# SkyTNT/midi-model

Measured on AMD Instinct MI355X. Metric: MIDI events/sec, training step (fwd+bwd+clip+AdamW), tv2o-medium, seq=2048, higher is better.
Workload: dtype bf16; 1 GPU; tv2o-medium bf16 training step, per-GPU batch 16 x 2048 events x 8 tokens (BASELINE.json configs[1]); random-init weights, synthetic events; global_batch=16, seq_len=2048, parallelism=dp1, accumulate_grad_batches=1, optimizer=AdamW bf16-true + global-norm clip 1.0

## Files before the change

### include/midihip.h

```cpp
#ifndef MIDIHIP_H
#define MIDIHIP_H
#include <stdint.h>
#ifdef __cplusplus
extern "C" {
#endif

#define MH_F32 0
#define MH_BF16 1

#define MH_OK 0
#define MH_ERR_ARG (-1)
#define MH_ERR_LAUNCH (-2)
#define MH_ERR_UNSUPPORTED (-3)

const char* mh_last_error(void);
int mh_version(void);
int mh_ab_builds(void);
int mh_set_option(const char* name, int value);
int mh_get_option(const char* name);

int mh_gemm_nt(const void* A, int64_t lda, const void* B, int64_t ldb, void* C, int64_t ldc, const void* R,
               int64_t ldr, int64_t M, int64_t N, int64_t K, float alpha, float beta, int dtype, int splitk,
               void* workspace, void* stream);
int mh_gemm(const void* A, int64_t lda, int transA, const void* B, int64_t ldb, int transB, void* C, int64_t ldc,
            const void* R, int64_t ldr, int64_t M, int64_t N, int64_t K, float alpha, float beta, int dtype, int splitk,
            void* workspace, void* stream);
int mh_gemm_swiglu(const void* A, int64_t lda, const void* W, int64_t ldw, void* GU, int64_t ldgu, void* ACT,
                   int64_t ldact, int64_t M, int64_t I, int64_t K, int dtype, void* stream);
int mh_gemm_rope(const void* A, int64_t lda, const void* W, int64_t ldw, void* C, int64_t ldc, const void* table,
                 int64_t npos, int64_t S, int64_t pos0, int head_dim, int64_t M, int64_t N, int64_t K, int dtype, void* stream);
int mh_gemm_dswiglu(const void* A, int64_t lda, const void* B, int64_t ldb, const void* GU, int64_t ldgu, void* DGU,
                    int64_t lddgu, int64_t M, int64_t I, int64_t K, int dtype, void* stream);
int mh_gemm_rowss(const void* A, int64_t lda, const void* B, int64_t ldb, void* C, int64_t ldc, const void* R, int64_t ldr,
                  float* rowss, int64_t M, int64_t N, int64_t K, int dtype, void* stream);
int mh_row_rstd(const void* x, int64_t ldx, const float* parts, int nparts, int64_t M, int D, float eps, float* rstd, int dtype,
                void* stream);
int mh_gemm_rope_scaled(const void* A, int64_t lda, const void* W, int64_t ldw, void* C, int64_t ldc, const void* table,
                        int64_t npos, int64_t S, int64_t pos0, int head_dim, const float* rowscale, int64_t M, int64_t N, int64_t K,
                        int dtype, void* stream);
int mh_gemm_swiglu_scaled(const void* A, int64_t lda, const void* W, int64_t ldw, void* GU, int64_t ldgu, void* ACT, int64_t ldact,
                          const float* rowscale, int64_t M, int64_t I, int64_t K, int dtype, void* stream);
int mh_gemm_nt_scaled(const void* A, int64_t lda, const void* B, int64_t ldb, void* C, int64_t ldc, const float* rowscale, int64_t M,
                      int64_t N, int64_t K, int dtype, void* stream);
int mh_gemm_dswiglu_scaled(const void* A, int64_t lda, const void* B, int64_t ldb, const void* GU, int64_t ldgu, void* DGU,
                           int64_t lddgu, const float* rowscale, int64_t M, int64_t I, int64_t K, int dtype, void* stream);
int mh_splitk_fold_blocks(int64_t M);
int mh_gemm_splitk_reduce_fold(const void* workspace, void* C, int64_t ldc, const void* R, int64_t ldr, int64_t M, int64_t N,
                               int splitk, float alpha, float beta, const void* wnorm, const void* W, int64_t ldw, float* colpart,
                               int dtype, void* stream);
int mh_rmsnorm_bwd_folded(const void* x, const float* rstd, const void* t, const void* dres, void* dx, int64_t M, int D, int dtype,
                          void* stream);
int mh_scale_cols(const void* W, int64_t ldw, const void* w, void* out, int64_t ldo, int64_t Nr, int K, int dtype, void* stream);
int mh_scale_cols_batched(const int64_t* jobs, int njobs, int K, int dtype, void* stream);
int mh_gemm_splitk_reduce(const void* workspace, void* C, int64_t ldc, const void* R, int64_t ldr, int64_t M,
                          int64_t N, int splitk, float alpha, float beta, int dtype, void* stream);
#define MH_SKINNY_PLAIN 0
#define MH_SKINNY_GATEUP 1
int mh_gemm_skinny(const void* A, int64_t lda, const void* W, int64_t ldw, void* C, int64_t ldc, const void* R,
                   int64_t ldr, int mode, float norm_eps, const int64_t* row_ids, const int64_t* res_ids, int64_t M,
                   int64_t N, int64_t K, int dtype, void* stream);
int mh_transpose(const void* in, int64_t ldi, void* out, int64_t ldo, int64_t rows, int64_t cols, int dtype,
                 void* stream);

int mh_embed_sum_fwd(const int64_t* tok, const void* table, void* out, int64_t M, int T, int64_t V, int D,
                     int dtype, void* stream);
int mh_concat_tok_fwd(const void* hidden, const int64_t* tok, int64_t ldtok, const void* table, void* out,
                      int64_t M, int T, int64_t V, int D, int dtype, void* stream);
int mh_embed_scatter_bwd(const int64_t* tok, int64_t ldtok, int T, const void* dout, int rows_per_m, int jstride,
                         int j0, float* dtable_f32, int64_t M, int64_t V, int D, int64_t pad_id, int dtype,
                         void* stream);
int mh_embed_segment_bwd(const int64_t* src_rows, const int64_t* seg_start, const void* dout, int64_t ld,
                         float* dtable_f32, int64_t V, int D, int64_t n_occ, int64_t pad_id, int dtype, void* stream);
int mh_token_segments_chunk(void);
int mh_token_segments(const int64_t* tok, int64_t ldtok, int64_t n_rows, int n_cols, int64_t V, int64_t row_mul,
                      int64_t col_mul, int64_t add, int64_t* src_rows, int64_t* seg_start, int32_t* work, void* stream);
int mh_cast_from_f32(const float* src, void* dst, int64_t n, int accumulate, int dtype, void* stream);
int mh_copy_rows(const void* src, int64_t src_ld, void* dst, int64_t dst_ld, int64_t M, int D, int accumulate,
                 int dtype, void* stream);

int mh_collate_windows(const int16_t* tokens, int64_t n_events, const int64_t* win_start, const int64_t* win_len,
                       int64_t* out, int64_t B, int64_t L, int T, int64_t pad_id, void* stream);

int mh_augment_piece_stats(const int16_t* tokens, const int64_t* piece_off, int64_t n_pieces, const int32_t* tab,
                           int32_t* stats, void* stream);
int mh_augment_collate_windows(const int16_t* tokens, int64_t n_events, const int64_t* win_start, const int64_t* win_len,
                               const int64_t* win_piece, const int32_t* shifts, const int32_t* stats, const int32_t* tab,
                               int64_t* out, int64_t B, int64_t L, int T, int64_t pad_id, void* stream);

int mh_rmsnorm_fwd(const void* x, const void* w, void* y, float* rstd, int64_t M, int D, float eps, int dtype,
                   void* stream);
int mh_rmsnorm_bwd_blocks(int64_t M);
int mh_rmsnorm_bwd(const void* x, const void* w, const float* rstd, const void* dy, const void* dres, void* dx,
                   float* dw_partial, int64_t M, int D, int dtype, void* stream);
int mh_colsum(float* partial , int64_t nblk, void* out, int D, int accumulate, int dtype, void* stream);

int mh_rope(void* qkv, const float* cos_t, const float* sin_t, int64_t M, int64_t S, int64_t pos0, int H, int hd,
            int dir, int dtype, void* stream);

int mh_attn_prep_fwd(const void* qkv, void* vt, int64_t B, int64_t S, int H, int dtype, void* stream);
int mh_attn_fwd(const void* qkv, const void* vt, void* o, float* lse, int64_t B, int64_t S, int H, float scale,
                int dtype, void* stream);
int mh_attn_prep_bwd(const void* qkv, const void* o, const void* dout, float* delta, void* qt, void* kt, void* dot,
                     int64_t B, int64_t S, int H, int dtype, void* stream);
int mh_attn_bwd(const void* qkv, const void* dout, const float* lse, const float* delta, const void* qt,
                const void* kt, const void* dot, void* dqkv, int64_t B, int64_t S, int H, float scale,
                const float* cos_t, const float* sin_t, int dtype, void* stream);
int mh_attn_bwd_o(const void* qkv, const void* o, const void* dout, const float* lse, float* delta, void* dqkv, int64_t B,
                  int64_t S, int H, float scale, const float* cos_t, const float* sin_t, int dtype, void* stream);
int mh_attn_bwd_o_scaled(const void* qkv, const void* o, const void* dout, const float* lse, float* delta, void* dqkv,
                         const float* rowscale, int64_t B, int64_t S, int H, float scale, const float* cos_t, const float* sin_t,
                         int dtype, void* stream);
int mh_attn_fwd_timeline(const void* qkv, void* o, float* lse, int64_t B, int64_t S, int H, float scale, int lazy,
                         uint32_t* stamps, void* stream);
int mh_attn_fwd_plain(const void* qkv, void* o, float* lse, int64_t B, int64_t S, int H, float scale, int dtype,
                      void* stream);
int mh_attn_bwd_plain(const void* qkv, const void* dout, const float* lse, const float* delta, void* dqkv, int64_t B,
                      int64_t S, int H, float scale, int dtype, void* stream);

int mh_tokattn_fwd(const void* qkv, void* o, int64_t N, int T, int H, float scale, const float* cos_t, const float* sin_t,
                   int dtype, void* stream);
int mh_tokattn_bwd(const void* qkv, const void* dout, void* dqkv, int64_t N, int T, int H, float scale, const float* cos_t,
                   const float* sin_t, int dtype, void* stream);
int mh_tokattn_bwd_scaled(const void* qkv, const void* dout, void* dqkv, const float* rowscale, int64_t N, int T, int H, float scale,
                          const float* cos_t, const float* sin_t, int dtype, void* stream);

int mh_swiglu_fwd(const void* gu, void* a, int64_t M, int I, int dtype, void* stream);
int mh_swiglu_bwd(const void* gu, const void* da, void* dgu, int64_t M, int I, int dtype, void* stream);

int mh_cross_entropy(const void* logits, int64_t ldl, const int64_t* target, float* row_loss, void* dlogits,
                     const float* scale_dev, int64_t* argmax_out, int64_t R, int V, int64_t ignore, int dtype,
                     void* stream);
int mh_sum_f32(const float* x, int64_t n, float* out, void* stream);
int mh_count_valid(const int64_t* target, int64_t n, int64_t ignore, float* count, float* inv, void* stream);

int mh_sumsq(const void* g, int64_t n, float* partial1024, float* out, int accumulate, int dtype, void* stream);
int mh_clip_coef(const float* sumsq, float max_norm, float* coef, float* norm, void* stream);
int mh_adamw(void* p, const void* g, void* m, void* v, int64_t n, float lr, float beta1, float beta2, float eps,
             float weight_decay, float bias_corr1, float bias_corr2, const float* coef_dev, int dtype, void* stream);

int mh_kv_append(void* qkv, const float* cos_t, const float* sin_t, void* kcache, void* vcache, int64_t B, int H,
                 int hd, int64_t Lmax, int64_t pos, const int32_t* pos_dev, int dtype, void* stream);
int mh_attn_decode(const void* qkv, const void* kcache, const void* vcache, void* o, int64_t B, int H, int hd,
                   int64_t Lmax, int64_t len, float scale, const int32_t* pos_dev, int dtype, void* stream);
int mh_attn_decode_append(const void* qkv, const float* cos_t, const float* sin_t, void* kcache, void* vcache, void* o,
                          int64_t B, int H, int hd, int64_t Lmax, int64_t pos, float scale, const int32_t* pos_dev,
                          int dtype, void* stream);
int mh_kv_store_rows(const void* qkv, void* kcache, void* vcache, int64_t B, int64_t S, int H, int hd, int64_t Lmax,
                     int64_t pos0, int dtype, void* stream);
int mh_kv_gather_rows(const void* kcache, const void* vcache, void* qkv, int64_t B, int64_t n, int64_t Stot, int H, int hd,
                      int64_t Lmax, int dtype, void* stream);
int mh_attn_fwd_tail(const void* qkv, void* o, float* lse, int64_t B, int64_t S, int H, float scale, int64_t q_start,
                     int dtype, void* stream);
int mh_kv_store_prefill(const void* qkv, void* kcache, void* vcache, int64_t B, int64_t S, int H, int hd,
                        int64_t Lmax, int dtype, void* stream);

int mh_masked_softmax(const void* logits, int64_t ldl, const int32_t* lo, const int32_t* hi,
                      const uint8_t* first_mask, float* probs, int64_t B, int V, float temp, int dtype,
                      void* stream);
int mh_sample_top_p_k(const void* logits, int64_t ldl, const uint8_t* first_mask, const uint8_t* ban_mask, int first_lo,
                      int first_hi,
                      const int32_t* lo_tab, const int32_t* hi_tab, int tab_stride, int max_range, const int64_t* ev,
                      int pos, const float* q, int64_t* out,
                      int64_t out_stride, int64_t* out_b, int64_t* out_c, int64_t B, int V, float temp, float top_p,
                      int top_k, int fill_rest, int64_t fill_id, int dtype, void* stream);

int mh_comm_unique_id(void* id128);
int mh_comm_init(int rank, int world, const void* id128, int device, void** comm_out);
int mh_comm_info(void* comm, int* rank, int* world, int* rccl_version);
int mh_comm_allreduce(void* comm, void* buf, int64_t count, int dtype, int mean, void* stream);
int mh_comm_broadcast(void* comm, void* buf, int64_t count, int dtype, int root, void* stream);
int mh_comm_destroy(void* comm);

#ifdef __cplusplus
}
#endif
#endif
```

### midi-model_amd/csrc/attention_mfma.hip

```cpp
#include "attn_mfma_common.h"

#ifdef MH_AB_BUILDS
template <bool MASK>
__device__ inline void fwd_tile(const char* tK, const char* tV, const bf16x8 (&qf)[4], f32x16 (&oacc)[2], float& m,
                                float& l, int pli, int hi, int qrel, float sc) {
  f32x16 sacc[2] = {zero16(), zero16()};
#pragma unroll
  for (int kb = 0; kb < 2; ++kb)
#pragma unroll
    for (int s = 0; s < 4; ++s) sacc[kb] = mfma32(lds_frag(tK, kb * 32 + pli, 2 * s + hi), qf[s], sacc[kb]);
  float mx = -INFINITY;
#pragma unroll
  for (int kb = 0; kb < 2; ++kb)
#pragma unroll
    for (int r = 0; r < 16; ++r) {
      if (MASK) {
        if (kb * 32 + reg_index(r, hi) > qrel) sacc[kb][r] = -INFINITY;
      }
      mx = fmaxf(mx, sacc[kb][r]);
    }
  mx = fmaxf(mx, __shfl_xor(mx, 32, 64)) * sc;
  float mn = m, alpha = 1.f;
  if (__any(mx > m + RESCALE_THR)) {
    mn = fmaxf(m, mx);
// ... 291 lines not shown
  f32x16 dkacc[2] = {zero16(), zero16()}, dvacc[2] = {zero16(), zero16()};
  const int pli = pi32(li);
  const int qt_first = k0 / 64, qt_last = (S - 1) / 64;

  auto stage_all = [&](int qt, char* dst) {
    stage64(qbase, D3, (int64_t)qt * 64, S - 1, 0, dst, wave, lane);
    stage64(dobase, D, (int64_t)qt * 64, S - 1, 0, dst + TILE64, wave, lane);
    stage64(qtbase, Sp, 0, HD - 1, (int64_t)qt * 64, dst + 2 * TILE64, wave, lane);
    stage64(dotbase, Sp, 0, HD - 1, (int64_t)qt * 64, dst + 3 * TILE64, wave, lane);
    if (wave < 2) {
      const float* base = (wave == 0 ? lse_b : delta_b) + (int64_t)qt * 64;
      int l15 = lane & 15;
      asm volatile("" : "+v"(l15));
      glds16(base + 4 * l15, dst + 4 * TILE64 + wave * 1024);
    }
  };
  if (qt_first <= qt_last) stage_all(qt_first, smem);
#pragma unroll
  for (int s = 0; s < 4; ++s) {
    asm volatile("" : "+v"(kf[s]));
    asm volatile("" : "+v"(vf[s]));
  }
  __syncthreads();
  for (int qt = qt_first; qt <= qt_last; ++qt) {
    const int st = (qt - qt_first) & 1;
    const char* cur = smem + st * STG;
    char* nxt = smem + (st ^ 1) * STG;
    if (qt + 1 <= qt_last) stage_all(qt + 1, nxt);
    const int qs = qt * 64;
    if (qs + 63 >= kw0) {
      if (qs < kw0 + 31 || qs + 64 > S)
        dkv_tile<true>(cur, cur + TILE64, cur + 2 * TILE64, cur + 3 * TILE64, kf, vf, dkacc, dvacc, cur + 4 * TILE64, pli, hi,
                       krow - qs, S - qs, sc);
      else
        dkv_tile<false>(cur, cur + TILE64, cur + 2 * TILE64, cur + 3 * TILE64, kf, vf, dkacc, dvacc, cur + 4 * TILE64, pli, hi,
                        0, 64, sc);
    }
    __syncthreads();
  }
  if (krow < S) {
    bf16* krow_out = dqkv + (b * S + krow) * D3 + D + (int64_t)h * HD;
    store_grad_row(krow_out, dkacc, scale, hi, cos_t, sin_t, krow);
    store_grad_row(krow_out + D, dvacc, 1.f, hi, nullptr, nullptr, 0);
  }
}

#endif

extern thread_local int g_attn_v3;
int mh_attn_fwd_mfma3(const void* qkv, const void* vt, void* o, float* lse, int64_t B, int64_t S, int H, float scale,
                      hipStream_t st, int64_t q_start = 0);
int mh_attn_bwd_mfma3(const void* qkv, const void* dout, const float* lse, const float* delta, const void* qt, const void* kt,
                      const void* dot, void* dqkv, int64_t B, int64_t S, int H, float scale, const float* cos_t,
                      const float* sin_t, int which, hipStream_t st, const void* o = nullptr);

int mh_attn_fwd_mfma(const void* qkv, const void* vt, void* o, float* lse, int64_t B, int64_t S, int H, float scale,
                     hipStream_t st, int64_t q_start) {
  MH_REQUIRE(S < (1 << 24), "attn_fwd: sequence too long");
  if ((g_attn_v3 & 1) && (vt != nullptr || (g_attn_v3 & 16)))
    return mh_attn_fwd_mfma3(qkv, vt, o, lse, B, S, H, scale, st, q_start);
  MH_REQUIRE(q_start == 0, "attn_fwd_tail: served by the third form of the forward kernel only");
#ifndef MH_AB_BUILDS
  MH_REQUIRE(false, "attn_fwd(bf16): option attn_v3 = %d selects the first form of the kernel, which is only in the A/B test "
             "library (libmidihip_ab.so)", g_attn_v3);
#else
  MH_REQUIRE(vt != nullptr, "attn_fwd(bf16): the first form needs the transposed V copy (mh_attn_prep_fwd)");
  const int64_t Sp = (S + 63) / 64 * 64;
  const int nt = (int)((S + 127) / 128), BH = (int)(B * H);
  const unsigned grid = (unsigned)(nt * 8 * ((BH + 7) / 8));
  attn_fwd_kernel<<<grid, 256, 4 * TILE64, st>>>((const bf16*)qkv, (const bf16*)vt, (bf16*)o, lse, (int)S, (int)Sp, H,
                                        scale * LOG2E, BH, nt);
  MH_LAUNCH_CHECK();
  return MH_OK;
#endif
}

int mh_attn_bwd_o_mfma(const void* qkv, const void* o, const void* dout, const float* lse, float* delta, void* dqkv, int64_t B,
                       int64_t S, int H, float scale, const float* cos_t, const float* sin_t, hipStream_t st) {
  MH_REQUIRE(S < (1 << 24), "attn_bwd: sequence too long");
  MH_REQUIRE((g_attn_v3 & 14) == 14, "attn_bwd_o: served by the third form with transpose reads (mh_set_option(\"attn_v3\") bits 2|4|8); "
             "use mh_attn_prep_bwd + mh_attn_bwd otherwise");
  return mh_attn_bwd_mfma3(qkv, dout, lse, delta, nullptr, nullptr, nullptr, dqkv, B, S, H, scale, cos_t, sin_t, 14, st, o);
}

int mh_attn_bwd_mfma(const void* qkv, const void* dout, const float* lse, const float* delta, const void* qt,
                     const void* kt, const void* dot, void* dqkv, int64_t B, int64_t S, int H, float scale,
                     const float* cos_t, const float* sin_t, hipStream_t st) {
  MH_REQUIRE(S < (1 << 24), "attn_bwd: sequence too long");
  if ((g_attn_v3 & 14) == 14)
    return mh_attn_bwd_mfma3(qkv, dout, lse, delta, nullptr, nullptr, nullptr, dqkv, B, S, H, scale, cos_t, sin_t, 14, st);
  MH_REQUIRE(qt != nullptr && kt != nullptr && dot != nullptr, "attn_bwd(bf16): needs the transposed copies (mh_attn_prep_bwd)");
  const int64_t Sp = (S + 63) / 64 * 64;
  const int nt = (int)((S + 127) / 128), BH = (int)(B * H);
  const unsigned grid = (unsigned)(nt * 8 * ((BH + 7) / 8));
  if (g_attn_v3 & 6) {
    const int rc = mh_attn_bwd_mfma3(qkv, dout, lse, delta, qt, kt, dot, dqkv, B, S, H, scale, cos_t, sin_t, g_attn_v3 & 14, st);
    if (rc != MH_OK) return rc;
  }
#ifndef MH_AB_BUILDS
  MH_REQUIRE((g_attn_v3 & 6) == 6, "attn_bwd(bf16): option attn_v3 = %d selects first-form kernels, which are only in the A/B "
             "test library (libmidihip_ab.so)", g_attn_v3);
#else
  if (!(g_attn_v3 & 2)) {
    attn_bwd_dq_kernel<<<grid, 256, 6 * TILE64, st>>>((const bf16*)qkv, (const bf16*)dout, lse, delta, (const bf16*)kt,
                                             (bf16*)dqkv, (int)S, (int)Sp, H, scale, BH, nt, cos_t, sin_t);
    MH_LAUNCH_CHECK();
  }
  if (!(g_attn_v3 & 4)) {
    attn_bwd_dkv_kernel<<<grid, 256, 2 * DKV_STAGE, st>>>((const bf16*)qkv, (const bf16*)dout, lse, delta, (const bf16*)qt,
                                              (const bf16*)dot, (bf16*)dqkv, (int)S, (int)Sp, H, scale, BH, nt, cos_t, sin_t);
    MH_LAUNCH_CHECK();
  }
#endif
  (void)grid;
  return MH_OK;
}
```

### midi-model_amd/csrc/attention_mfma3.hip

```cpp
#include <stdlib.h>

#include "attn_mfma_common.h"

static int attn_env_int(const char* name, int dflt) {
  const char* v = getenv(name);
  return (v && *v) ? atoi(v) : dflt;
}
thread_local int g_attn_v3 = attn_env_int("MH_ATTN_V3", 255);
thread_local int g_attn_passes = attn_env_int("MH_ATTN_PASSES", 5);
thread_local int g_attn_v3_wps = attn_env_int("MH_ATTN_V3_WPS", 0);
thread_local const float* g_attn_bwd_rowscale = nullptr;

__device__ inline bf16x8 ldsv(const char* p) { return *reinterpret_cast<const bf16x8*>(p); }
typedef __attribute__((ext_vector_type(2))) float f32x2;
typedef __attribute__((ext_vector_type(2))) __bf16 bf16x2;
__device__ inline bf16x8 pack8_pk(const f32x16& v, int base) {
  union {
    bf16x8 v;
    bf16x2 h[4];
  } r;
#pragma unroll
  for (int i = 0; i < 4; ++i) r.h[i] = __builtin_convertvector(f32x2{v[base + 2 * i], v[base + 2 * i + 1]}, bf16x2);
  return r.v;
}
__device__ inline float xhalf_max(float v) {
  const int iv = __float_as_int(v);
  const auto pr = __builtin_amdgcn_permlane32_swap(iv, iv, false, false);
  return fmaxf(__int_as_float(pr[0]), __int_as_float(pr[1]));
}

constexpr float LZ_BOUND = 1099511627776.f;
__device__ inline uint64_t tl_now() {
  uint64_t t;
  asm volatile("s_memtime %0" : "=s"(t));
  return t;
}
template <bool MASK, bool TR, bool LZ = false, bool TL = false>
__device__ inline void fwd3_tile(const char* tK, const char* tV, const int (&trof)[2][2], const int (&foff)[4],
                                 const bf16x8 (&qf)[4], f32x16 (&oacc)[2], float& m, float& l, int hi, int qrel, float sc,
                                 uint64_t* ts = nullptr) {
  bf16x8 kf[2][4];
#pragma unroll
  for (int s = 0; s < 4; ++s)
#pragma unroll
    for (int kb = 0; kb < 2; ++kb) kf[kb][s] = ldsv(tK + foff[s] + kb * 4096);
  __builtin_amdgcn_sched_barrier(0);
  if constexpr (TL) ts[2] = tl_now();
  f32x16 sacc[2] = {zero16(), zero16()};
#pragma unroll
  for (int s = 0; s < 4; ++s)
#pragma unroll
    for (int kb = 0; kb < 2; ++kb) sacc[kb] = mfma32(kf[kb][s], qf[s], sacc[kb]);
  bf16x8 vf[4][2];
  u32x2 vr[4][2][2];
  if (TR) {
    unsigned tv[2][2];
#pragma unroll
    for (int db = 0; db < 2; ++db)
#pragma unroll
      for (int half = 0; half < 2; ++half) tv[db][half] = lds_addr32(tV) + (unsigned)trof[db][half];
#pragma unroll
    for (int db = 0; db < 2; ++db)
#pragma unroll
      for (int half = 0; half < 2; ++half) {
// ... 743 lines not shown
#define MH_FWD(WPS, TR_, LZ_)                                                                                                    \
  attn_fwd3_kernel<WPS, TR_, 2, LZ_><<<grid, 256, 4 * TILE64, st>>>((const bf16*)qkv, (const bf16*)vt, (bf16*)o, lse, (int)S, (int)Sp, H, \
                                                                 scale * LOG2E, BH, nt, nt_all)
#define MH_FWD3S(WPS, TR_, LZ_)                                                                                                  \
  attn_fwd3_kernel<WPS, TR_, 3, LZ_><<<grid, 256, 6 * TILE64, st>>>((const bf16*)qkv, (const bf16*)vt, (bf16*)o, lse, (int)S, (int)Sp, \
                                                                  H, scale * LOG2E, BH, nt, nt_all)
  const bool tr = (vt == nullptr);
  const bool lz = (g_attn_v3 & 128) != 0;
  if (tr && g_attn_v3_wps == 4) {
    if (lz) MH_FWD(4, true, true); else MH_FWD(4, true, false);
  } else if (tr && (g_attn_v3 & 64)) {
    if (lz) {
      if (g_attn_v3_wps == 3) MH_FWD3S(3, true, true); else MH_FWD3S(2, true, true);
    } else {
      if (g_attn_v3_wps == 3) MH_FWD3S(3, true, false); else MH_FWD3S(2, true, false);
    }
  } else if (tr) {
    if (g_attn_v3_wps == 3) MH_FWD(3, true, false); else MH_FWD(2, true, false);
  } else {
    if (g_attn_v3_wps == 2) MH_FWD(2, false, false); else MH_FWD(3, false, false);
  }
#undef MH_FWD
#undef MH_FWD3S
  MH_LAUNCH_CHECK();
  return MH_OK;
}

extern "C" int mh_attn_fwd_timeline(const void* qkv, void* o, float* lse, int64_t B, int64_t S, int H, float scale, int lazy,
                                    uint32_t* stamps, void* stream) {
#ifdef MH_AB_BUILDS
  MH_REQUIRE(stamps != nullptr && S >= 128 && S * 3 * H * HD < (int64_t(1) << 31), "attn_fwd_timeline: bad arguments");
  hipStream_t st = (hipStream_t)stream;
  const int64_t Sp = (S + 63) / 64 * 64;
  const int nt_all = (int)((S + 127) / 128), BH0 = (int)(B * H), nt = nt_all;
  const int BH = BH0 | ((g_attn_passes & 127) << 24);
  const unsigned grid = (unsigned)(nt * 8 * ((BH0 + 7) / 8));
  if (lazy)
    attn_fwd3_kernel<2, true, 3, true, true><<<grid, 256, 6 * TILE64 + TL_BYTES, st>>>((const bf16*)qkv, (const bf16*)stamps, (bf16*)o, lse, (int)S,
                                                                                   (int)Sp, H, scale * LOG2E, BH, nt, nt_all);
  else
    attn_fwd3_kernel<2, true, 3, false, true><<<grid, 256, 6 * TILE64 + TL_BYTES, st>>>((const bf16*)qkv, (const bf16*)stamps, (bf16*)o, lse, (int)S,
                                                                                    (int)Sp, H, scale * LOG2E, BH, nt, nt_all);
  MH_LAUNCH_CHECK();
  return MH_OK;
#else
  mh_set_error("attn_fwd_timeline: only in the A/B library (libmidihip_ab.so)");
  return MH_ERR_UNSUPPORTED;
#endif
}

int mh_attn_bwd_mfma3(const void* qkv, const void* dout, const float* lse, const float* delta, const void* qt, const void* kt,
                      const void* dot, void* dqkv, int64_t B, int64_t S, int H, float scale, const float* cos_t,
                      const float* sin_t, int which ,
                      hipStream_t st, const void* o ) {
  MH_REQUIRE(o == nullptr || (which & 14) == 14, "attn_bwd: delta inside the dQ kernel needs the third form of both kernels");
  MH_REQUIRE(S * 3 * H * HD < (int64_t(1) << 31), "attn_bwd: sequence too long (32-bit panel offsets)");
  const bool tr = (which & 8) != 0;
  MH_REQUIRE(tr || (qt != nullptr && kt != nullptr && dot != nullptr), "attn_bwd(bf16): needs the transposed copies (mh_attn_prep_bwd)");
  const int64_t Sp = (S + 63) / 64 * 64;
  const int nt = (int)((S + 127) / 128), BH0 = (int)(B * H);
  MH_REQUIRE(BH0 < (1 << 24), "attn_bwd: too many (batch, head) pairs");
  const int BH = BH0 | ((g_attn_passes & 127) << 24);
  const unsigned grid = (unsigned)(nt * 8 * ((BH0 + 7) / 8));
#define MH_DQ(WPS, TR_)                                                                                                     \
  attn_bwd_dq3_kernel<WPS, TR_><<<grid, 256, (TR_ ? 4 : 6) * TILE64, st>>>((const bf16*)qkv, (const bf16*)dout, lse, delta,     \
                                                                        (const bf16*)kt, (bf16*)dqkv, (int)S, (int)Sp, H, scale, \
                                                                        BH, nt, cos_t, sin_t, (const bf16*)o,         \
                                                                        const_cast<float*>(delta), g_attn_bwd_rowscale)
  if (which & 2) {
    if (g_attn_v3_wps == 2) {
      if (tr) MH_DQ(2, true); else MH_DQ(2, false);
    } else {
      if (tr) MH_DQ(3, true); else MH_DQ(3, false);
    }
    MH_LAUNCH_CHECK();
  }
#undef MH_DQ
  if (which & 4) {
    if (tr && o != nullptr)
      attn_bwd_dkv3_kernel<true, true><<<grid, 256, 2 * (2 * TILE64 + 2048), st>>>((const bf16*)qkv, (const bf16*)dout,
                                                                                 delta + (int64_t)BH0 * Sp, delta, nullptr, nullptr,
                                                                                 (bf16*)dqkv, (int)S, (int)Sp, H, scale, BH, nt,
                                                                                 cos_t, sin_t, g_attn_bwd_rowscale);
    else if (tr)
      attn_bwd_dkv3_kernel<true><<<grid, 256, 2 * (2 * TILE64 + 2048), st>>>((const bf16*)qkv, (const bf16*)dout, lse, delta, nullptr,
                                                                           nullptr, (bf16*)dqkv, (int)S, (int)Sp, H, scale, BH, nt,
                                                                           cos_t, sin_t, g_attn_bwd_rowscale);
    else
      attn_bwd_dkv3_kernel<false><<<grid, 256, 2 * DKV_STAGE, st>>>((const bf16*)qkv, (const bf16*)dout, lse, delta, (const bf16*)qt,
                                                                  (const bf16*)dot, (bf16*)dqkv, (int)S, (int)Sp, H, scale, BH, nt,
                                                                  cos_t, sin_t, g_attn_bwd_rowscale);
    MH_LAUNCH_CHECK();
  }
  return MH_OK;
}
```

### midi-model_amd/csrc/attention_small.hip

```cpp
#include "common.h"

#define DISPATCH_T(dtype, CALL)                                    \
  do {                                                             \
    if ((dtype) == MH_BF16) { using T = bf16; CALL; }              \
    else if ((dtype) == MH_F32) { using T = float; CALL; }         \
    else { mh_set_error("bad dtype %d", (int)(dtype)); return MH_ERR_ARG; } \
  } while (0)

template <typename T> __device__ inline void ld4(const T* p, float (&o)[4]);
template <> __device__ inline void ld4<float>(const float* p, float (&o)[4]) {
  f32x4 v = *reinterpret_cast<const f32x4*>(p);
  o[0] = v[0]; o[1] = v[1]; o[2] = v[2]; o[3] = v[3];
}
template <> __device__ inline void ld4<bf16>(const bf16* p, float (&o)[4]) {
  bf16x4 v = *reinterpret_cast<const bf16x4*>(p);
  o[0] = (float)v[0]; o[1] = (float)v[1]; o[2] = (float)v[2]; o[3] = (float)v[3];
}
template <typename T> __device__ inline void st4(T* p, const float (&o)[4]);
template <> __device__ inline void st4<float>(float* p, const float (&o)[4]) {
  *reinterpret_cast<f32x4*>(p) = f32x4{o[0], o[1], o[2], o[3]};
}
template <> __device__ inline void st4<bf16>(bf16* p, const float (&o)[4]) {
  bf16x4 v;
  v[0] = (bf16)o[0]; v[1] = (bf16)o[1]; v[2] = (bf16)o[2]; v[3] = (bf16)o[3];
// ... 90 lines not shown
      for (int t = 0; t < TN; ++t) {
        unpack(kraw[t], k[t]);
        unpack(vraw[t], v[t]);
        if (rot) rope_row<T>(k[t], rope_c, rope_s, t, lane, 1.f, true);
      }
    } else {
#pragma unroll
      for (int t = 0; t < TK; ++t) {
        if (t < Tn) {
          ldp<T>(base + t * D3 + D, lane, k[t]);
          ldp<T>(base + t * D3 + 2 * D, lane, v[t]);
          if (rot) rope_row<T>(k[t], rope_c, rope_s, t, lane, 1.f, true);
        }
      }
    }
#pragma unroll
    for (int i = 0; i < TK; ++i) {
      if (TN ? i >= TN : i >= Tn) break;
      float q[4];
      if constexpr (TN != 0) unpack(qraw[i], q);
      else ldp<T>(base + i * D3, lane, q);
      if (rot) rope_row<T>(q, rope_c, rope_s, i, lane, 1.f, true);
      float s[TK];
      float mx = -INFINITY;
#pragma unroll
      for (int j = 0; j <= i; ++j) {
        float p = q[0] * k[j][0] + q[1] * k[j][1] + q[2] * k[j][2] + q[3] * k[j][3];
        s[j] = wave_sum_fast(p) * scale;
        mx = fmaxf(mx, s[j]);
      }
      float den = 0.f;
#pragma unroll
      for (int j = 0; j <= i; ++j) {
        s[j] = __expf(s[j] - mx);
        den += s[j];
      }
      const float inv = 1.f / den;
      float acc[4] = {0.f, 0.f, 0.f, 0.f};
#pragma unroll
      for (int j = 0; j <= i; ++j) {
        const float p = s[j] * inv;
#pragma unroll
        for (int e = 0; e < 4; ++e) acc[e] += p * v[j][e];
      }
      stp<T>(o + (n * Tn + i) * D + (int64_t)h * 256, lane, acc);
    }
  }
}

template <typename T, int TN, bool BR>
__global__ __launch_bounds__(256) void tokattn_bwd_kernel(const T* __restrict__ qkv, const T* __restrict__ dout,
                                                          T* __restrict__ dqkv, int64_t NH, int Tn, int H, float scale,
                                                          const float* __restrict__ cos_t, const float* __restrict__ sin_t,
                                                          const float* __restrict__ rowscale ) {
  const int lane = threadIdx.x & 63;
  const int64_t D = (int64_t)H * 256, D3 = 3 * D;
  __shared__ float rope_c[TK * 128], rope_s[TK * 128];
  const bool rot = cos_t != nullptr;
  if (rot) {
    for (int i = threadIdx.x; i < Tn * 128; i += 256) {
      rope_c[i] = rnd<T>(cos_t[i]);
      rope_s[i] = rnd<T>(sin_t[i]);
    }
    __syncthreads();
  }
  for (int64_t w = (int64_t)blockIdx.x * 4 + (threadIdx.x >> 6); w < NH; w += (int64_t)gridDim.x * 4) {
    const int64_t n = w / H;
    const int h = (int)(w - n * H);
    const int64_t off = (int64_t)h * 256;
    const T* base = qkv + n * Tn * D3 + off;
    T* ob = dqkv + n * Tn * D3 + off;
    float k[TK][4], v[TK][4], dk[TK][4], dv[TK][4];
    RawRow<T> qraw[TN ? TN : 1], doraw[TN ? TN : 1];
    const float rs_lane = (rowscale != nullptr && lane < Tn) ? rowscale[n * Tn + lane] : 1.f;
#pragma unroll
    for (int t = 0; t < TK; ++t)
#pragma unroll
      for (int e = 0; e < 4; ++e) dk[t][e] = dv[t][e] = 0.f;
    if constexpr (TN != 0) {
      RawRow<T> kraw[TN ? TN : 1], vraw[TN ? TN : 1];
#pragma unroll
      for (int t = 0; t < TN; ++t) {
        kraw[t] = ldraw<T>(base + t * D3 + D, lane);
        vraw[t] = ldraw<T>(base + t * D3 + 2 * D, lane);
      }
#pragma unroll
      for (int t = 0; t < TN; ++t) {
        qraw[t] = ldraw<T>(base + t * D3, lane);
        doraw[t] = ldraw<T>(dout + (n * Tn + t) * D + off, lane);
      }
#pragma unroll
      for (int t = 0; t < TN; ++t) {
        unpack(kraw[t], k[t]);
        unpack(vraw[t], v[t]);
        if (rot) rope_row<T>(k[t], rope_c, rope_s, t, lane, 1.f, true);
      }
    } else {
#pragma unroll
      for (int t = 0; t < TK; ++t) {
        if (t < Tn) {
          ldp<T>(base + t * D3 + D, lane, k[t]);
          ldp<T>(base + t * D3 + 2 * D, lane, v[t]);
          if (rot) rope_row<T>(k[t], rope_c, rope_s, t, lane, 1.f, true);
        }
      }
    }
#pragma unroll
    for (int i = 0; i < TK; ++i) {
      if (TN ? i >= TN : i >= Tn) break;
      float q[4], dO[4], dq[4] = {0.f, 0.f, 0.f, 0.f};
      if constexpr (TN != 0) {
        unpack(qraw[i], q);
        unpack(doraw[i], dO);
      } else {
        ldp<T>(base + i * D3, lane, q);
        ldp<T>(dout + (n * Tn + i) * D + off, lane, dO);
      }
      if (rot) rope_row<T>(q, rope_c, rope_s, i, lane, 1.f, true);
      float p[TK], dp[TK];
      float mx = -INFINITY;
      if constexpr (BR) {
#pragma unroll
        for (int j = 0; j <= i; j += 2) {
          const bool two = j + 1 <= i;
          const int j1 = two ? j + 1 : j;
          const float a0 = q[0] * k[j][0] + q[1] * k[j][1] + q[2] * k[j][2] + q[3] * k[j][3];
          const float b0 = dO[0] * v[j][0] + dO[1] * v[j][1] + dO[2] * v[j][2] + dO[3] * v[j][3];
          const float a1 = two ? q[0] * k[j1][0] + q[1] * k[j1][1] + q[2] * k[j1][2] + q[3] * k[j1][3] : 0.f;
          const float b1 = two ? dO[0] * v[j1][0] + dO[1] * v[j1][1] + dO[2] * v[j1][2] + dO[3] * v[j1][3] : 0.f;
          const float r4 = wave_sum4(a0, b0, a1, b1);
          p[j] = wave_sum4_get<0>(r4) * scale;
          dp[j] = wave_sum4_get<1>(r4);
          mx = fmaxf(mx, p[j]);
          if (two) {
            p[j1] = wave_sum4_get<2>(r4) * scale;
            dp[j1] = wave_sum4_get<3>(r4);
            mx = fmaxf(mx, p[j1]);
          }
        }
      } else {
#pragma unroll
      for (int j = 0; j <= i; ++j) {
        float a = q[0] * k[j][0] + q[1] * k[j][1] + q[2] * k[j][2] + q[3] * k[j][3];
        float b = dO[0] * v[j][0] + dO[1] * v[j][1] + dO[2] * v[j][2] + dO[3] * v[j][3];
        p[j] = wave_sum_fast(a) * scale;
        dp[j] = wave_sum_fast(b);
        mx = fmaxf(mx, p[j]);
      }
      }
      float den = 0.f;
#pragma unroll
      for (int j = 0; j <= i; ++j) {
        p[j] = __expf(p[j] - mx);
        den += p[j];
      }
      const float inv = 1.f / den;
      float dsum = 0.f;
#pragma unroll
      for (int j = 0; j <= i; ++j) {
        p[j] *= inv;
        dsum += p[j] * dp[j];
      }
#pragma unroll
      for (int j = 0; j <= i; ++j) {
        const float ds = p[j] * (dp[j] - dsum) * scale;
#pragma unroll
        for (int e = 0; e < 4; ++e) {
          dq[e] += ds * k[j][e];
          dk[j][e] += ds * q[e];
          dv[j][e] += p[j] * dO[e];
        }
      }
      if (rot) rope_row<T>(dq, rope_c, rope_s, i, lane, -1.f, false);
      if (rowscale != nullptr) {
        const float rsc = __shfl(rs_lane, i, 64);
#pragma unroll
        for (int e = 0; e < 4; ++e) dq[e] *= rsc;
      }
      stp<T>(ob + i * D3, lane, dq);
    }
#pragma unroll
    for (int t = 0; t < TK; ++t) {
      if (TN ? t < TN : t < Tn) {
        if (rot) rope_row<T>(dk[t], rope_c, rope_s, t, lane, -1.f, false);
        if (rowscale != nullptr) {
          const float rsc = __shfl(rs_lane, t, 64);
#pragma unroll
          for (int e = 0; e < 4; ++e) {
            dk[t][e] *= rsc;
            dv[t][e] *= rsc;
          }
        }
        stp<T>(ob + t * D3 + D, lane, dk[t]);
        stp<T>(ob + t * D3 + 2 * D, lane, dv[t]);
      }
    }
  }
}

extern "C" int mh_tokattn_fwd(const void* qkv, void* o, int64_t N, int Tn, int H, float scale, const float* cos_t,
                              const float* sin_t, int dtype, void* stream) {
  MH_REQUIRE(N > 0 && Tn >= 1 && Tn <= TK && H >= 1, "tokattn_fwd: bad shape N=%ld T=%d H=%d", (long)N, Tn, H);
  const int64_t NH = N * H;
  int64_t g = (NH + 3) / 4;
  if (g > 32768) g = 32768;
  if (Tn == TK)
    DISPATCH_T(dtype, (tokattn_fwd_kernel<T, TK><<<(int)g, 256, 0, (hipStream_t)stream>>>((const T*)qkv, (T*)o, NH, Tn, H, scale,
                                                                                          cos_t, sin_t)));
  else
    DISPATCH_T(dtype, (tokattn_fwd_kernel<T, 0><<<(int)g, 256, 0, (hipStream_t)stream>>>((const T*)qkv, (T*)o, NH, Tn, H, scale,
                                                                                         cos_t, sin_t)));
  MH_LAUNCH_CHECK();
  return MH_OK;
}

thread_local int g_tokattn_bwd_batched = 1;
static int tokattn_bwd_any(const void* qkv, const void* dout, void* dqkv, const float* rowscale, int64_t N, int Tn, int H, float scale,
                           const float* cos_t, const float* sin_t, int dtype, void* stream) {
  MH_REQUIRE(N > 0 && Tn >= 1 && Tn <= TK && H >= 1, "tokattn_bwd: bad shape");
  const int64_t NH = N * H;
  int64_t g = (NH + 3) / 4;
  if (g > 32768) g = 32768;
  if (Tn == TK && g_tokattn_bwd_batched)
    DISPATCH_T(dtype, (tokattn_bwd_kernel<T, TK, true><<<(int)g, 256, 0, (hipStream_t)stream>>>(
                          (const T*)qkv, (const T*)dout, (T*)dqkv, NH, Tn, H, scale, cos_t, sin_t, rowscale)));
  else if (Tn == TK)
    DISPATCH_T(dtype, (tokattn_bwd_kernel<T, TK, false><<<(int)g, 256, 0, (hipStream_t)stream>>>(
                          (const T*)qkv, (const T*)dout, (T*)dqkv, NH, Tn, H, scale, cos_t, sin_t, rowscale)));
  else
    DISPATCH_T(dtype, (tokattn_bwd_kernel<T, 0, false><<<(int)g, 256, 0, (hipStream_t)stream>>>(
                          (const T*)qkv, (const T*)dout, (T*)dqkv, NH, Tn, H, scale, cos_t, sin_t, rowscale)));
  MH_LAUNCH_CHECK();
  return MH_OK;
}
extern "C" int mh_tokattn_bwd(const void* qkv, const void* dout, void* dqkv, int64_t N, int Tn, int H, float scale,
                              const float* cos_t, const float* sin_t, int dtype, void* stream) {
  return tokattn_bwd_any(qkv, dout, dqkv, nullptr, N, Tn, H, scale, cos_t, sin_t, dtype, stream);
}
extern "C" int mh_tokattn_bwd_scaled(const void* qkv, const void* dout, void* dqkv, const float* rowscale, int64_t N, int Tn, int H,
                                     float scale, const float* cos_t, const float* sin_t, int dtype, void* stream) {
  MH_REQUIRE(rowscale != nullptr, "tokattn_bwd_scaled: rowscale is NULL");
  return tokattn_bwd_any(qkv, dout, dqkv, rowscale, N, Tn, H, scale, cos_t, sin_t, dtype, stream);
}

template <typename T>
__global__ __launch_bounds__(256) void kv_append_kernel(T* __restrict__ qkv, const float* __restrict__ cos_t,
                                                        const float* __restrict__ sin_t, T* __restrict__ kc,
                                                        T* __restrict__ vc, int64_t B, int H, int hd, int64_t Lmax,
                                                        int64_t pos, const int32_t* __restrict__ pos_dev) {
  if (pos_dev != nullptr) pos = *pos_dev;
  if (pos >= Lmax) return;
  const int half = hd / 2;
  const int64_t total = B * H * half;
  const int64_t D = (int64_t)H * hd;
  for (int64_t it = (int64_t)blockIdx.x * 256 + threadIdx.x; it < total; it += (int64_t)gridDim.x * 256) {
    const int i = (int)(it % half);
    const int64_t bh = it / half;
    const int h = (int)(bh % H);
    const int64_t b = bh / H;
    const float c = rnd<T>(cos_t[pos * half + i]), s = rnd<T>(sin_t[pos * half + i]);
    T* row = qkv + b * 3 * D + (int64_t)h * hd;
    const float q1 = to_f(row[i]), q2 = to_f(row[i + half]);
    row[i] = from_f<T>(q1 * c - q2 * s);
    row[i + half] = from_f<T>(q2 * c + q1 * s);
    const float k1 = to_f(row[D + i]), k2 = to_f(row[D + i + half]);
    const T kr1 = from_f<T>(k1 * c - k2 * s), kr2 = from_f<T>(k2 * c + k1 * s);
    row[D + i] = kr1;
    row[D + i + half] = kr2;
    T* kd = kc + ((b * H + h) * Lmax + pos) * hd;
    T* vd = vc + ((b * H + h) * Lmax + pos) * hd;
    kd[i] = kr1;
    kd[i + half] = kr2;
    vd[i] = row[2 * D + i];
    vd[i + half] = row[2 * D + i + half];
  }
}

extern "C" int mh_kv_append(void* qkv, const float* cos_t, const float* sin_t, void* kcache, void* vcache, int64_t B,
                            int H, int hd, int64_t Lmax, int64_t pos, const int32_t* pos_dev, int dtype, void* stream) {
  MH_REQUIRE(B > 0 && H > 0 && hd % 2 == 0 && ((pos >= 0 && pos < Lmax) || pos_dev != nullptr),
             "kv_append: bad args (pos=%ld Lmax=%ld)", (long)pos, (long)Lmax);
  const int64_t total = B * H * (hd / 2);
  DISPATCH_T(dtype, (kv_append_kernel<T><<<(int)((total + 255) / 256), 256, 0, (hipStream_t)stream>>>(
                        (T*)qkv, cos_t, sin_t, (T*)kcache, (T*)vcache, B, H, hd, Lmax, pos, pos_dev)));
  MH_LAUNCH_CHECK();
  return MH_OK;
}

template <typename T>
__global__ __launch_bounds__(256) void kv_store_prefill_kernel(const T* __restrict__ qkv, T* __restrict__ kc,
                                                               T* __restrict__ vc, int64_t B, int64_t S, int H, int hd,
                                                               int64_t Lmax, int64_t pos0) {
  constexpr int N = Pack<T>::N;
  const int cph = hd / N;
  const int64_t total = B * S * H * cph;
// ... 517 lines not shown
#pragma unroll
    for (int e = 0; e < N; ++e) tile[i][ch * N + e] = v.v[e];
  }
  __syncthreads();
  for (int p = 0; p < 64 / RPP; ++p) {
    const int d = rr + p * RPP;
    Pack<T> v;
#pragma unroll
    for (int e = 0; e < N; ++e) v.v[e] = tile[ch * N + e][d];
    st16(out + (bh * 64 + d) * Sp + s0 + ch * N, v);
  }
}

template <typename T>
static int transpose_heads(const T* in, int64_t ld, int64_t col0, T* out, int64_t B, int64_t S, int H, hipStream_t st) {
  const int64_t Sp = (S + 63) / 64 * 64;
  dim3 grid((unsigned)(Sp / 64), (unsigned)(B * H));
  attn_transpose_kernel<T><<<grid, 256, 0, st>>>(in, ld, col0, out, S, Sp, H);
  MH_LAUNCH_CHECK();
  return MH_OK;
}

extern "C" int mh_attn_prep_fwd(const void* qkv, void* vt, int64_t B, int64_t S, int H, int dtype, void* stream) {
  MH_REQUIRE(B > 0 && S > 0 && H > 0 && B * H < 65536, "attn_prep_fwd: bad shape");
  if (dtype != MH_BF16) return MH_OK;
  const int64_t D = (int64_t)H * 64;
  return transpose_heads<bf16>((const bf16*)qkv, 3 * D, 2 * D, (bf16*)vt, B, S, H, (hipStream_t)stream);
}

extern "C" int mh_attn_prep_bwd(const void* qkv, const void* o, const void* dout, float* delta, void* qt, void* kt,
                                void* dot, int64_t B, int64_t S, int H, int dtype, void* stream) {
  MH_REQUIRE(B > 0 && S > 0 && H > 0 && B * H < 65536, "attn_prep_bwd: bad shape");
  hipStream_t st = (hipStream_t)stream;
  const int64_t total = B * S * H;
  int64_t g = (total * 8 + 255) / 256;
  if (g > 16384) g = 16384;
  DISPATCH_T(dtype, (attn_delta_kernel<T><<<(int)g, 256, 0, st>>>((const T*)o, (const T*)dout, delta, B, S, H)));
  MH_LAUNCH_CHECK();
  if (dtype != MH_BF16 || qt == nullptr) return MH_OK;
  const int64_t D = (int64_t)H * 64;
  int rc;
  if ((rc = transpose_heads<bf16>((const bf16*)qkv, 3 * D, 0, (bf16*)qt, B, S, H, st)) != MH_OK) return rc;
  if ((rc = transpose_heads<bf16>((const bf16*)qkv, 3 * D, D, (bf16*)kt, B, S, H, st)) != MH_OK) return rc;
  return transpose_heads<bf16>((const bf16*)dout, D, 0, (bf16*)dot, B, S, H, st);
}

int mh_attn_fwd_mfma(const void* qkv, const void* vt, void* o, float* lse, int64_t B, int64_t S, int H, float scale,
                     hipStream_t st, int64_t q_start);
int mh_attn_bwd_mfma(const void* qkv, const void* dout, const float* lse, const float* delta, const void* qt,
                     const void* kt, const void* dot, void* dqkv, int64_t B, int64_t S, int H, float scale,
                     const float* cos_t, const float* sin_t, hipStream_t st);

int mh_attn_bwd_o_mfma(const void* qkv, const void* o, const void* dout, const float* lse, float* delta, void* dqkv, int64_t B,
                       int64_t S, int H, float scale, const float* cos_t, const float* sin_t, hipStream_t st);

template <typename T>
static int attn_plain_fwd(const void* qkv, void* o, float* lse, int64_t B, int64_t S, int H, float scale, hipStream_t st,
                          int64_t q_start = 0) {
  const int first = (int)(q_start / 64);
  dim3 grid((unsigned)((S + 63) / 64 - first), (unsigned)(B * H));
  attn_plain_fwd_kernel<T><<<grid, 64, 0, st>>>((const T*)qkv, (T*)o, lse, S, H, scale, first);
  MH_LAUNCH_CHECK();
  return MH_OK;
}

template <typename T>
static int attn_plain_bwd(const void* qkv, const void* dout, const float* lse, const float* delta, void* dqkv, int64_t B,
                          int64_t S, int H, float scale, hipStream_t st) {
  dim3 grid((unsigned)((S + 63) / 64), (unsigned)(B * H));
  attn_plain_bwd_dq_kernel<T><<<grid, 64, 0, st>>>((const T*)qkv, (const T*)dout, lse, delta, (T*)dqkv, S, H, scale);
  MH_LAUNCH_CHECK();
  attn_plain_bwd_dkv_kernel<T><<<grid, 64, 0, st>>>((const T*)qkv, (const T*)dout, lse, delta, (T*)dqkv, S, H, scale);
  MH_LAUNCH_CHECK();
  return MH_OK;
}

extern "C" int mh_attn_fwd_plain(const void* qkv, void* o, float* lse, int64_t B, int64_t S, int H, float scale,
                                 int dtype, void* stream) {
  MH_REQUIRE(B > 0 && S > 0 && H > 0 && B * H < 65536, "attn_fwd: bad shape");
  DISPATCH_T(dtype, return attn_plain_fwd<T>(qkv, o, lse, B, S, H, scale, (hipStream_t)stream));
}

extern "C" int mh_attn_bwd_plain(const void* qkv, const void* dout, const float* lse, const float* delta, void* dqkv,
                                 int64_t B, int64_t S, int H, float scale, int dtype, void* stream) {
  MH_REQUIRE(B > 0 && S > 0 && H > 0 && B * H < 65536, "attn_bwd: bad shape");
  DISPATCH_T(dtype, return attn_plain_bwd<T>(qkv, dout, lse, delta, dqkv, B, S, H, scale, (hipStream_t)stream));
}

extern "C" int mh_attn_fwd(const void* qkv, const void* vt, void* o, float* lse, int64_t B, int64_t S, int H, float scale,
                           int dtype, void* stream) {
  MH_REQUIRE(B > 0 && S > 0 && H > 0 && B * H < 65536, "attn_fwd: bad shape");
  if (dtype == MH_BF16) return mh_attn_fwd_mfma(qkv, vt, o, lse, B, S, H, scale, (hipStream_t)stream, 0);
  if (dtype == MH_F32) return attn_plain_fwd<float>(qkv, o, lse, B, S, H, scale, (hipStream_t)stream);
  mh_set_error("attn_fwd: bad dtype");
  return MH_ERR_ARG;
}

extern "C" int mh_attn_fwd_tail(const void* qkv, void* o, float* lse, int64_t B, int64_t S, int H, float scale, int64_t q_start,
                                int dtype, void* stream) {
  MH_REQUIRE(B > 0 && S > 0 && H > 0 && B * H < 65536 && q_start >= 0 && q_start < S, "attn_fwd_tail: bad shape");
  if (dtype == MH_BF16) return mh_attn_fwd_mfma(qkv, nullptr, o, lse, B, S, H, scale, (hipStream_t)stream, q_start);
  if (dtype == MH_F32) return attn_plain_fwd<float>(qkv, o, lse, B, S, H, scale, (hipStream_t)stream, q_start);
  mh_set_error("attn_fwd_tail: bad dtype");
  return MH_ERR_ARG;
}

extern "C" int mh_rope(void* qkv, const float* cos_t, const float* sin_t, int64_t M, int64_t S, int64_t pos0, int H, int hd,
                       int dir, int dtype, void* stream);

extern "C" int mh_attn_bwd(const void* qkv, const void* dout, const float* lse, const float* delta, const void* qt,
                           const void* kt, const void* dot, void* dqkv, int64_t B, int64_t S, int H, float scale,
                           const float* cos_t, const float* sin_t, int dtype, void* stream) {
  MH_REQUIRE(B > 0 && S > 0 && H > 0 && B * H < 65536, "attn_bwd: bad shape");
  MH_REQUIRE((cos_t == nullptr) == (sin_t == nullptr), "attn_bwd: cos and sin tables come together");
  if (dtype == MH_BF16)
    return mh_attn_bwd_mfma(qkv, dout, lse, delta, qt, kt, dot, dqkv, B, S, H, scale, cos_t, sin_t, (hipStream_t)stream);
  if (dtype == MH_F32) {
    int rc = attn_plain_bwd<float>(qkv, dout, lse, delta, dqkv, B, S, H, scale, (hipStream_t)stream);
    if (rc == MH_OK && cos_t != nullptr) rc = mh_rope(dqkv, cos_t, sin_t, B * S, S, 0, H, 64, -1, dtype, stream);
    return rc;
  }
  mh_set_error("attn_bwd: bad dtype");
  return MH_ERR_ARG;
}

extern thread_local const float* g_attn_bwd_rowscale;
extern thread_local int g_attn_v3;
extern "C" int mh_attn_bwd_o_scaled(const void* qkv, const void* o, const void* dout, const float* lse, float* delta, void* dqkv,
                                    const float* rowscale, int64_t B, int64_t S, int H, float scale, const float* cos_t,
                                    const float* sin_t, int dtype, void* stream) {
  MH_REQUIRE(rowscale != nullptr, "attn_bwd_o_scaled: rowscale is NULL");
  MH_REQUIRE((g_attn_v3 & 46) == 46, "attn_bwd_o_scaled: needs the third form of the backward kernels (attn_v3 bits 1, 2, 3, 5)");
  g_attn_bwd_rowscale = rowscale;
  const int rc = mh_attn_bwd_o(qkv, o, dout, lse, delta, dqkv, B, S, H, scale, cos_t, sin_t, dtype, stream);
  g_attn_bwd_rowscale = nullptr;
  return rc;
}

extern "C" int mh_attn_bwd_o(const void* qkv, const void* o, const void* dout, const float* lse, float* delta, void* dqkv,
                             int64_t B, int64_t S, int H, float scale, const float* cos_t, const float* sin_t, int dtype,
                             void* stream) {
  MH_REQUIRE(B > 0 && S > 0 && H > 0 && B * H < 65536, "attn_bwd_o: bad shape");
  MH_REQUIRE((cos_t == nullptr) == (sin_t == nullptr), "attn_bwd_o: cos and sin tables come together");
  MH_REQUIRE(dtype == MH_BF16, "attn_bwd_o: bf16 only (fp32: mh_attn_prep_bwd + mh_attn_bwd)");
  return mh_attn_bwd_o_mfma(qkv, o, dout, lse, delta, dqkv, B, S, H, scale, cos_t, sin_t, (hipStream_t)stream);
}
```

### midi-model_amd/csrc/elementwise.hip

```cpp
#include "common.h"

#define DISPATCH_T(dtype, CALL)                                    \
  do {                                                             \
    if ((dtype) == MH_BF16) { using T = bf16; CALL; }              \
    else if ((dtype) == MH_F32) { using T = float; CALL; }         \
    else { mh_set_error("bad dtype %d", (int)(dtype)); return MH_ERR_ARG; } \
  } while (0)

static inline int grid_for(int64_t items, int per_block, int cap = 1 << 20) {
  int64_t g = (items + per_block - 1) / per_block;
  if (g < 1) g = 1;
  if (g > cap) g = cap;
  return (int)g;
}

template <typename T>
__global__ __launch_bounds__(256) void embed_sum_fwd_kernel(const int64_t* __restrict__ tok, const T* __restrict__ table,
                                                            T* __restrict__ out, int64_t M, int TT, int D, int64_t V) {
  constexpr int N = Pack<T>::N;
  const int lane = threadIdx.x & 63;
  const int64_t wave0 = (int64_t)blockIdx.x * 4 + (threadIdx.x >> 6);
  for (int64_t m = wave0; m < M; m += (int64_t)gridDim.x * 4) {
    constexpr int TMAXI = 8;
    int64_t ids[TMAXI];
// ... 489 lines not shown
  else
    DISPATCH_T(dtype, (rmsnorm_fwd_kernel<T><<<grid_for(M, 4, 65536), 256, 0, (hipStream_t)stream>>>(
                          (const T*)x, (const T*)w, (T*)y, rstd, M, D, eps)));
#undef MH_RMSF
  MH_LAUNCH_CHECK();
  return MH_OK;
}

__global__ __launch_bounds__(256) void rstd_from_parts_kernel(const float* __restrict__ parts, int nparts, int64_t M, float inv_d,
                                                              float eps, float* __restrict__ rstd) {
  __shared__ float acc[4][64];
  const int r = threadIdx.x & 63, q = threadIdx.x >> 6;
  const int64_t m = (int64_t)blockIdx.x * 64 + r;
  float ss = 0.f;
  if (m < M) {
#pragma unroll 4
    for (int p = q; p < nparts; p += 4) ss += parts[(int64_t)p * M + m];
  }
  acc[q][r] = ss;
  __syncthreads();
  if (q == 0 && m < M) rstd[m] = rsqrtf((acc[0][r] + acc[1][r] + acc[2][r] + acc[3][r]) * inv_d + eps);
}
template <typename T>
__global__ __launch_bounds__(256) void row_rstd_kernel(const T* __restrict__ x, int64_t ldx, int64_t M, int D, float eps,
                                                       float* __restrict__ rstd) {
  constexpr int N = Pack<T>::N;
  const int lane = threadIdx.x & 63;
  for (int64_t m = (int64_t)blockIdx.x * 4 + (threadIdx.x >> 6); m < M; m += (int64_t)gridDim.x * 4) {
    const T* xr = x + m * ldx;
    float ss = 0.f;
    for (int c = lane * N; c < D; c += 64 * N) {
      Pack<T> v = ld16(xr + c);
#pragma unroll
      for (int e = 0; e < N; ++e) ss += v.get(e) * v.get(e);
    }
    ss = wave_sum(ss);
    if (lane == 0) rstd[m] = rsqrtf(ss / (float)D + eps);
  }
}
extern "C" int mh_row_rstd(const void* x, int64_t ldx, const float* parts, int nparts, int64_t M, int D, float eps, float* rstd,
                           int dtype, void* stream) {
  MH_REQUIRE(M > 0 && D > 0 && rstd != nullptr && ((x != nullptr) != (parts != nullptr)), "row_rstd: give x OR parts (M=%ld D=%d)", (long)M, D);
  if (parts != nullptr) {
    MH_REQUIRE(nparts > 0 && (int64_t)nparts * 64 == D, "row_rstd: nparts = %d must be D / 64 (D = %d): one sum of squares per 64 columns", nparts, D);
    rstd_from_parts_kernel<<<(unsigned)((M + 63) / 64), 256, 0, (hipStream_t)stream>>>(parts, nparts, M, 1.0f / (float)D, eps, rstd);
  } else {
    MH_REQUIRE(D % 8 == 0 && ldx % 8 == 0 && ldx >= D && ((uintptr_t)x & 15) == 0, "row_rstd: rows must be 16-byte aligned");
    DISPATCH_T(dtype, (row_rstd_kernel<T><<<grid_for(M, 4, 65536), 256, 0, (hipStream_t)stream>>>((const T*)x, ldx, M, D, eps, rstd)));
  }
  MH_LAUNCH_CHECK();
  return MH_OK;
}

constexpr int RMS_BWD_MAX_BLOCKS = 1024;
extern "C" int mh_rmsnorm_bwd_blocks(int64_t M) {
  int64_t g = (M + 3) / 4;
  return (int)(g < RMS_BWD_MAX_BLOCKS ? (g < 1 ? 1 : g) : RMS_BWD_MAX_BLOCKS);
}

template <typename T>
__global__ __launch_bounds__(256) void rmsnorm_bwd_kernel(const T* __restrict__ x, const T* __restrict__ w,
                                                          const float* __restrict__ rstd, const T* __restrict__ dy,
                                                          const T* dres, T* dx, float* __restrict__ dw_partial,
                                                          int64_t M, int D) {
  constexpr int N = Pack<T>::N;
  extern __shared__ __attribute__((aligned(16))) float dw_acc[];
  const int lane = threadIdx.x & 63, wv = threadIdx.x >> 6;
  float* mine = dw_acc + wv * D;
  for (int c = lane; c < D; c += 64) mine[c] = 0.f;
  __syncthreads();
  for (int64_t m = (int64_t)blockIdx.x * 4 + wv; m < M; m += (int64_t)gridDim.x * 4) {
    const T* xr = x + m * D;
    const T* gr = dy + m * D;
    const float r = rstd[m];
    float dot = 0.f;
    for (int c = lane * N; c < D; c += 64 * N) {
      Pack<T> xv = ld16(xr + c), gv = ld16(gr + c), wv_ = ld16(w + c);
#pragma unroll
      for (int e = 0; e < N; ++e) dot += gv.get(e) * wv_.get(e) * (xv.get(e) * r);
    }
    dot = wave_sum(dot) / (float)D;
    for (int c = lane * N; c < D; c += 64 * N) {
      Pack<T> xv = ld16(xr + c), gv = ld16(gr + c), wv_ = ld16(w + c), o;
      Pack<T> rv;
      if (dres != nullptr) rv = ld16(dres + m * D + c);
#pragma unroll
      for (int e = 0; e < N; ++e) {
        const float xh = xv.get(e) * r;
        float d = r * (gv.get(e) * wv_.get(e) - xh * dot);
        if (dres != nullptr) d += rv.get(e);
        o.set(e, d);
        mine[c + e] += gv.get(e) * rnd<T>(xh);
      }
      st16(dx + m * D + c, o);
    }
  }
  __syncthreads();
  for (int c = threadIdx.x; c < D; c += 256)
    dw_partial[(int64_t)blockIdx.x * D + c] = dw_acc[c] + dw_acc[D + c] + dw_acc[2 * D + c] + dw_acc[3 * D + c];
}

template <typename T, int NCH, bool NT>
__global__ __launch_bounds__(256) void rmsnorm_bwd_reg_kernel(const T* __restrict__ x, const T* __restrict__ w,
                                                              const float* __restrict__ rstd, const T* __restrict__ dy,
                                                              const T* dres, T* dx, float* __restrict__ dw_partial,
                                                              int64_t M, int D) {
// ... 388 lines not shown
```

### midi-model_amd/csrc/gemm.hip

```cpp
#include <type_traits>

#include "common.h"

__device__ __attribute__((aligned(16))) char g_zero16[16];

template <typename T> struct Mma;
template <> struct Mma<bf16> {
  __device__ static inline f32x4 run(const Pack<bf16>& a, const Pack<bf16>& b, f32x4 c) {
    return __builtin_amdgcn_mfma_f32_16x16x32_bf16(a.v, b.v, c, 0, 0, 0);
  }
};
template <> struct Mma<float> {
  __device__ static inline f32x4 run(const Pack<float>& a, const Pack<float>& b, f32x4 c) {
#pragma unroll
    for (int e = 0; e < 4; ++e) c = __builtin_amdgcn_mfma_f32_16x16x4f32(a.v[e], b.v[e], c, 0, 0, 0);
    return c;
  }
};

constexpr int BM = 128, BN = 128;
constexpr int TILE_BYTES = 128 * 128;

template <typename T>
__device__ inline void stage_tile(const T* __restrict__ base, int64_t ld, int64_t row0, int64_t nrows, int64_t k0,
// ... 250 lines not shown
}

template <bool FOLD>
__global__ __launch_bounds__(256) void splitk_reduce4_kernel(const float* __restrict__ ws, bf16* __restrict__ C, int64_t ldc,
                                                             const bf16* R, int64_t ldr, int64_t M, int64_t N, int splitk,
                                                             float alpha, float beta, const bf16* __restrict__ wnorm,
                                                             const bf16* __restrict__ W, int64_t ldw, float* __restrict__ colpart);

template <typename T>
static int splitk_reduce_launch(const void* workspace, void* C, int64_t ldc, const void* R, int64_t ldr, int64_t M,
                                int64_t N, int splitk, float alpha, float beta, hipStream_t st) {
  MH_REQUIRE(M > 0 && N > 0 && splitk >= 1 && workspace != nullptr, "splitk_reduce: bad args");
  if constexpr (std::is_same<T, bf16>::value) {
    if (N % 4 == 0 && ldc % 4 == 0 && (R == nullptr || ldr % 4 == 0) && (((uintptr_t)C | (uintptr_t)R) & 7) == 0 &&
        ((uintptr_t)workspace & 15) == 0) {
      const int64_t rows_y = M < 2048 ? M : 2048;
      dim3 grid((unsigned)((N / 4 + 255) / 256), (unsigned)rows_y);
      splitk_reduce4_kernel<false><<<grid, 256, 0, st>>>((const float*)workspace, (bf16*)C, ldc, (const bf16*)R, ldr, M, N, splitk, alpha,
                                                         beta, nullptr, nullptr, 0, nullptr);
      MH_LAUNCH_CHECK();
      return MH_OK;
    }
  }
  const int64_t total = M * N;
  const int blocks = (int)((total + 255) / 256 < 4096 ? (total + 255) / 256 : 4096);
  splitk_reduce_kernel<T><<<blocks, 256, 0, st>>>((const float*)workspace, (T*)C, ldc, (const T*)R, ldr, M, N, splitk,
                                                  alpha, beta);
  MH_LAUNCH_CHECK();
  return MH_OK;
}

extern "C" int mh_gemm_splitk_reduce(const void* workspace, void* C, int64_t ldc, const void* R, int64_t ldr, int64_t M,
                                     int64_t N, int splitk, float alpha, float beta, int dtype, void* stream) {
  hipStream_t st = (hipStream_t)stream;
  if (dtype == MH_BF16) return splitk_reduce_launch<bf16>(workspace, C, ldc, R, ldr, M, N, splitk, alpha, beta, st);
  if (dtype == MH_F32) return splitk_reduce_launch<float>(workspace, C, ldc, R, ldr, M, N, splitk, alpha, beta, st);
  mh_set_error("splitk_reduce: bad dtype %d", dtype);
  return MH_ERR_ARG;
}

extern "C" int mh_gemm(const void* A, int64_t lda, int transA, const void* B, int64_t ldb, int transB, void* C,
                       int64_t ldc, const void* R, int64_t ldr, int64_t M, int64_t N, int64_t K, float alpha, float beta,
                       int dtype, int splitk, void* workspace, void* stream) {
  hipStream_t st = (hipStream_t)stream;
  if (dtype == MH_BF16)
    return gemm_launch<bf16>(A, lda, transA, B, ldb, transB, C, ldc, R, ldr, M, N, K, alpha, beta, splitk, workspace, st);
  if (dtype == MH_F32)
    return gemm_launch<float>(A, lda, transA, B, ldb, transB, C, ldc, R, ldr, M, N, K, alpha, beta, splitk, workspace, st);
  mh_set_error("gemm: bad dtype %d", dtype);
  return MH_ERR_ARG;
}

int mh_gemm_pp256_dswiglu_bf16(const void* A, int64_t lda, const void* B, int64_t ldb, const void* GU, int64_t ldgu,
                               void* DGU, int64_t lddgu, int64_t M, int64_t I, int64_t K, hipStream_t st, const float* rowscale);
int mh_gemm_pp256_scaled_bf16(const void* A, int64_t lda, const void* B, int64_t ldb, void* C, int64_t ldc, int64_t M, int64_t N,
                              int64_t K, const float* rowscale, hipStream_t st);

int mh_gemm_pp256_swiglu_bf16(const void* A, int64_t lda, const void* W, int64_t ldw, void* GU, int64_t ldgu, void* ACT,
                              int64_t ldact, int64_t M, int64_t I, int64_t K, hipStream_t st, const float* rowscale);

static int gemm_swiglu_any(const void* A, int64_t lda, const void* W, int64_t ldw, void* GU, int64_t ldgu, void* ACT,
                           int64_t ldact, const float* rowscale, int64_t M, int64_t I, int64_t K, int dtype, void* stream);

extern "C" int mh_gemm_swiglu(const void* A, int64_t lda, const void* W, int64_t ldw, void* GU, int64_t ldgu, void* ACT,
                              int64_t ldact, int64_t M, int64_t I, int64_t K, int dtype, void* stream) {
  return gemm_swiglu_any(A, lda, W, ldw, GU, ldgu, ACT, ldact, nullptr, M, I, K, dtype, stream);
}
extern "C" int mh_gemm_swiglu_scaled(const void* A, int64_t lda, const void* W, int64_t ldw, void* GU, int64_t ldgu, void* ACT,
                                     int64_t ldact, const float* rowscale, int64_t M, int64_t I, int64_t K, int dtype, void* stream) {
  MH_REQUIRE(rowscale != nullptr && ((uintptr_t)rowscale & 15) == 0, "gemm_swiglu_scaled: rowscale must be a 16-byte aligned fp32 [M]");
  return gemm_swiglu_any(A, lda, W, ldw, GU, ldgu, ACT, ldact, rowscale, M, I, K, dtype, stream);
}

static int gemm_swiglu_any(const void* A, int64_t lda, const void* W, int64_t ldw, void* GU, int64_t ldgu, void* ACT,
                           int64_t ldact, const float* rowscale, int64_t M, int64_t I, int64_t K, int dtype, void* stream) {
  MH_REQUIRE(dtype == MH_BF16 && g_mh_gemm_variant != 0,
             "gemm_swiglu: served by the production bf16 kernel only (use mh_gemm + mh_swiglu_fwd otherwise)");
  MH_REQUIRE(M > 0 && I > 0 && K > 0 && I % 128 == 0, "gemm_swiglu: bad shape M=%ld I=%ld K=%ld (I must be a multiple of 128)",
             (long)M, (long)I, (long)K);
  MH_REQUIRE(lda % 8 == 0 && ldw % 8 == 0 && ldact % 8 == 0 && lda >= K && ldw >= K && ldact >= I &&
                 (GU == nullptr || (ldgu % 8 == 0 && ldgu >= 2 * I)),
             "gemm_swiglu: leading dimensions must be multiples of 8 elements and cover the rows");
  MH_REQUIRE((((uintptr_t)A | (uintptr_t)W | (uintptr_t)GU | (uintptr_t)ACT) & 15) == 0, "gemm_swiglu: 16-byte alignment");
  return mh_gemm_pp256_swiglu_bf16(A, lda, W, ldw, GU, ldgu, ACT, ldact, M, I, K, (hipStream_t)stream, rowscale);
}

int mh_gemm_pp256_rope_bf16(const void* A, int64_t lda, const void* W, int64_t ldw, void* C, int64_t ldc, const void* table,
                            int64_t S, int64_t pos0, int64_t M, int64_t N, int64_t K, hipStream_t st, const float* rowscale);

static int gemm_rope_any(const void* A, int64_t lda, const void* W, int64_t ldw, void* C, int64_t ldc, const void* table,
                         int64_t npos, int64_t S, int64_t pos0, int head_dim, const float* rowscale, int64_t M, int64_t N, int64_t K,
                         int dtype, void* stream);

extern "C" int mh_gemm_rope(const void* A, int64_t lda, const void* W, int64_t ldw, void* C, int64_t ldc, const void* table,
                            int64_t npos, int64_t S, int64_t pos0, int head_dim, int64_t M, int64_t N, int64_t K, int dtype,
                            void* stream) {
  return gemm_rope_any(A, lda, W, ldw, C, ldc, table, npos, S, pos0, head_dim, nullptr, M, N, K, dtype, stream);
}
extern "C" int mh_gemm_rope_scaled(const void* A, int64_t lda, const void* W, int64_t ldw, void* C, int64_t ldc, const void* table,
                                   int64_t npos, int64_t S, int64_t pos0, int head_dim, const float* rowscale, int64_t M, int64_t N,
                                   int64_t K, int dtype, void* stream) {
  MH_REQUIRE(rowscale != nullptr && ((uintptr_t)rowscale & 15) == 0, "gemm_rope_scaled: rowscale must be a 16-byte aligned fp32 [M]");
  return gemm_rope_any(A, lda, W, ldw, C, ldc, table, npos, S, pos0, head_dim, rowscale, M, N, K, dtype, stream);
}

static int gemm_rope_any(const void* A, int64_t lda, const void* W, int64_t ldw, void* C, int64_t ldc, const void* table,
                         int64_t npos, int64_t S, int64_t pos0, int head_dim, const float* rowscale, int64_t M, int64_t N, int64_t K,
                         int dtype, void* stream) {
  MH_REQUIRE(dtype == MH_BF16 && g_mh_gemm_variant != 0,
             "gemm_rope: served by the production bf16 kernel only (use mh_gemm + mh_rope otherwise)");
  MH_REQUIRE(M > 0 && K > 0 && N > 0 && N % 192 == 0 && head_dim == 64,
             "gemm_rope: bad shape M=%ld N=%ld K=%ld head_dim=%d (N = 3 * heads * 64)", (long)M, (long)N, (long)K, head_dim);
  MH_REQUIRE(S > 0 && pos0 >= 0 && pos0 + (S < M ? S : M) <= npos && npos < (int64_t(1) << 31), "gemm_rope: table too short");
  MH_REQUIRE(S < (int64_t(1) << 31), "gemm_rope: S = %ld does not fit the 32 bits it travels in", (long)S);
  MH_REQUIRE(lda % 8 == 0 && ldw % 8 == 0 && ldc % 8 == 0 && lda >= K && ldw >= K && ldc >= N,
             "gemm_rope: leading dimensions must be multiples of 8 elements and cover the rows");
  MH_REQUIRE((((uintptr_t)A | (uintptr_t)W | (uintptr_t)C | (uintptr_t)table) & 15) == 0, "gemm_rope: 16-byte alignment");
  return mh_gemm_pp256_rope_bf16(A, lda, W, ldw, C, ldc, table, S, pos0, M, N, K, (hipStream_t)stream, rowscale);
}

int mh_gemm_pp256_rowss_bf16(const void* A, int64_t lda, const void* B, int64_t ldb, void* C, int64_t ldc, const void* R,
                             int64_t ldr, int64_t M, int64_t N, int64_t K, float* rowss, hipStream_t st);

extern "C" int mh_gemm_rowss(const void* A, int64_t lda, const void* B, int64_t ldb, void* C, int64_t ldc, const void* R,
                             int64_t ldr, float* rowss, int64_t M, int64_t N, int64_t K, int dtype, void* stream) {
  MH_REQUIRE(dtype == MH_BF16 && g_mh_gemm_variant != 0, "gemm_rowss: served by the production bf16 kernel only");
  MH_REQUIRE(M > 0 && N > 0 && K > 0 && N % 64 == 0 && rowss != nullptr, "gemm_rowss: bad shape M=%ld N=%ld K=%ld (N must be a multiple of 64)",
             (long)M, (long)N, (long)K);
  MH_REQUIRE(lda % 8 == 0 && ldb % 8 == 0 && ldc % 8 == 0 && lda >= K && ldb >= K && ldc >= N && (R == nullptr || (ldr % 8 == 0 && ldr >= N)),
             "gemm_rowss: leading dimensions must be multiples of 8 elements and cover the rows");
  MH_REQUIRE((((uintptr_t)A | (uintptr_t)B | (uintptr_t)C | (uintptr_t)R) & 15) == 0, "gemm_rowss: 16-byte alignment");
  MH_REQUIRE(((M + 255) / 256) * ((N + 255) / 256) < (1ll << 30), "gemm_rowss: too many tiles");
  return mh_gemm_pp256_rowss_bf16(A, lda, B, ldb, C, ldc, R, ldr, M, N, K, rowss, (hipStream_t)stream);
}

extern "C" int mh_gemm_dswiglu(const void* A, int64_t lda, const void* B, int64_t ldb, const void* GU, int64_t ldgu,
                               void* DGU, int64_t lddgu, int64_t M, int64_t I, int64_t K, int dtype, void* stream) {
  MH_REQUIRE(dtype == MH_BF16 && g_mh_gemm_variant != 0,
             "gemm_dswiglu: served by the production bf16 kernel only (use mh_gemm + mh_swiglu_bwd otherwise)");
  MH_REQUIRE(M > 0 && I > 0 && K > 0 && I % 8 == 0, "gemm_dswiglu: bad shape M=%ld I=%ld K=%ld", (long)M, (long)I, (long)K);
  MH_REQUIRE(lda % 8 == 0 && ldb % 8 == 0 && ldgu % 8 == 0 && lddgu % 8 == 0 && lda >= K && ldb >= I && ldgu >= 2 * I &&
                 lddgu >= 2 * I,
             "gemm_dswiglu: leading dimensions must be multiples of 8 elements and cover the rows");
  MH_REQUIRE((((uintptr_t)A | (uintptr_t)B | (uintptr_t)GU | (uintptr_t)DGU) & 15) == 0, "gemm_dswiglu: 16-byte alignment");
  return mh_gemm_pp256_dswiglu_bf16(A, lda, B, ldb, GU, ldgu, DGU, lddgu, M, I, K, (hipStream_t)stream, nullptr);
}

extern "C" int mh_gemm_dswiglu_scaled(const void* A, int64_t lda, const void* B, int64_t ldb, const void* GU, int64_t ldgu,
                                      void* DGU, int64_t lddgu, const float* rowscale, int64_t M, int64_t I, int64_t K, int dtype,
                                      void* stream) {
  MH_REQUIRE(dtype == MH_BF16 && g_mh_gemm_variant != 0, "gemm_dswiglu_scaled: served by the production bf16 kernel only");
  MH_REQUIRE(rowscale != nullptr && ((uintptr_t)rowscale & 15) == 0, "gemm_dswiglu_scaled: rowscale must be a 16-byte aligned fp32 [M]");
  MH_REQUIRE(M > 0 && I > 0 && K > 0 && I % 8 == 0, "gemm_dswiglu_scaled: bad shape M=%ld I=%ld K=%ld", (long)M, (long)I, (long)K);
  MH_REQUIRE(lda % 8 == 0 && ldb % 8 == 0 && ldgu % 8 == 0 && lddgu % 8 == 0 && lda >= K && ldb >= I && ldgu >= 2 * I &&
                 lddgu >= 2 * I,
             "gemm_dswiglu_scaled: leading dimensions must be multiples of 8 elements and cover the rows");
  MH_REQUIRE((((uintptr_t)A | (uintptr_t)B | (uintptr_t)GU | (uintptr_t)DGU) & 15) == 0, "gemm_dswiglu_scaled: 16-byte alignment");
  return mh_gemm_pp256_dswiglu_bf16(A, lda, B, ldb, GU, ldgu, DGU, lddgu, M, I, K, (hipStream_t)stream, rowscale);
}

extern "C" int mh_gemm_nt_scaled(const void* A, int64_t lda, const void* B, int64_t ldb, void* C, int64_t ldc,
                                 const float* rowscale, int64_t M, int64_t N, int64_t K, int dtype, void* stream) {
  MH_REQUIRE(dtype == MH_BF16 && g_mh_gemm_variant != 0, "gemm_nt_scaled: served by the production bf16 kernel only");
  MH_REQUIRE(rowscale != nullptr && ((uintptr_t)rowscale & 15) == 0, "gemm_nt_scaled: rowscale must be a 16-byte aligned fp32 [M]");
  MH_REQUIRE(M > 0 && N > 0 && K > 0, "gemm_nt_scaled: empty problem");
  MH_REQUIRE(lda % 8 == 0 && ldb % 8 == 0 && lda >= K && ldb >= K && ldc >= N, "gemm_nt_scaled: leading dimensions");
  MH_REQUIRE((((uintptr_t)A | (uintptr_t)B) & 15) == 0, "gemm_nt_scaled: 16-byte alignment");
  MH_REQUIRE(((M + 255) / 256) * ((N + 255) / 256) < (1ll << 30), "gemm_nt_scaled: too many tiles");
  return mh_gemm_pp256_scaled_bf16(A, lda, B, ldb, C, ldc, M, N, K, rowscale, (hipStream_t)stream);
}

constexpr int SKF_MAX_BLOCKS = 1024;
extern "C" int mh_splitk_fold_blocks(int64_t M) { return (int)(M < SKF_MAX_BLOCKS ? (M < 1 ? 1 : M) : SKF_MAX_BLOCKS); }

template <bool FOLD>
__global__ __launch_bounds__(256) void splitk_reduce4_kernel(const float* __restrict__ ws, bf16* __restrict__ C, int64_t ldc,
                                                             const bf16* R, int64_t ldr, int64_t M, int64_t N, int splitk,
                                                             float alpha, float beta, const bf16* __restrict__ wnorm,
                                                             const bf16* __restrict__ W, int64_t ldw, float* __restrict__ colpart) {
  const int64_t c = ((int64_t)blockIdx.x * 256 + threadIdx.x) * 4;
  if (c >= N) return;
  const int64_t total = M * N;
  float wn[4] = {1.f, 1.f, 1.f, 1.f}, cs[4] = {0.f, 0.f, 0.f, 0.f};
  if constexpr (FOLD) {
    const bf16x4 w4 = *reinterpret_cast<const bf16x4*>(wnorm + c);
#pragma unroll
    for (int e = 0; e < 4; ++e) wn[e] = (float)w4[e];
  }
  const bool use_r = (R != nullptr && beta != 0.f);
  for (int64_t m = blockIdx.y; m < M; m += gridDim.y) {
    f32x4 s = *reinterpret_cast<const f32x4*>(ws + m * N + c);
    if (splitk <= 8) {
      f32x4 p[7];
#pragma unroll
      for (int z = 1; z < 8; ++z)
        if (z < splitk) p[z - 1] = *reinterpret_cast<const f32x4*>(ws + (int64_t)z * total + m * N + c);
#pragma unroll
      for (int z = 1; z < 8; ++z)
        if (z < splitk) {
#pragma unroll
          for (int e = 0; e < 4; ++e) s[e] += p[z - 1][e];
        }
    } else {
      for (int z = 1; z < splitk; ++z) {
        const f32x4 p = *reinterpret_cast<const f32x4*>(ws + (int64_t)z * total + m * N + c);
#pragma unroll
        for (int e = 0; e < 4; ++e) s[e] += p[e];
      }
    }
    float x[4];
#pragma unroll
// ... 100 lines not shown
```

### midi-model_amd/csrc/gemm_pp256.hip

```cpp
#include <limits.h>

#include <type_traits>

#include "common.h"

namespace {

__device__ __attribute__((aligned(16))) char g_zero16[16];

constexpr int QBM = 256, QBN = 256, QBK = 32;
constexpr int OP_BYTES = 256 * 64;
constexpr int STAGE_BYTES = 2 * OP_BYTES;
constexpr int NSTAGE = 4;
constexpr int LDS_BYTES = NSTAGE * STAGE_BYTES;
constexpr int NWAVE = 8;
constexpr int NI = 2;

typedef __attribute__((ext_vector_type(4))) short s16x4_t;

__device__ inline int tswz(int krow) { return (krow & 3) | ((krow >> 1) & 4); }
__device__ inline int xswz(int row) { return (0x1230 >> (((row >> 2) & 3) * 4)) & 3; }

struct StageCtx {
  const bf16* p[NI];
// ... 24 lines not shown
    c.klim[it] = (r < nrows) ? (int)kend - krow : INT_MIN;
  }
}
template <bool TR>
__device__ inline bf16x8 frag(const char* tile, int row0, int fi, int fg) {
  if constexpr (!TR) {
    const int row = row0 + fi;
    return *reinterpret_cast<const bf16x8*>(tile + row * 64 + ((fg ^ xswz(row)) << 4));
  } else {
    typedef __attribute__((ext_vector_type(2))) unsigned int u32x2_t;
    union {
      bf16x8 v;
      u32x2_t h[2];
    } u;
#pragma unroll
    for (int t = 0; t < 2; ++t) {
      const int krow = fg * 8 + t * 4 + (fi >> 2);
      const int off = krow * 512 + (((row0 >> 4) ^ tswz(krow)) << 5) + ((fi & 3) << 3);
      const unsigned addr = (unsigned)(uintptr_t)(__attribute__((address_space(3))) const char*)(tile + off);
      asm volatile("ds_read_b64_tr_b16 %0, %1" : "=v"(u.h[t]) : "v"(addr));
    }
    return u.v;
  }
}

typedef __attribute__((ext_vector_type(4))) unsigned int u32x4;
__device__ inline __amdgpu_buffer_rsrc_t tile_rsrc(const void* base, int64_t bytes) {
  const unsigned n = bytes <= 0 ? 0u : (bytes > 0xfffffff0ll ? 0xfffffff0u : (unsigned)bytes);
  const uint64_t b = (uint64_t)(uintptr_t)base;
  const uint64_t bu = (uint64_t)(unsigned)__builtin_amdgcn_readfirstlane((int)(unsigned)b) |
                      ((uint64_t)(unsigned)__builtin_amdgcn_readfirstlane((int)(unsigned)(b >> 32)) << 32);
  return __builtin_amdgcn_make_buffer_rsrc(reinterpret_cast<void*>((uintptr_t)bu), 0, (unsigned)__builtin_amdgcn_readfirstlane((int)n), 0x00020000);
}
template <int AUX>
__device__ inline void tile_store_(const u32x4& v, __amdgpu_buffer_rsrc_t r, unsigned voff) {
  __builtin_amdgcn_raw_buffer_store_b128(v, r, voff, 0, AUX);
}
#define tile_store(v, r, voff, aux) tile_store_<aux>(v, r, voff)
__device__ inline u32x4 as_u32x4(const bf16x8& v) {
  union {
    bf16x8 b;
    u32x4 u;
  } x;
  x.b = v;
  return x.u;
}
__device__ inline bf16x8 as_bf16x8(const u32x4& v) {
  union {
    bf16x8 b;
    u32x4 u;
  } x;
  x.u = v;
  return x.b;
}

constexpr int P8_REGION = 128 * 128;
constexpr int P8_BUF = 4 * P8_REGION;
constexpr int P8_DBG_BYTES = 8 * 2048;

template <int EPI, int ABL, bool TB>
__device__ __forceinline__ void p8_main_loop(char* smem, const bf16* __restrict__ A, int64_t lda, const bf16* __restrict__ B,
                                             int64_t ldb, int64_t M, int64_t N, int64_t m0, int64_t n0, int64_t kbeg, int64_t kend,
                                             int wave, int lane, const void* __restrict__ zero16, f32x4 (&acc)[4][8]) {
  constexpr bool TL = (ABL & 128) != 0;
  constexpr int LA = 7;
  const int grp = wave >> 2, wn = wave & 3;
  const int fi = lane & 15, fg = lane >> 4;
  const int nt = (kend > kbeg) ? (int)((kend - kbeg + 63) / 64) : 0;
  const int nreg = 4 * nt;

  int tl_n = 0;
  auto stamp = [&]() {
    if constexpr (TL) {
      const uint64_t c = __builtin_readcyclecounter();
      if (lane == 0 && tl_n < 252) *reinterpret_cast<uint64_t*>(smem + 2 * P8_BUF + wave * 2048 + tl_n * 8) = c;
      ++tl_n;
    }
  };
  auto mark = [&](int slot) {
    if constexpr (TL) {
      const uint64_t c = __builtin_readcyclecounter();
      if (lane == 0) *reinterpret_cast<uint64_t*>(smem + 2 * P8_BUF + wave * 2048 + slot * 8) = c;
    }
  };
  mark(252);

  const bf16* pa[2];
  const bf16* pb[2];
  int kla[2][2], klb[2][2];
  const int64_t hoff_a = 64 * lda, hoff_b = TB ? 32 * ldb : (EPI == 2) ? (N / 2) * ldb : 32 * ldb;
#pragma unroll
  for (int it = 0; it < 2; ++it) {
    const int lr = (wave * 2 + it) * 8 + (lane >> 3);
    const int ch = (lane & 7) ^ ((lr >> 1) & 7);
    const int64_t ra = m0 + (lr >> 6) * 128 + (lr & 63);
    pa[it] = A + (ra < M ? ra : 0) * lda + ch * 8;
    kla[0][it] = (ra < M) ? (int)kend - ch * 8 : INT_MIN;
    kla[1][it] = (ra + 64 < M) ? (int)kend - ch * 8 : INT_MIN;
    if constexpr (TB) {
      const int krow = (wave + NWAVE * it) * 2 + (lane >> 5), pc = lane & 31;
      const int lg = (pc >> 1) ^ tswz(krow);
      const int64_t r = n0 + lg * 16 + (pc & 1) * 8;
      pb[it] = B + (int64_t)krow * ldb + (r < N ? r : 0);
      klb[0][it] = (r < N) ? (int)kend - krow : INT_MIN;
      klb[1][it] = (r < N) ? (int)kend - krow - 32 : INT_MIN;
    } else {
// ... 121 lines not shown
  auto tile_g0 = [&](int t, auto steady) {
#pragma unroll
    for (int p = 0; p < 2; ++p) {
      stamp();
      load_slot(t, p, steady);
      bar();
      stamp();
      mfma_phase(p);
      wait_next(2 * t + p, steady);
      bar();
    }
  };
  auto tile_g1 = [&](int t, auto steady) {
#pragma unroll
    for (int p = 0; p < 2; ++p) {
      stamp();
      if (2 * t + p > 0) mfma_phase(p ^ 1);
      else stamp();
      bar();
      stamp();
      load_slot(t, p, steady);
      wait_next(2 * t + p, steady);
      bar();
    }
  };

#pragma unroll
  for (int s = 0; s < LA; ++s)
    if (s < nreg) issue(s);
  if (nt > 0) wait_out((nreg < LA ? nreg : LA) - need(0));
  bar();
  mark(253);
  const int nsteady = nt > 2 ? nt - 2 : 0;
  if (grp == 0) {
    for (int t = 0; t < nsteady; ++t) tile_g0(t, std::true_type{});
    for (int t = nsteady; t < nt; ++t) tile_g0(t, std::false_type{});
  } else {
    for (int t = 0; t < nsteady; ++t) tile_g1(t, std::true_type{});
    for (int t = nsteady; t < nt; ++t) tile_g1(t, std::false_type{});
    if (nt > 0) mfma_phase(1);
  }
  mark(254);
  if constexpr (TL) {
    asm volatile("s_waitcnt lgkmcnt(0)" ::: "memory");
  }
}

template <bool TA, bool TB, int ABL, int EPI, int ML, int NRM>
__global__ __launch_bounds__(512, 2) void gemm_pp256_kernel(const bf16* __restrict__ A, int64_t lda,
                                                            const bf16* __restrict__ B, int64_t ldb, bf16* C, int64_t ldc,
                                                            const bf16* R, int64_t ldr, int64_t M, int64_t N, int64_t K,
                                                            float alpha, float beta, int tiles_n, int nwg,
                                                            int64_t k_per_split, float* __restrict__ ws,
                                                            const void* __restrict__ zero16, float* aux, int lean_epi) {
  static_assert(NRM == 0 || (ML == 1 && ABL == 0 && !TA && (!TB || (EPI == 1 && NRM == 2))), "the norm forms ride on the K-step-64 loops only");
  static_assert(NRM != 1 || EPI == 0, "sum-of-squares partials come out of the plain epilogue");
  extern __shared__ __attribute__((aligned(16))) char smem[];
  const int tid = threadIdx.x, lane = tid & 63;
  const int wave = __builtin_amdgcn_readfirstlane(tid >> 6);
  const int grp = wave >> 2;
  const int wn = wave & 3;

  const int nitems = nwg * (int)gridDim.z;
  const int lin = blockIdx.x + nwg * (int)blockIdx.z;
  const int q = nitems >> 3, r8 = nitems & 7, xcd = lin & 7;
  const int item = (xcd < r8 ? xcd * (q + 1) : r8 * (q + 1) + (xcd - r8) * q) + (lin >> 3);
  const int zslice = item / nwg;
  int tm, tn;
  gemm_tile_of(item - zslice * nwg, nwg / tiles_n, tiles_n, 4, tm, tn);
  const int64_t m0 = (int64_t)tm * QBM, n0 = (int64_t)tn * (EPI == 2 ? 128 : QBN);

  const int64_t kbeg = (int64_t)zslice * k_per_split;
  const int64_t kend = (kbeg + k_per_split < K) ? kbeg + k_per_split : K;

  f32x4 acc[4][8];
#pragma unroll
  for (int a = 0; a < 4; ++a)
#pragma unroll
    for (int b = 0; b < 8; ++b) acc[a][b] = f32x4{0.f, 0.f, 0.f, 0.f};
  const int fi = lane & 15, fg = lane >> 4;
  auto bar = [&]() {
    __builtin_amdgcn_sched_barrier(0);
    __builtin_amdgcn_s_barrier();
    __builtin_amdgcn_sched_barrier(0);
  };

  if constexpr (ML >= 1) {
    if constexpr (NRM == 2) {
      if (wave == 0) {
        const int64_t r = m0 + lane * 4;
        glds16((r + 4 <= M) ? (const void*)(aux + r) : zero16, smem + LDS_BYTES);
      }
    }
    p8_main_loop<EPI, ABL, TB>(smem, A, lda, B, ldb, M, N, m0, n0, kbeg, kend, wave, lane, zero16, acc);
    if constexpr ((ABL & 128) != 0) {
      __syncthreads();
      if (blockIdx.x == 0 && blockIdx.z == 0)
        for (int i = tid; i < P8_DBG_BYTES / 8; i += 512)
          reinterpret_cast<uint64_t*>(ws)[i] = reinterpret_cast<const uint64_t*>(smem + 2 * P8_BUF)[i];
      __syncthreads();
    }
  } else {
  const int nt = (kend > kbeg) ? (int)((kend - kbeg + QBK - 1) / QBK) : 0;
  StageCtx ca, cb;
  if constexpr (TA) stage_init_t(ca, A, lda, m0, M, kend, wave, lane);
  else stage_init_n(ca, A, lda, m0, M, kend, wave, lane, (ABL & 8) != 0);
  if constexpr (TB) stage_init_t(cb, B, ldb, n0, N, kend, wave, lane);
  else stage_init_n(cb, B, ldb, n0, N, kend, wave, lane, (ABL & 8) != 0, EPI == 2 ? N / 2 - 128 : 0);
  auto issue_one = [&](int t, int j) {
    char* buf = smem + (t & (NSTAGE - 1)) * STAGE_BYTES + (j >> 1) * OP_BYTES + (wave + NWAVE * (j & 1)) * 1024;
    const int k0 = (int)kbeg + t * QBK;
    const StageCtx& c = (j >> 1) ? cb : ca;
    const bool tr = (j >> 1) ? TB : TA;
    const int64_t ld = (j >> 1) ? ldb : lda;
    const bf16* p = c.p[j & 1] + (tr ? (int64_t)k0 * ld : (int64_t)k0);
    const void* src = (k0 < c.klim[j & 1]) ? (const void*)p : zero16;
    glds16(src, buf);
  };
#pragma unroll
  for (int s0 = 0; s0 < 3; ++s0)
    if (s0 < nt) {
#pragma unroll
      for (int j = 0; j < 4; ++j) issue_one(s0, j);
    }

  bf16x8 fx[8], fw[4];
  auto load_frags = [&](int t) {
    const char* tA = smem + (t & (NSTAGE - 1)) * STAGE_BYTES;
    const char* tB = tA + OP_BYTES;
    if ((ABL & 2) && t > 0) return;
#pragma unroll
    for (int f = 0; f < 4; ++f)
      fw[f] = frag<TB>(tB, EPI == 2 ? (f >> 1) * 128 + wn * 32 + (f & 1) * 16 : wn * 64 + f * 16, fi, fg);
#pragma unroll
    for (int f = 0; f < 8; ++f) fx[f] = frag<TA>(tA, grp * 128 + f * 16, fi, fg);
  };
  auto mfma_all = [&](int t) {
    __builtin_amdgcn_s_setprio(1);
#pragma unroll
    for (int fn = 0; fn < 4; ++fn) {
#pragma unroll
      for (int fm = 0; fm < 8; ++fm)
        if (!(ABL & 4)) acc[fn][fm] = __builtin_amdgcn_mfma_f32_16x16x32_bf16(fw[fn], fx[fm], acc[fn][fm], 0, 0, 0);
    }
    __builtin_amdgcn_s_setprio(0);
  };
  auto wait_step = [&](int t) {
    if (t + 2 < nt) asm volatile("s_waitcnt vmcnt(8)" ::: "memory");
    else if (t + 1 < nt) asm volatile("s_waitcnt vmcnt(4)" ::: "memory");
    else asm volatile("s_waitcnt vmcnt(0)" ::: "memory");
  };
  auto load_segment = [&](int t) {
    load_frags(t);
    if (t + 3 < nt && !(ABL & 1)) {
#pragma unroll
      for (int j = 0; j < 4; ++j) issue_one(t + 3, j);
    }
    asm volatile("s_waitcnt lgkmcnt(0)" ::: "memory");
    __builtin_amdgcn_sched_barrier(0);
  };
  constexpr bool MIDBAR = ((ABL & 64) != 0) == (TA || TB);
  if (grp == 0) {
    for (int t = 0; t < nt; ++t) {
      wait_step(t);
      bar();
      load_segment(t);
      if (MIDBAR) bar();
      mfma_all(t);
    }
    bar();
  } else {
    for (int t = 0; t < nt; ++t) {
      wait_step(t);
      bar();
      if (t > 0) mfma_all(t - 1);
      if (MIDBAR) bar();
      load_segment(t);
    }
    bar();
    if (nt > 0) mfma_all(nt - 1);
  }
  }

  float rs[8];
  if constexpr (NRM == 2) {
    const float* rl = reinterpret_cast<const float*>(smem + LDS_BYTES);
#pragma unroll
    for (int fm = 0; fm < 8; ++fm) rs[fm] = rl[grp * 128 + fm * 16 + fi];
  }
  const bool partial = (gridDim.z > 1);
  float* wsz = partial ? ws + (int64_t)zslice * M * N : nullptr;
  if constexpr ((ABL & 32) != 0) {
    if (acc[0][0][0] != 1.2345e38f) return;
  }
  if constexpr (EPI == 1) {
    if (lean_epi && m0 + QBM <= M && n0 + QBN <= N && ldc < (1 << 22) && ldr < (1 << 22)) {
      char* wreg = smem + wave * 16384;
      const int lrow = lane >> 3, c = lane & 7;
      const __amdgpu_buffer_rsrc_t rg = tile_rsrc(R + m0 * ldr + n0 + wn * 64, (255 * ldr + N + 64) * 2);
      const __amdgpu_buffer_rsrc_t rc = tile_rsrc(C + m0 * ldc + n0 + wn * 64, (255 * ldc + N + 64) * 2);
      const unsigned vo_r = (unsigned)(((grp * 128 + lrow) * (int)ldr + c * 8) * 2), so_r = (unsigned)ldr * 16u;
      const unsigned vo_c = (unsigned)(((grp * 128 + lrow) * (int)ldc + c * 8) * 2), so_c = (unsigned)ldc * 16u;
      const unsigned up_off = (unsigned)N * 2u;
      bf16x8 gq[2][8], uq[2][8];
      auto request = [&](int half, int i0) {
#pragma unroll
        for (int i = i0; i < i0 + 4; ++i) {
          gq[half][i] = as_bf16x8(__builtin_amdgcn_raw_buffer_load_b128(rg, vo_r, (unsigned)(half * 8 + i) * so_r, 0));
          uq[half][i] = as_bf16x8(__builtin_amdgcn_raw_buffer_load_b128(rg, vo_r, (unsigned)(half * 8 + i) * so_r + up_off, 0));
        }
      };
      request(0, 0);
      request(0, 4);
#pragma unroll
      for (int half = 0; half < 2; ++half) {
#pragma unroll
        for (int fmh = 0; fmh < 4; ++fmh)
#pragma unroll
          for (int fn = 0; fn < 4; ++fn) {
            const int row = fmh * 16 + fi, ch = fn * 4 + fg;
            f32x4 t4 = acc[fn][half * 4 + fmh];
            if constexpr (NRM == 2) t4 *= rs[half * 4 + fmh];
            *reinterpret_cast<f32x4*>(wreg + row * 256 + ((ch ^ (row & 15)) << 4)) = t4;
          }
#pragma unroll
        for (int i = 0; i < 8; ++i) {
          if (half == 0 && (i == 2 || i == 6)) request(1, i == 2 ? 0 : 4);
          const int row = i * 8 + lrow;
          const f32x4 lo = *reinterpret_cast<const f32x4*>(wreg + row * 256 + (((2 * c) ^ (row & 15)) << 4));
          const f32x4 hi = *reinterpret_cast<const f32x4*>(wreg + row * 256 + (((2 * c + 1) ^ (row & 15)) << 4));
          const float v[8] = {lo[0], lo[1], lo[2], lo[3], hi[0], hi[1], hi[2], hi[3]};
          float dv[8], g[8], u[8], dg[8], du[8];
          expand8_bf16(cvt8_bf16(v), dv);
          expand8_bf16(gq[half][i], g);
          expand8_bf16(uq[half][i], u);
          mh_dswiglu8(dv, g, u, dg, du);
          const unsigned so = (unsigned)(half * 8 + i) * so_c;
          tile_store(as_u32x4(cvt8_bf16(dg)), rc, vo_c + so, 2 );
          tile_store(as_u32x4(cvt8_bf16(du)), rc, vo_c + so + up_off, 2);
        }
      }
      return;
    }
    char* wreg = smem + wave * 16384;
    const int lrow = lane >> 3, c = lane & 7;
    const int64_t n = n0 + wn * 64 + c * 8;
    const bool n_ok = (n + 8 <= N);
    bf16x8 gq[2][8], uq[2][8];
    auto request = [&](int half) {
#pragma unroll
      for (int i = 0; i < 8; ++i) {
        const int64_t m = m0 + grp * 128 + half * 64 + i * 8 + lrow;
        if (m < M && n_ok) {
          gq[half][i] = *reinterpret_cast<const bf16x8*>(R + m * ldr + n);
          uq[half][i] = *reinterpret_cast<const bf16x8*>(R + m * ldr + N + n);
        }
      }
    };
    request(0);
#pragma unroll
    for (int half = 0; half < 2; ++half) {
      const bf16x8 (&gv)[8] = gq[half];
      const bf16x8 (&uv)[8] = uq[half];
#pragma unroll
      for (int fmh = 0; fmh < 4; ++fmh)
#pragma unroll
        for (int fn = 0; fn < 4; ++fn) {
          const int row = fmh * 16 + fi, ch = fn * 4 + fg;
          f32x4 t4 = acc[fn][half * 4 + fmh];
          if constexpr (NRM == 2) t4 *= rs[half * 4 + fmh];
          *reinterpret_cast<f32x4*>(wreg + row * 256 + ((ch ^ (row & 15)) << 4)) = t4;
        }
      if (half == 0) request(1);
#pragma unroll
      for (int i = 0; i < 8; ++i) {
        const int row = i * 8 + lrow;
        const f32x4 lo = *reinterpret_cast<const f32x4*>(wreg + row * 256 + (((2 * c) ^ (row & 15)) << 4));
        const f32x4 hi = *reinterpret_cast<const f32x4*>(wreg + row * 256 + (((2 * c + 1) ^ (row & 15)) << 4));
        const int64_t m = m0 + grp * 128 + half * 64 + row;
        if (m >= M || !n_ok) continue;
        const float v[8] = {lo[0], lo[1], lo[2], lo[3], hi[0], hi[1], hi[2], hi[3]};
        float dv[8], g[8], u[8], dg[8], du[8];
        expand8_bf16(cvt8_bf16(v), dv);
        expand8_bf16(gv[i], g);
        expand8_bf16(uv[i], u);
#pragma unroll
        for (int e = 0; e < 8; ++e) {
          const float sig = mh_sigmoid(g[e]);
          const float silu = g[e] * sig;
          dg[e] = dv[e] * u[e] * (sig * (1.f + g[e] * (1.f - sig)));
          du[e] = dv[e] * silu;
        }
        const bf16x8 og = cvt8_bf16(dg), ou = cvt8_bf16(du);
        __builtin_nontemporal_store(og, reinterpret_cast<bf16x8*>(C + m * ldc + n));
        __builtin_nontemporal_store(ou, reinterpret_cast<bf16x8*>(C + m * ldc + N + n));
      }
    }
    return;
  }
  if constexpr (EPI == 2 && ML == 1) {
    char* wreg = smem + wave * 16384;
    const int64_t I = N >> 1, colw = n0 + wn * 32;
    bf16* act = const_cast<bf16*>(R);
    const int64_t rows_left = (M - m0 < QBM) ? M - m0 : QBM;
    const __amdgpu_buffer_rsrc_t ra = tile_rsrc(act + m0 * ldr + colw, ((rows_left - 1) * ldr + 32) * 2);
    const __amdgpu_buffer_rsrc_t rc = tile_rsrc(C != nullptr ? C + m0 * ldc + colw : nullptr, C != nullptr ? ((rows_left - 1) * ldc + I + 32) * 2 : 0);
    const int r4 = lane >> 2, c4 = lane & 3;
    const unsigned vo_a = (unsigned)(((grp * 128 + r4) * (int)ldr + c4 * 8) * 2), so_a = (unsigned)ldr * 32u;
    const unsigned vo_c = (unsigned)(((grp * 128 + r4) * (int)ldc + c4 * 8) * 2), so_c = (unsigned)ldc * 32u;
    const bool keep = (C != nullptr);
#pragma unroll
    for (int half = 0; half < 2; ++half) {
#pragma unroll
      for (int fmh = 0; fmh < 4; ++fmh) {
        const int fm = half * 4 + fmh;
        float gf[8], uf[8];
#pragma unroll
        for (int e = 0; e < 4; ++e) {
          gf[e] = acc[0][fm][e];
          gf[4 + e] = acc[1][fm][e];
          uf[e] = acc[2][fm][e];
          uf[4 + e] = acc[3][fm][e];
        }
        if constexpr (NRM == 2) {
#pragma unroll
          for (int e = 0; e < 8; ++e) {
            gf[e] *= rs[fm];
            uf[e] *= rs[fm];
          }
        }
        const bf16x8 og = cvt8_bf16(gf), ou = cvt8_bf16(uf);
        float gr[8], ur[8], sv[8], sr[8], av[8];
        expand8_bf16(og, gr);
        expand8_bf16(ou, ur);
        mh_silu8(gr, sv);
        expand8_bf16(cvt8_bf16(sv), sr);
#pragma unroll
        for (int e = 0; e < 8; ++e) av[e] = sr[e] * ur[e];
        const bf16x8 oa = cvt8_bf16(av);
        const int row = fmh * 16 + fi, off = row * 64 + ((fg ^ ((row >> 1) & 3)) << 4);
        *reinterpret_cast<u32x4*>(wreg + off) = as_u32x4(oa);
        if (keep) {
          *reinterpret_cast<u32x4*>(wreg + 4096 + off) = as_u32x4(og);
          *reinterpret_cast<u32x4*>(wreg + 8192 + off) = as_u32x4(ou);
        }
      }
#pragma unroll
      for (int i = 0; i < 4; ++i) {
// ... 140 lines not shown
    bf16x8 cq[2][8], sq[2][8];
    auto request = [&](int half) {
      if (rot) {
#pragma unroll
        for (int i = 0; i < 8; ++i) {
          const int64_t m = m0 + grp * 128 + half * 64 + i * 8 + lrow;
          const int64_t pos = pos0 + (m < M ? m : M - 1) % S_;
          cq[half][i] = *reinterpret_cast<const bf16x8*>(tab + pos * 96 + fo);
          sq[half][i] = *reinterpret_cast<const bf16x8*>(tab + pos * 96 + so);
        }
      }
    };
    request(0);
#pragma unroll
    for (int half = 0; half < 2; ++half) {
      const bf16x8 (&cv)[8] = cq[half];
      const bf16x8 (&sv)[8] = sq[half];
#pragma unroll
      for (int fmh = 0; fmh < 4; ++fmh)
#pragma unroll
        for (int fn = 0; fn < 4; ++fn) {
          const int row = fmh * 16 + fi, ch = fn * 4 + fg;
          f32x4 a4 = acc[fn][half * 4 + fmh];
          if constexpr (NRM == 2) a4 *= rs[half * 4 + fmh];
          const bf16x2 lo = __builtin_convertvector(f32x2{a4[0], a4[1]}, bf16x2), hi2 = __builtin_convertvector(f32x2{a4[2], a4[3]}, bf16x2);
          f32x4 r4;
          r4[0] = (float)lo[0];
          r4[1] = (float)lo[1];
          r4[2] = (float)hi2[0];
          r4[3] = (float)hi2[1];
          *reinterpret_cast<f32x4*>(wreg + row * 256 + ((ch ^ (row & 15)) << 4)) = r4;
        }
      if (half == 0) request(1);
#pragma unroll
      for (int i = 0; i < 8; ++i) {
        const int row = i * 8 + lrow;
        const f32x4 lo = *reinterpret_cast<const f32x4*>(wreg + row * 256 + (((2 * c) ^ (row & 15)) << 4));
        const f32x4 hi = *reinterpret_cast<const f32x4*>(wreg + row * 256 + (((2 * c + 1) ^ (row & 15)) << 4));
        const int64_t m = m0 + grp * 128 + half * 64 + row;
        float v[8] = {lo[0], lo[1], lo[2], lo[3], hi[0], hi[1], hi[2], hi[3]};
        if (rot) {
          const int pc = c ^ 4;
          const f32x4 plo = *reinterpret_cast<const f32x4*>(wreg + row * 256 + (((2 * pc) ^ (row & 15)) << 4));
          const f32x4 phi = *reinterpret_cast<const f32x4*>(wreg + row * 256 + (((2 * pc + 1) ^ (row & 15)) << 4));
          const float pv[8] = {plo[0], plo[1], plo[2], plo[3], phi[0], phi[1], phi[2], phi[3]};
          float cf[8], sf[8];
          expand8_bf16(cv[i], cf);
          expand8_bf16(sv[i], sf);
#pragma unroll
          for (int e = 0; e < 8; ++e) v[e] = __builtin_fmaf(v[e], cf[e], pv[e] * sf[e]);
        }
        if (m >= M || n + 8 > N) continue;
        __builtin_nontemporal_store(cvt8_bf16(v), reinterpret_cast<bf16x8*>(C + m * ldc + n));
      }
    }
    return;
  }
  const bool use_r = (R != nullptr && beta != 0.f);
  const bool line_ok = !partial && (ldc & 7) == 0 && ((uintptr_t)C & 15) == 0 &&
                       (!use_r || ((ldr & 7) == 0 && ((uintptr_t)R & 15) == 0));
  if (lean_epi && line_ok && m0 + QBM <= M && n0 + QBN <= N && ldc < (1 << 22) && ldr < (1 << 22)) {
    char* wreg = smem + wave * 16384;
    const int lrow = lane >> 3, c = lane & 7;
    const __amdgpu_buffer_rsrc_t rc = tile_rsrc(C + m0 * ldc + n0 + wn * 64, (255 * ldc + 64) * 2);
    const __amdgpu_buffer_rsrc_t rr = tile_rsrc(use_r ? R + m0 * ldr + n0 + wn * 64 : nullptr, use_r ? (255 * ldr + 64) * 2 : 0);
    const unsigned vo_c = (unsigned)(((grp * 128 + lrow) * (int)ldc + c * 8) * 2), so_c = (unsigned)ldc * 16u;
    const unsigned vo_r = (unsigned)(((grp * 128 + lrow) * (int)ldr + c * 8) * 2), so_r = (unsigned)ldr * 16u;
    float* auxp = nullptr;
    if constexpr (NRM == 1) auxp = aux + ((n0 + wn * 64) >> 6) * M + m0 + grp * 128 + lrow;
    auto turn = [&](auto with_r) {
    constexpr bool use_r = decltype(with_r)::value;
    bf16x8 rv[2][8];
    if (use_r) {
#pragma unroll
      for (int half = 0; half < 2; ++half)
#pragma unroll
        for (int i = 0; i < 8; ++i)
          rv[half][i] = as_bf16x8(__builtin_amdgcn_raw_buffer_load_b128(rr, vo_r, (unsigned)(half * 8 + i) * so_r, 0));
    }
#pragma unroll
    for (int half = 0; half < 2; ++half) {
#pragma unroll
      for (int fmh = 0; fmh < 4; ++fmh)
#pragma unroll
        for (int fn = 0; fn < 4; ++fn) {
          const int row = fmh * 16 + fi, ch = fn * 4 + fg;
          f32x4 t4 = acc[fn][half * 4 + fmh];
          if constexpr (NRM == 2) t4 *= rs[half * 4 + fmh];
          *reinterpret_cast<f32x4*>(wreg + row * 256 + ((ch ^ (row & 15)) << 4)) = t4;
        }
#pragma unroll
      for (int i = 0; i < 8; ++i) {
        const int row = i * 8 + lrow;
        const f32x4 lo = *reinterpret_cast<const f32x4*>(wreg + row * 256 + (((2 * c) ^ (row & 15)) << 4));
        const f32x4 hi = *reinterpret_cast<const f32x4*>(wreg + row * 256 + (((2 * c + 1) ^ (row & 15)) << 4));
        float v[8] = {lo[0], lo[1], lo[2], lo[3], hi[0], hi[1], hi[2], hi[3]};
        if (use_r) {
#pragma unroll
          for (int e = 0; e < 8; ++e) v[e] = alpha * v[e] + beta * (float)rv[half][i][e];
        } else {
#pragma unroll
          for (int e = 0; e < 8; ++e) v[e] = alpha * v[e];
        }
        bf16x8 o;
#pragma unroll
        for (int e = 0; e < 8; ++e) o[e] = (bf16)v[e];
// ... 92 lines not shown
  }
  const bool vec_ok = partial ? ((N & 3) == 0)
                              : ((ldc & 3) == 0 && ((uintptr_t)C & 15) == 0 &&
                                 (R == nullptr || ((ldr & 3) == 0 && ((uintptr_t)R & 15) == 0)));
#pragma unroll
  for (int fm = 0; fm < 8; ++fm) {
    const int64_t m = m0 + grp * 128 + fm * 16 + fi;
    if (m >= M) continue;
#pragma unroll
    for (int fn = 0; fn < 4; ++fn) {
      const int64_t n = n0 + wn * 64 + fn * 16 + fg * 4;
      if (n >= N) continue;
      f32x4 v = acc[fn][fm];
      if constexpr (NRM == 2) v *= rs[fm];
      if (partial) {
        float* dst = wsz + m * N + n;
        if (vec_ok && n + 3 < N) {
          *reinterpret_cast<f32x4*>(dst) = v;
        } else {
          for (int e = 0; e < 4 && n + e < N; ++e) dst[e] = v[e];
        }
        continue;
      }
      if (vec_ok && n + 3 < N) {
        if (R != nullptr && beta != 0.f) {
          bf16x4 rv = *reinterpret_cast<const bf16x4*>(R + m * ldr + n);
#pragma unroll
          for (int e = 0; e < 4; ++e) v[e] = alpha * v[e] + beta * (float)rv[e];
        } else {
#pragma unroll
          for (int e = 0; e < 4; ++e) v[e] = alpha * v[e];
        }
        bf16x4 o;
#pragma unroll
        for (int e = 0; e < 4; ++e) o[e] = (bf16)v[e];
        *reinterpret_cast<bf16x4*>(C + m * ldc + n) = o;
      } else {
        for (int e = 0; e < 4 && n + e < N; ++e) {
          float x = alpha * v[e];
          if (R != nullptr && beta != 0.f) x += beta * (float)R[m * ldr + n + e];
          C[m * ldc + n + e] = (bf16)x;
        }
      }
    }
  }
}

}
extern thread_local int g_mh_gemm_lean_epi;
namespace {
template <bool TA, bool TB, int ABL, int EPI = 0, int ML = 0, int NRM = 0>
int launch_one(const void* A, int64_t lda, const void* B, int64_t ldb, void* C, int64_t ldc, const void* R, int64_t ldr,
               int64_t M, int64_t N, int64_t K, float alpha, float beta, int splitk, void* workspace, hipStream_t st,
               float* aux = nullptr) {
  constexpr int LDSB = LDS_BYTES + ((ABL & 128) ? P8_DBG_BYTES : 0) + (NRM == 2 ? 1024 : 0);
  constexpr int MAX_DEV = 64;
  static void* zero16_of[MAX_DEV] = {};
  static bool attr_set_of[MAX_DEV] = {};
  int dev = 0;
  if (hipGetDevice(&dev) != hipSuccess || dev < 0 || dev >= MAX_DEV) {
    mh_set_error("gemm_pp256: no current device (or ordinal %d beyond %d)", dev, MAX_DEV - 1);
    return MH_ERR_LAUNCH;
  }
  void* zero16 = __atomic_load_n(&zero16_of[dev], __ATOMIC_ACQUIRE);
  if (zero16 == nullptr) {
    if (hipGetSymbolAddress(&zero16, HIP_SYMBOL(g_zero16)) != hipSuccess) {
      mh_set_error("gemm_pp256: hipGetSymbolAddress(g_zero16) failed");
      return MH_ERR_LAUNCH;
    }
    __atomic_store_n(&zero16_of[dev], zero16, __ATOMIC_RELEASE);
  }
  if (!__atomic_load_n(&attr_set_of[dev], __ATOMIC_ACQUIRE)) {
    hipError_t e = hipFuncSetAttribute(reinterpret_cast<const void*>(&gemm_pp256_kernel<TA, TB, ABL, EPI, ML, NRM>),
                                       hipFuncAttributeMaxDynamicSharedMemorySize, LDSB);
    if (e != hipSuccess) {
      mh_set_error("gemm_pp256: cannot raise dynamic LDS to %d bytes: %s", LDSB, hipGetErrorString(e));
      return MH_ERR_LAUNCH;
    }
    __atomic_store_n(&attr_set_of[dev], true, __ATOMIC_RELEASE);
  }
  const int64_t tiles_m = (M + QBM - 1) / QBM, tiles_n = (EPI == 2) ? N / 256 : (N + QBN - 1) / QBN;
  const int nwg = (int)(tiles_m * tiles_n);
  constexpr int KSTEP = (ML == 1) ? 64 : QBK;
  const int64_t kps = ((K + splitk - 1) / splitk + KSTEP - 1) / KSTEP * KSTEP;
  dim3 grid(nwg, 1, splitk);
  gemm_pp256_kernel<TA, TB, ABL, EPI, ML, NRM><<<grid, 512, LDSB, st>>>((const bf16*)A, lda, (const bf16*)B, ldb, (bf16*)C, ldc,
                                                          (const bf16*)R, ldr, M, N, K, alpha, beta, (int)tiles_n, nwg, kps,
                                                          (float*)workspace, zero16, aux, g_mh_gemm_lean_epi);
  MH_LAUNCH_CHECK();
  return MH_OK;
}

}

extern thread_local int g_mh_gemm_ablate;
extern thread_local int g_mh_gemm_k64;

int mh_gemm_pp256_bf16(const void* A, int64_t lda, int ta, const void* B, int64_t ldb, int tb, void* C, int64_t ldc,
                       const void* R, int64_t ldr, int64_t M, int64_t N, int64_t K, float alpha, float beta, int splitk,
                       void* workspace, hipStream_t st) {
#define MH_PP(TA_, TB_, ABL_) \
  return launch_one<TA_, TB_, ABL_>(A, lda, B, ldb, C, ldc, R, ldr, M, N, K, alpha, beta, splitk, workspace, st)
#ifndef MH_AB_BUILDS
  MH_REQUIRE(g_mh_gemm_ablate == 0, "gemm: option gemm_ablate = %d selects a micro-benchmark build, which is only in the A/B test "
             "library (libmidihip_ab.so)", g_mh_gemm_ablate);
#else
  MH_REQUIRE(g_mh_gemm_ablate != 128 || (workspace != nullptr && splitk == 1), "gemm_ablate 128 (timeline) needs a workspace and splitk 1");
  MH_REQUIRE(!(g_mh_gemm_k64 && !ta && !tb) || g_mh_gemm_ablate == 0 || g_mh_gemm_ablate == 1 || g_mh_gemm_ablate == 4 ||
                 g_mh_gemm_ablate == 128 || g_mh_gemm_ablate == 64,
             "gemm_ablate %d is not built for the K-step-64 main loop (set gemm_k64 = 0 for the K-step-32 ablations)", g_mh_gemm_ablate);
  if (ta == tb && g_mh_gemm_ablate && !(g_mh_gemm_k64 && !ta)) {
#define MH_AB(X_) \
  case X_:        \
    if (ta) MH_PP(true, true, X_); \
    MH_PP(false, false, X_);
    switch (g_mh_gemm_ablate) { MH_AB(1) MH_AB(3) MH_AB(4) MH_AB(5) MH_AB(8) MH_AB(12) MH_AB(32) default: break; }
#undef MH_AB
  }
  if (g_mh_gemm_ablate == 64) {
    if (ta && tb) MH_PP(true, true, 64);
    if (ta) MH_PP(true, false, 64);
    if (tb) MH_PP(false, true, 64);
    MH_PP(false, false, 64);
  }
#endif
  if (ta && tb) MH_PP(true, true, 0);
  if (ta) MH_PP(true, false, 0);
  if (tb && g_mh_gemm_k64 == 1)
    return launch_one<false, true, 0, 0, 1>(A, lda, B, ldb, C, ldc, R, ldr, M, N, K, alpha, beta, splitk, workspace, st);
  if (tb) MH_PP(false, true, 0);
  if (g_mh_gemm_k64) {
#define MH_P8(ABL_) \
  return launch_one<false, false, ABL_, 0, 1>(A, lda, B, ldb, C, ldc, R, ldr, M, N, K, alpha, beta, splitk, workspace, st)
#ifdef MH_AB_BUILDS
    switch (g_mh_gemm_ablate) {
      case 1: MH_P8(1);
      case 4: MH_P8(4);
      case 128: MH_P8(128);
      default: break;
    }
#endif
    MH_P8(0);
#undef MH_P8
  }
  MH_PP(false, false, 0);
#undef MH_PP
}

int mh_gemm_pp256_swiglu_bf16(const void* A, int64_t lda, const void* W, int64_t ldw, void* GU, int64_t ldgu, void* ACT,
                              int64_t ldact, int64_t M, int64_t I, int64_t K, hipStream_t st, const float* rowscale) {
  MH_REQUIRE(ldgu < (1 << 22) && ldact < (1 << 22), "gemm_swiglu: row strides beyond 2^22 elements are not supported (32-bit tile offsets)");
  if (rowscale != nullptr) {
    MH_REQUIRE(g_mh_gemm_k64 != 0 && M % 4 == 0, "gemm_swiglu: the row-scaled form needs the K-step-64 main loop and M %% 4 == 0");
    return launch_one<false, false, 0, 2, 1, 2>(A, lda, W, ldw, GU, ldgu, ACT, ldact, M, 2 * I, K, 1.f, 0.f, 1, nullptr, st,
                                                const_cast<float*>(rowscale));
  }
  if (g_mh_gemm_k64) return launch_one<false, false, 0, 2, 1>(A, lda, W, ldw, GU, ldgu, ACT, ldact, M, 2 * I, K, 1.f, 0.f, 1, nullptr, st);
  return launch_one<false, false, 0, 2>(A, lda, W, ldw, GU, ldgu, ACT, ldact, M, 2 * I, K, 1.f, 0.f, 1, nullptr, st);
}

int mh_gemm_pp256_rope_bf16(const void* A, int64_t lda, const void* W, int64_t ldw, void* C, int64_t ldc, const void* table,
                            int64_t S, int64_t pos0, int64_t M, int64_t N, int64_t K, hipStream_t st, const float* rowscale) {
  MH_REQUIRE(ldc < (1 << 22) && M < (int64_t(1) << 31) - 256, "gemm_rope: row stride beyond 2^22 elements / more than 2^31 rows are not supported (32-bit tile offsets and positions)");
  if (rowscale != nullptr) {
    MH_REQUIRE(g_mh_gemm_k64 != 0 && M % 4 == 0, "gemm_rope: the row-scaled form needs the K-step-64 main loop and M %% 4 == 0");
    return launch_one<false, false, 0, 3, 1, 2>(A, lda, W, ldw, C, ldc, table, S | (pos0 << 32), M, N, K, 1.f, 0.f, 1, nullptr, st,
                                                const_cast<float*>(rowscale));
  }
  if (g_mh_gemm_k64) return launch_one<false, false, 0, 3, 1>(A, lda, W, ldw, C, ldc, table, S | (pos0 << 32), M, N, K, 1.f, 0.f, 1, nullptr, st);
  return launch_one<false, false, 0, 3>(A, lda, W, ldw, C, ldc, table, S | (pos0 << 32), M, N, K, 1.f, 0.f, 1, nullptr, st);
}

int mh_gemm_pp256_scaled_bf16(const void* A, int64_t lda, const void* B, int64_t ldb, void* C, int64_t ldc, int64_t M, int64_t N,
                              int64_t K, const float* rowscale, hipStream_t st) {
  MH_REQUIRE(g_mh_gemm_k64 != 0 && M % 4 == 0, "gemm_nt_scaled: needs the K-step-64 main loop and M %% 4 == 0");
  return launch_one<false, false, 0, 0, 1, 2>(A, lda, B, ldb, C, ldc, nullptr, 0, M, N, K, 1.f, 0.f, 1, nullptr, st,
                                              const_cast<float*>(rowscale));
}

int mh_gemm_pp256_dswiglu_bf16(const void* A, int64_t lda, const void* B, int64_t ldb, const void* GU, int64_t ldgu,
                               void* DGU, int64_t lddgu, int64_t M, int64_t I, int64_t K, hipStream_t st, const float* rowscale) {
  if (rowscale != nullptr) {
    MH_REQUIRE(g_mh_gemm_k64 == 1 && M % 4 == 0, "gemm_dswiglu_scaled: needs the K-step-64 dgrad loop and M %% 4 == 0");
    return launch_one<false, true, 0, 1, 1, 2>(A, lda, B, ldb, DGU, lddgu, GU, ldgu, M, I, K, 1.f, 0.f, 1, nullptr, st,
                                               const_cast<float*>(rowscale));
  }
  if (g_mh_gemm_k64 == 1) return launch_one<false, true, 0, 1, 1>(A, lda, B, ldb, DGU, lddgu, GU, ldgu, M, I, K, 1.f, 0.f, 1, nullptr, st);
  return launch_one<false, true, 0, 1>(A, lda, B, ldb, DGU, lddgu, GU, ldgu, M, I, K, 1.f, 0.f, 1, nullptr, st);
}

int mh_gemm_pp256_rowss_bf16(const void* A, int64_t lda, const void* B, int64_t ldb, void* C, int64_t ldc, const void* R,
                             int64_t ldr, int64_t M, int64_t N, int64_t K, float* rowss, hipStream_t st) {
  MH_REQUIRE(g_mh_gemm_k64 != 0, "gemm_rowss: needs the K-step-64 main loop (option gemm_k64)");
  return launch_one<false, false, 0, 0, 1, 1>(A, lda, B, ldb, C, ldc, R, ldr, M, N, K, 1.f, R ? 1.f : 0.f, 1, nullptr, st, rowss);
}
```

### midi-model_amd/engine.py

```python
from __future__ import annotations

import math
from dataclasses import dataclass, field
from typing import Callable, List, NamedTuple, Optional

import os

import torch

from . import ops


@dataclass
class StackSpec:
    name: str
    D: int
    H: int
    I: int
    L: int
    eps: float
    theta: float
    kind: str

    @property
    def hd(self) -> int:
        return self.D // self.H

    @property
    def scale(self) -> float:
        return self.hd ** -0.5


@dataclass
class LayerTensors:
    wqkv: torch.Tensor = None
    wo: torch.Tensor = None
    wgu: torch.Tensor = None
    wd: torch.Tensor = None
    n1: torch.Tensor = None
    n2: torch.Tensor = None


@dataclass
class StackTensors:
    embed: torch.Tensor = None
    layers: List[LayerTensors] = field(default_factory=list)
    norm: torch.Tensor = None


class RopeTable:

    def __init__(self, hd: int, theta: float, device, npos: int = 0):
        self.hd, self.theta, self.device = hd, theta, device
        self.cos = self.sin = None
        self._fused = None
        self.n = 0
        if npos:
            self.ensure(npos)

    def ensure(self, npos: int):
        if npos <= self.n:
            return
        npos = max(npos, 2 * self.n, 64)
# ... 112 lines not shown

FOLD_MIN_ROWS_PREFOLDED = 8192
FOLD_MIN_ROWS_ON_THE_FLY = 131072


def layer_forward_folded(spec: StackSpec, lw: LayerTensors, fold, x: torch.Tensor, nseq: int, slen: int, rope: RopeTable,
                         parts_in: Optional[torch.Tensor], kv_out: Optional[list] = None, saved_out: Optional[list] = None,
                         lean: bool = False):
    M, D = x.shape
    H, I = spec.H, spec.I
    save = saved_out is not None
    wq_n, wgu_n = fold
    rstd1 = _empty((M,), x, torch.float32)
    if parts_in is not None:
        ops.row_rstd(rstd1, D, spec.eps, parts=parts_in)
    else:
        ops.row_rstd(rstd1, D, spec.eps, x=x)
    qkv = _empty((M, 3 * D), x)
    o = _empty((M, D), x)
    lse = None
    if spec.kind == "event":
        ops.gemm_rope(x, wq_n, qkv, rope.fused(), slen, 0, spec.hd, rowscale=rstd1)
        lse = _empty((nseq * H * ops.round_up(slen, 64),), x, torch.float32)
        ops.attn_fwd(qkv, o, lse, nseq, slen, H, spec.scale)
    else:
        ops.gemm_nt_scaled(x, wq_n, qkv, rstd1)
        ops.tokattn_fwd(qkv, o, nseq, slen, H, spec.scale, rope.cos, rope.sin)
    if kv_out is not None:
        kv_out.append(qkv)
    parts = _empty((D // 64, M), x, torch.float32)
    x2 = _empty((M, D), x)
    ops.gemm_rowss(o, lw.wo, x2, parts, res=x)
    rstd2 = _empty((M,), x, torch.float32) if save else rstd1
    ops.row_rstd(rstd2, D, spec.eps, parts=parts)
    gu = _empty((M, 2 * I), x) if save else None
    a = _empty((M, I), x)
    ops.gemm_swiglu(x2, wgu_n, gu, a, rowscale=rstd2)
    parts3 = _empty((D // 64, M), x, torch.float32) if save else parts
    x3 = _empty((M, D), x)
    ops.gemm_rowss(a, lw.wd, x3, parts3, res=x2)
    if save:
        saved_out.append(LayerSaved(x, rstd1, None, qkv, o, lse, x2, rstd2, None, gu, None if lean else a))
    return x3, parts3


def train_fold_ok(spec: StackSpec, x: torch.Tensor) -> bool:
    ok = (x.dtype == torch.bfloat16 and ops.swiglu_fused_ok(x, spec.I) and ops.dswiglu_ok(x, spec.I) and spec.D % 64 == 0
          and x.shape[0] % 4 == 0 and ops.get_option("gemm_k64") == 1 and os.environ.get("MH_NORM_FOLD_TRAIN", "1") != "0")
    if ok and spec.kind == "event":
        ok = ops.rope_fused_ok(x, spec.hd) and ops.attn_bwd_scaled_ok(x)
    return ok


def runs_folded(spec: StackSpec, x: torch.Tensor, save: bool, kv_out: Optional[list], fold_kept: bool) -> bool:
    if save:
        return fold_kept and kv_out is None and train_fold_ok(spec, x)
    return (spec.kind == "event" and x.shape[0] >= (FOLD_MIN_ROWS_PREFOLDED if fold_kept else FOLD_MIN_ROWS_ON_THE_FLY)
            and ops.norm_fold_ok(x, spec.D, spec.hd, spec.I))


def layer_backward(spec: StackSpec, lw: LayerTensors, lg: LayerTensors, keep: LayerSaved, dx: torch.Tensor, nseq: int, slen: int,
                   rope: RopeTable, accumulate: bool) -> torch.Tensor:
    M, D = dx.shape
    H, I = spec.H, spec.I
    a = keep.a
    if a is None:
        a = _empty((M, I), dx)
        ops.swiglu_fwd(keep.gu, a)
    dgu = _empty((M, 2 * I), dx)
    if ops.dswiglu_ok(dx, I):
        ops.gemm_dswiglu(dx, lw.wd, keep.gu, dgu)
    else:
        da = _empty((M, I), dx)
        ops.gemm_nt(dx, lw.wd, da, tb=True)
        ops.swiglu_bwd(keep.gu, da, dgu)
        del da
    linear_wgrad(dx, a, lg.wd, accumulate)
    del a
    dh2 = _empty((M, D), dx)
    ops.gemm_nt(dgu, lw.wgu, dh2, tb=True)
    linear_wgrad(dgu, keep.h2, lg.wgu, accumulate)
    del dgu
    dx2 = _empty((M, D), dx)
    ops.rmsnorm_bwd(keep.x2, lw.n2, keep.rstd2, dh2, dx, dx2, lg.n2, accumulate)
    do = dh2
    ops.gemm_nt(dx2, lw.wo, do, tb=True)
    linear_wgrad(dx2, keep.o, lg.wo, accumulate)
    dqkv = _empty((M, 3 * D), dx)
    if spec.kind == "event":
        ops.attn_bwd(keep.qkv, keep.o, do, keep.lse, dqkv, nseq, slen, H, spec.scale, rope.cos, rope.sin)
    else:
        ops.tokattn_bwd(keep.qkv, do, dqkv, nseq, slen, H, spec.scale, rope.cos, rope.sin)
    dh1 = do
    ops.gemm_nt(dqkv, lw.wqkv, dh1, tb=True)
    linear_wgrad(dqkv, keep.h1, lg.wqkv, accumulate)
    del dqkv
    ops.rmsnorm_bwd(keep.x, lw.n1, keep.rstd1, dh1, dx2, dx, lg.n1, accumulate)
    return dx


def layer_backward_folded(spec: StackSpec, lw: LayerTensors, lg: LayerTensors, fold, keep: LayerSaved, dx: torch.Tensor, nseq: int,
                          slen: int, rope: RopeTable, accumulate: bool) -> torch.Tensor:
    M, D = dx.shape
    H, I = spec.H, spec.I
    wq_n, wgu_n = fold
    a = keep.a
    if a is None:
        a = _empty((M, I), dx)
        ops.swiglu_fwd(keep.gu, a)
    dz2 = _empty((M, 2 * I), dx)
    ops.gemm_dswiglu(dx, lw.wd, keep.gu, dz2, rowscale=keep.rstd2)
    linear_wgrad(dx, a, lg.wd, accumulate)
    del a
    t2 = _empty((M, D), dx)
    ops.gemm_nt(dz2, wgu_n, t2, tb=True)
    ops.wgrad_folded(dz2, keep.x2, lg.wgu, lw.n2, lw.wgu, lg.n2, accumulate)
    del dz2
    dx2 = _empty((M, D), dx)
    ops.rmsnorm_bwd_folded(keep.x2, keep.rstd2, t2, dx, dx2)
    do = t2
    ops.gemm_nt(dx2, lw.wo, do, tb=True)
    linear_wgrad(dx2, keep.o, lg.wo, accumulate)
    dz1 = _empty((M, 3 * D), dx)
    if spec.kind == "event":
        ops.attn_bwd(keep.qkv, keep.o, do, keep.lse, dz1, nseq, slen, H, spec.scale, rope.cos, rope.sin, rowscale=keep.rstd1)
    else:
        ops.tokattn_bwd(keep.qkv, do, dz1, nseq, slen, H, spec.scale, rope.cos, rope.sin, rowscale=keep.rstd1)
    t1 = do
    ops.gemm_nt(dz1, wq_n, t1, tb=True)
    ops.wgrad_folded(dz1, keep.x, lg.wqkv, lw.n1, lw.wqkv, lg.n1, accumulate)
    del dz1
    ops.rmsnorm_bwd_folded(keep.x, keep.rstd1, t1, dx2, dx)
    return dx


def stack_forward(spec: StackSpec, W: StackTensors, x: torch.Tensor, nseq: int, slen: int, rope: RopeTable,
                  save: bool, kv_out: Optional[list] = None, lean: bool = False, folded=None):
    _check_heads(spec)
    M, D = x.shape
    assert M == nseq * slen
    rope.ensure(slen)
    if runs_folded(spec, x, save, kv_out, folded is not None):
        if folded is None:
            folded = fold_norm_weights(W)
    else:
        folded = None
    saved = [] if save else None
    parts = None
    for li, lw in enumerate(W.layers):
        if folded is not None:
            x, parts = layer_forward_folded(spec, lw, folded[li], x, nseq, slen, rope, parts, kv_out, saved, lean)
        else:
            x, keep = layer_forward(spec, lw, x, nseq, slen, rope, kv_out, save, lean and save)
            if save:
                saved.append(keep)
    y = _empty((M, D), x)
    rstdf = _empty((M,), x, torch.float32) if save or folded is None else None
    ops.rmsnorm_fwd(x, W.norm, y, rstdf, spec.eps)
    return y, (StackSaved(saved, x, rstdf, nseq, slen, folded) if save else None)


def stack_backward(spec: StackSpec, W: StackTensors, G: StackTensors, ctx: StackSaved, dy: torch.Tensor,
                   rope: RopeTable, accumulate: bool, on_layer_done: Optional[Callable[[int], None]] = None):
    M, D = dy.shape
    dx = _empty((M, D), dy)
    ops.rmsnorm_bwd(ctx.x_last, W.norm, ctx.rstdf, dy, None, dx, G.norm, accumulate)
    for li in range(len(W.layers) - 1, -1, -1):
        lw, lg = W.layers[li], G.layers[li]
        if ctx.folded is not None:
            dx = layer_backward_folded(spec, lw, lg, ctx.folded[li], ctx.layers[li], dx, ctx.nseq, ctx.slen, rope, accumulate)
        else:
            dx = layer_backward(spec, lw, lg, ctx.layers[li], dx, ctx.nseq, ctx.slen, rope, accumulate)
        ctx.layers[li] = None
        if on_layer_done is not None:
            on_layer_done(li)
    return dx
# ... 155 lines not shown
```

### midi-model_amd/ops.py

```python
from __future__ import annotations

from typing import Optional

import os
import threading

import torch

from .lib import MH_BF16, MH_F32, lib

_DT = {torch.float32: MH_F32, torch.bfloat16: MH_BF16}


def dt(t: torch.Tensor) -> int:
    try:
        return _DT[t.dtype]
    except KeyError:
        raise TypeError(f"unsupported dtype {t.dtype}: the HIP path computes in float32 or bfloat16") from None


def _stream() -> int:
    return torch.cuda.current_stream().cuda_stream


# ... 162 lines not shown
              rowscale: Optional[torch.Tensor] = None):
    M, K = x.shape
    N = wqkv.shape[0]
    assert qkv.shape == (M, N) and wqkv.shape[1] == K and table.dtype == torch.bfloat16 and table.shape[1] == 96
    prof = gemm_profile
    if prof is not None:
        e0, e1 = torch.cuda.Event(enable_timing=True), torch.cuda.Event(enable_timing=True)
        e0.record()
    if rowscale is not None:
        assert rowscale.shape == (M,) and rowscale.dtype == torch.float32 and rowscale.is_contiguous()
        lib().call("mh_gemm_rope_scaled", _p(x), _rowmajor(x), _p(wqkv), _rowmajor(wqkv), _p(qkv), _rowmajor(qkv), _p(table),
                   table.shape[0], S, pos0, hd, _p(rowscale), M, N, K, dt(x), _stream())
    else:
        lib().call("mh_gemm_rope", _p(x), _rowmajor(x), _p(wqkv), _rowmajor(wqkv), _p(qkv), _rowmajor(qkv), _p(table),
                   table.shape[0], S, pos0, hd, M, N, K, dt(x), _stream())
    if prof is not None:
        e1.record()
        prof.append((e0, e1, 2.0 * M * N * K, (M, N, K, 1, 0, 0, "+rope")))
    return qkv


def swiglu_fused_ok(x: torch.Tensor, I: int) -> bool:
    return x.dtype == torch.bfloat16 and I % 128 == 0 and get_option("gemm") != 0 and (_FUSE & 1) != 0


def gemm_swiglu(x: torch.Tensor, wgu: torch.Tensor, gu: Optional[torch.Tensor], a: torch.Tensor,
                rowscale: Optional[torch.Tensor] = None) -> torch.Tensor:
    M, K = x.shape
    I = a.shape[1]
    assert wgu.shape == (2 * I, K) and a.shape[0] == M and x.dtype == wgu.dtype == a.dtype
    assert gu is None or (gu.shape == (M, 2 * I) and gu.dtype == x.dtype)
    prof = gemm_profile
    if prof is not None:
        e0, e1 = torch.cuda.Event(enable_timing=True), torch.cuda.Event(enable_timing=True)
        e0.record()
    if rowscale is not None:
        assert rowscale.shape == (M,) and rowscale.dtype == torch.float32 and rowscale.is_contiguous()
        lib().call("mh_gemm_swiglu_scaled", _p(x), _rowmajor(x), _p(wgu), _rowmajor(wgu), _p(gu), _rowmajor(gu) if gu is not None else 0,
                   _p(a), _rowmajor(a), _p(rowscale), M, I, K, dt(x), _stream())
    else:
        lib().call("mh_gemm_swiglu", _p(x), _rowmajor(x), _p(wgu), _rowmajor(wgu), _p(gu), _rowmajor(gu) if gu is not None else 0,
                   _p(a), _rowmajor(a), M, I, K, dt(x), _stream())
    if prof is not None:
        e1.record()
        prof.append((e0, e1, 2.0 * M * 2 * I * K, (M, 2 * I, K, 1, 0, 0, "+swiglu")))
    return a


def dswiglu_ok(dx: torch.Tensor, I: int) -> bool:
    return dx.dtype == torch.bfloat16 and I % 8 == 0 and get_option("gemm") != 0 and (_FUSE & 2) != 0


def gemm_dswiglu(dx: torch.Tensor, wd: torch.Tensor, gu: torch.Tensor, dgu: torch.Tensor,
                 rowscale: Optional[torch.Tensor] = None) -> torch.Tensor:
    M, K = dx.shape
    I = wd.shape[1]
    assert wd.shape[0] == K and gu.shape == (M, 2 * I) and dgu.shape == (M, 2 * I) and dx.dtype == wd.dtype == gu.dtype
    prof = gemm_profile
    if prof is not None:
        e0, e1 = torch.cuda.Event(enable_timing=True), torch.cuda.Event(enable_timing=True)
        e0.record()
    if rowscale is not None:
        assert rowscale.shape == (M,) and rowscale.dtype == torch.float32 and rowscale.is_contiguous()
        lib().call("mh_gemm_dswiglu_scaled", _p(dx), _rowmajor(dx), _p(wd), _rowmajor(wd), _p(gu), _rowmajor(gu), _p(dgu),
                   _rowmajor(dgu), _p(rowscale), M, I, K, dt(dx), _stream())
    else:
        lib().call("mh_gemm_dswiglu", _p(dx), _rowmajor(dx), _p(wd), _rowmajor(wd), _p(gu), _rowmajor(gu), _p(dgu), _rowmajor(dgu),
                   M, I, K, dt(dx), _stream())
    if prof is not None:
        e1.record()
        prof.append((e0, e1, 2.0 * M * I * K, (M, I, K, 1, 0, 1, "+dswiglu")))
    return dgu


SKINNY_PLAIN, SKINNY_GATEUP = 0, 1


def gemm_skinny(a: torch.Tensor, w: torch.Tensor, out: torch.Tensor, *, mode: int = SKINNY_PLAIN,
                res: Optional[torch.Tensor] = None, norm_eps: float = 0.0, row_ids: Optional[torch.Tensor] = None,
                res_ids: Optional[torch.Tensor] = None) -> torch.Tensor:
    M, N = out.shape
    K = w.shape[1]
    assert a.shape[1] == K and (row_ids is not None or a.shape[0] == M), (a.shape, out.shape)
    assert w.shape[0] == (2 * N if mode == SKINNY_GATEUP else N), (a.shape, w.shape, out.shape, mode)
    for t in (row_ids, res_ids):
        assert t is None or (t.dtype == torch.int64 and t.is_contiguous() and t.numel() == M)
    assert a.shape[0] * _rowmajor(a) < 2 ** 31 and (res is None or res.shape[0] * _rowmajor(res) < 2 ** 31), "gemm_skinny: table too large"
    lib().call("mh_gemm_skinny", _p(a), _rowmajor(a), _p(w), _rowmajor(w), _p(out), _rowmajor(out), _p(res),
               _rowmajor(res) if res is not None else 0, mode, norm_eps, _p(row_ids), _p(res_ids), M, N, K, dt(out),
               _stream())
    return out


def skinny_ok(x: torch.Tensor, K: int) -> bool:
    return x.dtype == torch.bfloat16 and x.shape[0] <= 64 and K % 256 == 0


gemm_profile = None


def transpose(x: torch.Tensor, out: Optional[torch.Tensor] = None, pad_to: int = 8) -> torch.Tensor:
    R, C = x.shape
    if out is None:
        Rp = round_up(R, pad_to)
        out = torch.empty((C, Rp), dtype=x.dtype, device=x.device)
        if Rp != R:
            out[:, R:].zero_()
    lib().call("mh_transpose", _p(x), _rowmajor(x), _p(out), _rowmajor(out), R, C, dt(x), _stream())
    return out


def collate_windows(tokens_i16: torch.Tensor, win_start: torch.Tensor, win_len: torch.Tensor, out: torch.Tensor, pad_id: int):
    B, L, T = out.shape
    assert tokens_i16.dtype == torch.int16 and tokens_i16.is_contiguous() and tokens_i16.shape[1] == T
    assert win_start.dtype == torch.int64 and win_len.dtype == torch.int64 and out.dtype == torch.int64 and out.is_contiguous()
# ... 162 lines not shown

def rope_(qkv: torch.Tensor, cos_t: torch.Tensor, sin_t: torch.Tensor, S: int, pos0: int, H: int, hd: int, direction: int = 1):
    M = qkv.shape[0]
    assert qkv.is_contiguous() and qkv.shape[1] == 3 * H * hd
    assert cos_t.shape[0] >= pos0 + min(S, M), "RoPE table too short"
    lib().call("mh_rope", _p(qkv), _p(cos_t), _p(sin_t), M, S, pos0, H, hd, direction, dt(qkv), _stream())
    return qkv


def attn_fwd(qkv, o, lse, B: int, S: int, H: int, scale: float):
    vt = None
    if qkv.dtype == torch.bfloat16 and (_attn_v3() & 17) != 17:
        Sp = round_up(S, 64)
        vt = torch.empty((B * H * 64 * Sp,), dtype=qkv.dtype, device=qkv.device)
        lib().call("mh_attn_prep_fwd", _p(qkv), _p(vt), B, S, H, dt(qkv), _stream())
    lib().call("mh_attn_fwd", _p(qkv), _p(vt), _p(o), _p(lse), B, S, H, scale, dt(qkv), _stream())
    return o


def attn_bwd_scaled_ok(qkv: torch.Tensor) -> bool:
    return qkv.dtype == torch.bfloat16 and (_attn_v3() & 46) == 46


def attn_bwd(qkv, o, dout, lse, dqkv, B: int, S: int, H: int, scale: float, cos_t=None, sin_t=None, rowscale=None):
    Sp = round_up(S, 64)
    v3 = _attn_v3()
    fused = qkv.dtype == torch.bfloat16 and (v3 & 14) == 14 and (v3 & 32) != 0
    delta = torch.empty(((2 if fused else 1) * B * H * Sp,), dtype=torch.float32, device=qkv.device)
    if rowscale is not None:
        assert fused and rowscale.shape == (B * S,) and rowscale.dtype == torch.float32 and rowscale.is_contiguous()
        lib().call("mh_attn_bwd_o_scaled", _p(qkv), _p(o), _p(dout), _p(lse), _p(delta), _p(dqkv), _p(rowscale), B, S, H, scale,
                   _p(cos_t), _p(sin_t), dt(qkv), _stream())
        return dqkv
    if fused:
        lib().call("mh_attn_bwd_o", _p(qkv), _p(o), _p(dout), _p(lse), _p(delta), _p(dqkv), B, S, H, scale, _p(cos_t), _p(sin_t),
                   dt(qkv), _stream())
        return dqkv
    qt = kt = dot = None
    if qkv.dtype == torch.bfloat16 and (v3 & 14) != 14:
        n = B * H * 64 * Sp
        buf = torch.empty((3, n), dtype=qkv.dtype, device=qkv.device)
        qt, kt, dot = buf[0], buf[1], buf[2]
    lib().call("mh_attn_prep_bwd", _p(qkv), _p(o), _p(dout), _p(delta), _p(qt), _p(kt), _p(dot), B, S, H, dt(qkv), _stream())
    lib().call("mh_attn_bwd", _p(qkv), _p(dout), _p(lse), _p(delta), _p(qt), _p(kt), _p(dot), _p(dqkv), B, S, H, scale,
               _p(cos_t), _p(sin_t), dt(qkv), _stream())
    return dqkv


def tokattn_fwd(qkv, o, N: int, T: int, H: int, scale: float, cos_t=None, sin_t=None):
    lib().call("mh_tokattn_fwd", _p(qkv), _p(o), N, T, H, scale, _p(cos_t), _p(sin_t), dt(qkv), _stream())
    return o


def tokattn_bwd(qkv, dout, dqkv, N: int, T: int, H: int, scale: float, cos_t=None, sin_t=None, rowscale=None):
    if rowscale is not None:
        assert rowscale.shape == (N * T,) and rowscale.dtype == torch.float32 and rowscale.is_contiguous()
        lib().call("mh_tokattn_bwd_scaled", _p(qkv), _p(dout), _p(dqkv), _p(rowscale), N, T, H, scale, _p(cos_t), _p(sin_t),
                   dt(qkv), _stream())
        return dqkv
    lib().call("mh_tokattn_bwd", _p(qkv), _p(dout), _p(dqkv), N, T, H, scale, _p(cos_t), _p(sin_t), dt(qkv), _stream())
    return dqkv


def swiglu_fwd(gu, a):
    M, I2 = gu.shape
    lib().call("mh_swiglu_fwd", _p(gu), _p(a), M, I2 // 2, dt(gu), _stream())
    return a


def swiglu_bwd(gu, da, dgu):
    M, I2 = gu.shape
    lib().call("mh_swiglu_bwd", _p(gu), _p(da), _p(dgu), M, I2 // 2, dt(gu), _stream())
    return dgu


def cross_entropy(logits, V: int, target, row_loss, dlogits=None, scale_dev=None, argmax_out=None, ignore: int = 0):
    R = logits.shape[0]
    lib().call("mh_cross_entropy", _p(logits), _rowmajor(logits), _p(target), _p(row_loss), _p(dlogits), _p(scale_dev),
               _p(argmax_out), R, V, ignore, dt(logits), _stream())


def sum_f32(x, out):
    lib().call("mh_sum_f32", _p(x), x.numel(), _p(out), _stream())


def count_valid(target, ignore: int, count, inv):
    lib().call("mh_count_valid", _p(target), target.numel(), ignore, _p(count), _p(inv), _stream())


def sumsq(g, partial1024, out, accumulate: bool):
    lib().call("mh_sumsq", _p(g), g.numel(), _p(partial1024), _p(out), int(accumulate), dt(g), _stream())


def clip_coef(sumsq_t, max_norm: float, coef, norm):
    lib().call("mh_clip_coef", _p(sumsq_t), max_norm, _p(coef), _p(norm), _stream())


def adamw(p, g, m, v, lr, b1, b2, eps, wd, bc1, bc2, coef_dev):
    lib().call("mh_adamw", _p(p), _p(g), _p(m), _p(v), p.numel(), lr, b1, b2, eps, wd, bc1, bc2, _p(coef_dev), dt(p), _stream())


def kv_append(qkv, cos_t, sin_t, kc, vc, B: int, H: int, hd: int, Lmax: int, pos: int, pos_dev=None):
    lib().call("mh_kv_append", _p(qkv), _p(cos_t), _p(sin_t), _p(kc), _p(vc), B, H, hd, Lmax, pos, _p(pos_dev), dt(qkv),
               _stream())


def attn_decode(qkv, kc, vc, o, B: int, H: int, hd: int, Lmax: int, length: int, scale: float, pos_dev=None):
# ... 67 lines not shown
```

Baseline: 362,400 events/s.

## Fuse RMSNorm backward into dgrad GEMM epilogue via row-dot partials

Computes the RMSNorm-backward row-dot partials inside the dswiglu GEMM and the token-attention backward kernel. A small kernel turns those partials into per-row coefficients, and a new dgrad GEMM epilogue applies the norm backward and the residual add directly. This removes the separate rmsnorm_bwd_folded pass and the intermediate t2/dx round trip for token stacks, and for event stacks on the MLP path only when the env var is set to 2. The costs are extra partial buffers, one extra coefficient launch, and heavier GEMM and attention epilogues. The attention rowscale is also passed explicitly instead of through a thread-local global.

```diff
diff --git a/include/midihip.h b/include/midihip.h
--- a/include/midihip.h
+++ b/include/midihip.h
@@ -44,6 +44,11 @@
                       int64_t N, int64_t K, int dtype, void* stream);
 int mh_gemm_dswiglu_scaled(const void* A, int64_t lda, const void* B, int64_t ldb, const void* GU, int64_t ldgu, void* DGU,
                            int64_t lddgu, const float* rowscale, int64_t M, int64_t I, int64_t K, int dtype, void* stream);
+int mh_gemm_dswiglu_parts(const void* A, int64_t lda, const void* B, int64_t ldb, const void* GU, int64_t ldgu, void* DGU,
+                          int64_t lddgu, const float* rowscale, float* parts, int64_t M, int64_t I, int64_t K, int dtype, void* stream);
+int mh_row_coef(const float* parts, int nparts, const float* rstd, int64_t M, int D, float* coef, void* stream);
+int mh_gemm_dgrad_normbwd(const void* A, int64_t lda, const void* B, int64_t ldb, void* C, int64_t ldc, const void* R, int64_t ldr,
+                          const void* X, int64_t ldx, const float* coef, int64_t M, int64_t N, int64_t K, int dtype, void* stream);
 int mh_splitk_fold_blocks(int64_t M);
 int mh_gemm_splitk_reduce_fold(const void* workspace, void* C, int64_t ldc, const void* R, int64_t ldr, int64_t M, int64_t N,
                                int splitk, float alpha, float beta, const void* wnorm, const void* W, int64_t ldw, float* colpart,
@@ -123,6 +128,8 @@
                    const float* sin_t, int dtype, void* stream);
 int mh_tokattn_bwd_scaled(const void* qkv, const void* dout, void* dqkv, const float* rowscale, int64_t N, int T, int H, float scale,
                           const float* cos_t, const float* sin_t, int dtype, void* stream);
+int mh_tokattn_bwd_parts(const void* qkv, const void* dout, void* dqkv, const float* rowscale, float* parts, int64_t N, int T, int H,
+                         float scale, const float* cos_t, const float* sin_t, int dtype, void* stream);
 
 int mh_swiglu_fwd(const void* gu, void* a, int64_t M, int I, int dtype, void* stream);
 int mh_swiglu_bwd(const void* gu, const void* da, void* dgu, int64_t M, int I, int dtype, void* stream);
diff --git a/midi-model_amd/csrc/attention_mfma.hip b/midi-model_amd/csrc/attention_mfma.hip
--- a/midi-model_amd/csrc/attention_mfma.hip
+++ b/midi-model_amd/csrc/attention_mfma.hip
@@ -367,7 +367,7 @@
                       hipStream_t st, int64_t q_start = 0);
 int mh_attn_bwd_mfma3(const void* qkv, const void* dout, const float* lse, const float* delta, const void* qt, const void* kt,
                       const void* dot, void* dqkv, int64_t B, int64_t S, int H, float scale, const float* cos_t,
-                      const float* sin_t, int which, hipStream_t st, const void* o = nullptr);
+                      const float* sin_t, int which, hipStream_t st, const void* o = nullptr, const float* rowscale = nullptr);
 
 int mh_attn_fwd_mfma(const void* qkv, const void* vt, void* o, float* lse, int64_t B, int64_t S, int H, float scale,
                      hipStream_t st, int64_t q_start) {
@@ -391,11 +391,12 @@
 }
 
 int mh_attn_bwd_o_mfma(const void* qkv, const void* o, const void* dout, const float* lse, float* delta, void* dqkv, int64_t B,
-                       int64_t S, int H, float scale, const float* cos_t, const float* sin_t, hipStream_t st) {
+                       int64_t S, int H, float scale, const float* cos_t, const float* sin_t, hipStream_t st,
+                       const float* rowscale ) {
   MH_REQUIRE(S < (1 << 24), "attn_bwd: sequence too long");
   MH_REQUIRE((g_attn_v3 & 14) == 14, "attn_bwd_o: served by the third form with transpose reads (mh_set_option(\"attn_v3\") bits 2|4|8); "
              "use mh_attn_prep_bwd + mh_attn_bwd otherwise");
-  return mh_attn_bwd_mfma3(qkv, dout, lse, delta, nullptr, nullptr, nullptr, dqkv, B, S, H, scale, cos_t, sin_t, 14, st, o);
+  return mh_attn_bwd_mfma3(qkv, dout, lse, delta, nullptr, nullptr, nullptr, dqkv, B, S, H, scale, cos_t, sin_t, 14, st, o, rowscale);
 }
 
 int mh_attn_bwd_mfma(const void* qkv, const void* dout, const float* lse, const float* delta, const void* qt,
diff --git a/midi-model_amd/csrc/attention_mfma3.hip b/midi-model_amd/csrc/attention_mfma3.hip
--- a/midi-model_amd/csrc/attention_mfma3.hip
+++ b/midi-model_amd/csrc/attention_mfma3.hip
@@ -9,7 +9,6 @@
 thread_local int g_attn_v3 = attn_env_int("MH_ATTN_V3", 255);
 thread_local int g_attn_passes = attn_env_int("MH_ATTN_PASSES", 5);
 thread_local int g_attn_v3_wps = attn_env_int("MH_ATTN_V3_WPS", 0);
-thread_local const float* g_attn_bwd_rowscale = nullptr;
 
 __device__ inline bf16x8 ldsv(const char* p) { return *reinterpret_cast<const bf16x8*>(p); }
 typedef __attribute__((ext_vector_type(2))) float f32x2;
@@ -859,7 +858,8 @@
 int mh_attn_bwd_mfma3(const void* qkv, const void* dout, const float* lse, const float* delta, const void* qt, const void* kt,
                       const void* dot, void* dqkv, int64_t B, int64_t S, int H, float scale, const float* cos_t,
                       const float* sin_t, int which ,
-                      hipStream_t st, const void* o ) {
+                      hipStream_t st, const void* o ,
+                      const float* rowscale ) {
   MH_REQUIRE(o == nullptr || (which & 14) == 14, "attn_bwd: delta inside the dQ kernel needs the third form of both kernels");
   MH_REQUIRE(S * 3 * H * HD < (int64_t(1) << 31), "attn_bwd: sequence too long (32-bit panel offsets)");
   const bool tr = (which & 8) != 0;
@@ -873,7 +873,7 @@
   attn_bwd_dq3_kernel<WPS, TR_><<<grid, 256, (TR_ ? 4 : 6) * TILE64, st>>>((const bf16*)qkv, (const bf16*)dout, lse, delta,     \
                                                                         (const bf16*)kt, (bf16*)dqkv, (int)S, (int)Sp, H, scale, \
                                                                         BH, nt, cos_t, sin_t, (const bf16*)o,         \
-                                                                        const_cast<float*>(delta), g_attn_bwd_rowscale)
+                                                                        const_cast<float*>(delta), rowscale)
   if (which & 2) {
     if (g_attn_v3_wps == 2) {
       if (tr) MH_DQ(2, true); else MH_DQ(2, false);
@@ -888,15 +888,15 @@
       attn_bwd_dkv3_kernel<true, true><<<grid, 256, 2 * (2 * TILE64 + 2048), st>>>((const bf16*)qkv, (const bf16*)dout,
                                                                                  delta + (int64_t)BH0 * Sp, delta, nullptr, nullptr,
                                                                                  (bf16*)dqkv, (int)S, (int)Sp, H, scale, BH, nt,
-                                                                                 cos_t, sin_t, g_attn_bwd_rowscale);
+                                                                                 cos_t, sin_t, rowscale);
     else if (tr)
       attn_bwd_dkv3_kernel<true><<<grid, 256, 2 * (2 * TILE64 + 2048), st>>>((const bf16*)qkv, (const bf16*)dout, lse, delta, nullptr,
                                                                            nullptr, (bf16*)dqkv, (int)S, (int)Sp, H, scale, BH, nt,
-                                                                           cos_t, sin_t, g_attn_bwd_rowscale);
+                                                                           cos_t, sin_t, rowscale);
     else
       attn_bwd_dkv3_kernel<false><<<grid, 256, 2 * DKV_STAGE, st>>>((const bf16*)qkv, (const bf16*)dout, lse, delta, (const bf16*)qt,
                                                                   (const bf16*)dot, (bf16*)dqkv, (int)S, (int)Sp, H, scale, BH, nt,
-                                                                  cos_t, sin_t, g_attn_bwd_rowscale);
+                                                                  cos_t, sin_t, rowscale);
     MH_LAUNCH_CHECK();
   }
   return MH_OK;
diff --git a/midi-model_amd/csrc/attention_small.hip b/midi-model_amd/csrc/attention_small.hip
--- a/midi-model_amd/csrc/attention_small.hip
+++ b/midi-model_amd/csrc/attention_small.hip
@@ -166,7 +166,8 @@
 __global__ __launch_bounds__(256) void tokattn_bwd_kernel(const T* __restrict__ qkv, const T* __restrict__ dout,
                                                           T* __restrict__ dqkv, int64_t NH, int Tn, int H, float scale,
                                                           const float* __restrict__ cos_t, const float* __restrict__ sin_t,
-                                                          const float* __restrict__ rowscale ) {
+                                                          const float* __restrict__ rowscale ,
+                                                          float* __restrict__ parts ) {
   const int lane = threadIdx.x & 63;
   const int64_t D = (int64_t)H * 256, D3 = 3 * D;
   __shared__ float rope_c[TK * 128], rope_s[TK * 128];
@@ -185,6 +186,10 @@
     const T* base = qkv + n * Tn * D3 + off;
     T* ob = dqkv + n * Tn * D3 + off;
     float k[TK][4], v[TK][4], dk[TK][4], dv[TK][4];
+    auto uni = [](float x) { return __int_as_float(__builtin_amdgcn_readfirstlane(__float_as_int(x))); };
+    float rd[TK];
+#pragma unroll
+    for (int t = 0; t < TK; ++t) rd[t] = 0.f;
     RawRow<T> qraw[TN ? TN : 1], doraw[TN ? TN : 1];
     const float rs_lane = (rowscale != nullptr && lane < Tn) ? rowscale[n * Tn + lane] : 1.f;
 #pragma unroll
@@ -262,6 +267,11 @@
         mx = fmaxf(mx, p[j]);
       }
       }
+      float ssc[TK];
+      if (parts != nullptr) {
+#pragma unroll
+        for (int j = 0; j <= i; ++j) ssc[j] = uni(p[j]);
+      }
       float den = 0.f;
 #pragma unroll
       for (int j = 0; j <= i; ++j) {
@@ -274,6 +284,16 @@
       for (int j = 0; j <= i; ++j) {
         p[j] *= inv;
         dsum += p[j] * dp[j];
+      }
+      if (parts != nullptr) {
+        float dqq = 0.f;
+#pragma unroll
+        for (int j = 0; j <= i; ++j) {
+          const float u = p[j] * (dp[j] - dsum) * ssc[j];
+          dqq += u;
+          if (j < i) rd[j] = uni(rd[j] + (u + p[j] * dp[j]));
+          else rd[i] = uni(rd[i] + (dqq + (u + p[j] * dp[j])));
+        }
       }
 #pragma unroll
       for (int j = 0; j <= i; ++j) {
@@ -308,6 +328,12 @@
         stp<T>(ob + t * D3 + D, lane, dk[t]);
         stp<T>(ob + t * D3 + 2 * D, lane, dv[t]);
       }
+    }
+    if (parts != nullptr) {
+      static_assert(TK == 8, "the select below covers eight rows");
+      const float lo = (lane & 2) ? ((lane & 1) ? rd[3] : rd[2]) : ((lane & 1) ? rd[1] : rd[0]);
+      const float hi = (lane & 2) ? ((lane & 1) ? rd[7] : rd[6]) : ((lane & 1) ? rd[5] : rd[4]);
+      if (lane < Tn) parts[(int64_t)h * (NH / H) * Tn + n * Tn + lane] = rs_lane * ((lane & 4) ? hi : lo);
     }
   }
 }
@@ -329,32 +355,38 @@
 }
 
 thread_local int g_tokattn_bwd_batched = 1;
-static int tokattn_bwd_any(const void* qkv, const void* dout, void* dqkv, const float* rowscale, int64_t N, int Tn, int H, float scale,
-                           const float* cos_t, const float* sin_t, int dtype, void* stream) {
+static int tokattn_bwd_any(const void* qkv, const void* dout, void* dqkv, const float* rowscale, float* parts, int64_t N, int Tn, int H,
+                           float scale, const float* cos_t, const float* sin_t, int dtype, void* stream) {
   MH_REQUIRE(N > 0 && Tn >= 1 && Tn <= TK && H >= 1, "tokattn_bwd: bad shape");
+  MH_REQUIRE(parts == nullptr || rowscale != nullptr, "tokattn_bwd: the row-dot partials come with the row-scaled form");
   const int64_t NH = N * H;
   int64_t g = (NH + 3) / 4;
   if (g > 32768) g = 32768;
   if (Tn == TK && g_tokattn_bwd_batched)
     DISPATCH_T(dtype, (tokattn_bwd_kernel<T, TK, true><<<(int)g, 256, 0, (hipStream_t)stream>>>(
-                          (const T*)qkv, (const T*)dout, (T*)dqkv, NH, Tn, H, scale, cos_t, sin_t, rowscale)));
+                          (const T*)qkv, (const T*)dout, (T*)dqkv, NH, Tn, H, scale, cos_t, sin_t, rowscale, parts)));
   else if (Tn == TK)
     DISPATCH_T(dtype, (tokattn_bwd_kernel<T, TK, false><<<(int)g, 256, 0, (hipStream_t)stream>>>(
-                          (const T*)qkv, (const T*)dout, (T*)dqkv, NH, Tn, H, scale, cos_t, sin_t, rowscale)));
+                          (const T*)qkv, (const T*)dout, (T*)dqkv, NH, Tn, H, scale, cos_t, sin_t, rowscale, parts)));
   else
     DISPATCH_T(dtype, (tokattn_bwd_kernel<T, 0, false><<<(int)g, 256, 0, (hipStream_t)stream>>>(
-                          (const T*)qkv, (const T*)dout, (T*)dqkv, NH, Tn, H, scale, cos_t, sin_t, rowscale)));
+                          (const T*)qkv, (const T*)dout, (T*)dqkv, NH, Tn, H, scale, cos_t, sin_t, rowscale, parts)));
   MH_LAUNCH_CHECK();
   return MH_OK;
 }
 extern "C" int mh_tokattn_bwd(const void* qkv, const void* dout, void* dqkv, int64_t N, int Tn, int H, float scale,
                               const float* cos_t, const float* sin_t, int dtype, void* stream) {
-  return tokattn_bwd_any(qkv, dout, dqkv, nullptr, N, Tn, H, scale, cos_t, sin_t, dtype, stream);
+  return tokattn_bwd_any(qkv, dout, dqkv, nullptr, nullptr, N, Tn, H, scale, cos_t, sin_t, dtype, stream);
 }
 extern "C" int mh_tokattn_bwd_scaled(const void* qkv, const void* dout, void* dqkv, const float* rowscale, int64_t N, int Tn, int H,
                                      float scale, const float* cos_t, const float* sin_t, int dtype, void* stream) {
   MH_REQUIRE(rowscale != nullptr, "tokattn_bwd_scaled: rowscale is NULL");
-  return tokattn_bwd_any(qkv, dout, dqkv, rowscale, N, Tn, H, scale, cos_t, sin_t, dtype, stream);
+  return tokattn_bwd_any(qkv, dout, dqkv, rowscale, nullptr, N, Tn, H, scale, cos_t, sin_t, dtype, stream);
+}
+extern "C" int mh_tokattn_bwd_parts(const void* qkv, const void* dout, void* dqkv, const float* rowscale, float* parts, int64_t N, int Tn,
+                                    int H, float scale, const float* cos_t, const float* sin_t, int dtype, void* stream) {
+  MH_REQUIRE(rowscale != nullptr && parts != nullptr, "tokattn_bwd_parts: rowscale or parts is NULL");
+  return tokattn_bwd_any(qkv, dout, dqkv, rowscale, parts, N, Tn, H, scale, cos_t, sin_t, dtype, stream);
 }
 
 template <typename T>
@@ -978,7 +1010,7 @@
                      const float* cos_t, const float* sin_t, hipStream_t st);
 
 int mh_attn_bwd_o_mfma(const void* qkv, const void* o, const void* dout, const float* lse, float* delta, void* dqkv, int64_t B,
-                       int64_t S, int H, float scale, const float* cos_t, const float* sin_t, hipStream_t st);
+                       int64_t S, int H, float scale, const float* cos_t, const float* sin_t, hipStream_t st, const float* rowscale);
 
 template <typename T>
 static int attn_plain_fwd(const void* qkv, void* o, float* lse, int64_t B, int64_t S, int H, float scale, hipStream_t st,
@@ -1050,17 +1082,16 @@
   return MH_ERR_ARG;
 }
 
-extern thread_local const float* g_attn_bwd_rowscale;
 extern thread_local int g_attn_v3;
 extern "C" int mh_attn_bwd_o_scaled(const void* qkv, const void* o, const void* dout, const float* lse, float* delta, void* dqkv,
                                     const float* rowscale, int64_t B, int64_t S, int H, float scale, const float* cos_t,
                                     const float* sin_t, int dtype, void* stream) {
   MH_REQUIRE(rowscale != nullptr, "attn_bwd_o_scaled: rowscale is NULL");
   MH_REQUIRE((g_attn_v3 & 46) == 46, "attn_bwd_o_scaled: needs the third form of the backward kernels (attn_v3 bits 1, 2, 3, 5)");
-  g_attn_bwd_rowscale = rowscale;
-  const int rc = mh_attn_bwd_o(qkv, o, dout, lse, delta, dqkv, B, S, H, scale, cos_t, sin_t, dtype, stream);
-  g_attn_bwd_rowscale = nullptr;
-  return rc;
+  MH_REQUIRE(B > 0 && S > 0 && H > 0 && B * H < 65536, "attn_bwd_o_scaled: bad shape");
+  MH_REQUIRE((cos_t == nullptr) == (sin_t == nullptr), "attn_bwd_o_scaled: cos and sin tables come together");
+  MH_REQUIRE(dtype == MH_BF16, "attn_bwd_o_scaled: bf16 only");
+  return mh_attn_bwd_o_mfma(qkv, o, dout, lse, delta, dqkv, B, S, H, scale, cos_t, sin_t, (hipStream_t)stream, rowscale);
 }
 
 extern "C" int mh_attn_bwd_o(const void* qkv, const void* o, const void* dout, const float* lse, float* delta, void* dqkv,
@@ -1069,5 +1100,5 @@
   MH_REQUIRE(B > 0 && S > 0 && H > 0 && B * H < 65536, "attn_bwd_o: bad shape");
   MH_REQUIRE((cos_t == nullptr) == (sin_t == nullptr), "attn_bwd_o: cos and sin tables come together");
   MH_REQUIRE(dtype == MH_BF16, "attn_bwd_o: bf16 only (fp32: mh_attn_prep_bwd + mh_attn_bwd)");
-  return mh_attn_bwd_o_mfma(qkv, o, dout, lse, delta, dqkv, B, S, H, scale, cos_t, sin_t, (hipStream_t)stream);
-}
+  return mh_attn_bwd_o_mfma(qkv, o, dout, lse, delta, dqkv, B, S, H, scale, cos_t, sin_t, (hipStream_t)stream, nullptr);
+}
diff --git a/midi-model_amd/csrc/elementwise.hip b/midi-model_amd/csrc/elementwise.hip
--- a/midi-model_amd/csrc/elementwise.hip
+++ b/midi-model_amd/csrc/elementwise.hip
@@ -565,6 +565,27 @@
   return MH_OK;
 }
 
+__global__ __launch_bounds__(256) void coef_from_parts_kernel(const float* __restrict__ parts, int nparts, const float* __restrict__ rstd,
+                                                              int64_t M, float inv_d, float* __restrict__ coef) {
+  __shared__ float acc[4][64];
+  const int r = threadIdx.x & 63, q = threadIdx.x >> 6;
+  const int64_t m = (int64_t)blockIdx.x * 64 + r;
+  float s = 0.f;
+  if (m < M) {
+#pragma unroll 4
+    for (int p = q; p < nparts; p += 4) s += parts[(int64_t)p * M + m];
+  }
+  acc[q][r] = s;
+  __syncthreads();
+  if (q == 0 && m < M) coef[m] = rstd[m] * inv_d * (acc[0][r] + acc[1][r] + acc[2][r] + acc[3][r]);
+}
+extern "C" int mh_row_coef(const float* parts, int nparts, const float* rstd, int64_t M, int D, float* coef, void* stream) {
+  MH_REQUIRE(M > 0 && D > 0 && nparts > 0 && parts != nullptr && rstd != nullptr && coef != nullptr, "row_coef: bad arguments M=%ld D=%d nparts=%d", (long)M, D, nparts);
+  coef_from_parts_kernel<<<(unsigned)((M + 63) / 64), 256, 0, (hipStream_t)stream>>>(parts, nparts, rstd, M, 1.0f / (float)D, coef);
+  MH_LAUNCH_CHECK();
+  return MH_OK;
+}
+
 constexpr int RMS_BWD_MAX_BLOCKS = 1024;
 extern "C" int mh_rmsnorm_bwd_blocks(int64_t M) {
   int64_t g = (M + 3) / 4;
diff --git a/midi-model_amd/csrc/gemm.hip b/midi-model_amd/csrc/gemm.hip
--- a/midi-model_amd/csrc/gemm.hip
+++ b/midi-model_amd/csrc/gemm.hip
@@ -326,7 +326,11 @@
 }
 
 int mh_gemm_pp256_dswiglu_bf16(const void* A, int64_t lda, const void* B, int64_t ldb, const void* GU, int64_t ldgu,
-                               void* DGU, int64_t lddgu, int64_t M, int64_t I, int64_t K, hipStream_t st, const float* rowscale);
+                               void* DGU, int64_t lddgu, int64_t M, int64_t I, int64_t K, hipStream_t st, const float* rowscale,
+                               float* parts);
+int mh_gemm_pp256_normbwd_bf16(const void* A, int64_t lda, const void* B, int64_t ldb, void* C, int64_t ldc, const void* R,
+                               int64_t ldr, const void* X, int64_t ldx, const float* coef, int64_t M, int64_t N, int64_t K,
+                               hipStream_t st);
 int mh_gemm_pp256_scaled_bf16(const void* A, int64_t lda, const void* B, int64_t ldb, void* C, int64_t ldc, int64_t M, int64_t N,
                               int64_t K, const float* rowscale, hipStream_t st);
 
@@ -417,12 +421,12 @@
                  lddgu >= 2 * I,
              "gemm_dswiglu: leading dimensions must be multiples of 8 elements and cover the rows");
   MH_REQUIRE((((uintptr_t)A | (uintptr_t)B | (uintptr_t)GU | (uintptr_t)DGU) & 15) == 0, "gemm_dswiglu: 16-byte alignment");
-  return mh_gemm_pp256_dswiglu_bf16(A, lda, B, ldb, GU, ldgu, DGU, lddgu, M, I, K, (hipStream_t)stream, nullptr);
-}
-
-extern "C" int mh_gemm_dswiglu_scaled(const void* A, int64_t lda, const void* B, int64_t ldb, const void* GU, int64_t ldgu,
-                                      void* DGU, int64_t lddgu, const float* rowscale, int64_t M, int64_t I, int64_t K, int dtype,
-                                      void* stream) {
+  return mh_gemm_pp256_dswiglu_bf16(A, lda, B, ldb, GU, ldgu, DGU, lddgu, M, I, K, (hipStream_t)stream, nullptr, nullptr);
+}
+
+static int gemm_dswiglu_scaled_any(const void* A, int64_t lda, const void* B, int64_t ldb, const void* GU, int64_t ldgu,
+                                   void* DGU, int64_t lddgu, const float* rowscale, float* parts, int64_t M, int64_t I, int64_t K,
+                                   int dtype, void* stream) {
   MH_REQUIRE(dtype == MH_BF16 && g_mh_gemm_variant != 0, "gemm_dswiglu_scaled: served by the production bf16 kernel only");
   MH_REQUIRE(rowscale != nullptr && ((uintptr_t)rowscale & 15) == 0, "gemm_dswiglu_scaled: rowscale must be a 16-byte aligned fp32 [M]");
   MH_REQUIRE(M > 0 && I > 0 && K > 0 && I % 8 == 0, "gemm_dswiglu_scaled: bad shape M=%ld I=%ld K=%ld", (long)M, (long)I, (long)K);
@@ -430,7 +434,36 @@
                  lddgu >= 2 * I,
              "gemm_dswiglu_scaled: leading dimensions must be multiples of 8 elements and cover the rows");
   MH_REQUIRE((((uintptr_t)A | (uintptr_t)B | (uintptr_t)GU | (uintptr_t)DGU) & 15) == 0, "gemm_dswiglu_scaled: 16-byte alignment");
-  return mh_gemm_pp256_dswiglu_bf16(A, lda, B, ldb, GU, ldgu, DGU, lddgu, M, I, K, (hipStream_t)stream, rowscale);
+  return mh_gemm_pp256_dswiglu_bf16(A, lda, B, ldb, GU, ldgu, DGU, lddgu, M, I, K, (hipStream_t)stream, rowscale, parts);
+}
+
+extern "C" int mh_gemm_dswiglu_scaled(const void* A, int64_t lda, const void* B, int64_t ldb, const void* GU, int64_t ldgu,
+                                      void* DGU, int64_t lddgu, const float* rowscale, int64_t M, int64_t I, int64_t K, int dtype,
+                                      void* stream) {
+  return gemm_dswiglu_scaled_any(A, lda, B, ldb, GU, ldgu, DGU, lddgu, rowscale, nullptr, M, I, K, dtype, stream);
+}
+
+extern "C" int mh_gemm_dswiglu_parts(const void* A, int64_t lda, const void* B, int64_t ldb, const void* GU, int64_t ldgu,
+                                     void* DGU, int64_t lddgu, const float* rowscale, float* parts, int64_t M, int64_t I, int64_t K,
+                                     int dtype, void* stream) {
+  MH_REQUIRE(parts != nullptr && I % 64 == 0, "gemm_dswiglu_parts: parts is NULL or I = %ld is not a multiple of 64", (long)I);
+  return gemm_dswiglu_scaled_any(A, lda, B, ldb, GU, ldgu, DGU, lddgu, rowscale, parts, M, I, K, dtype, stream);
+}
+
+extern "C" int mh_gemm_dgrad_normbwd(const void* A, int64_t lda, const void* B, int64_t ldb, void* C, int64_t ldc, const void* R,
+                                     int64_t ldr, const void* X, int64_t ldx, const float* coef, int64_t M, int64_t N, int64_t K,
+                                     int dtype, void* stream) {
+  MH_REQUIRE(dtype == MH_BF16 && g_mh_gemm_variant != 0, "gemm_dgrad_normbwd: served by the production bf16 kernel only");
+  MH_REQUIRE(A != nullptr && B != nullptr && C != nullptr && R != nullptr && X != nullptr && coef != nullptr, "gemm_dgrad_normbwd: NULL argument");
+  MH_REQUIRE(((uintptr_t)coef & 15) == 0, "gemm_dgrad_normbwd: coef must be a 16-byte aligned fp32 [M]");
+  MH_REQUIRE(M > 0 && N > 0 && K > 0, "gemm_dgrad_normbwd: empty problem");
+  MH_REQUIRE(lda % 8 == 0 && ldb % 8 == 0 && ldc % 8 == 0 && ldr % 8 == 0 && ldx % 8 == 0 && lda >= K && ldb >= N && ldc >= N &&
+                 ldr >= N && ldx >= N,
+             "gemm_dgrad_normbwd: leading dimensions must be multiples of 8 elements and cover the rows");
+  MH_REQUIRE((((uintptr_t)A | (uintptr_t)B | (uintptr_t)C | (uintptr_t)R | (uintptr_t)X) & 15) == 0, "gemm_dgrad_normbwd: 16-byte alignment");
+  MH_REQUIRE(C != R && C != X, "gemm_dgrad_normbwd: C must alias neither R nor X");
+  MH_REQUIRE(((M + 255) / 256) * (N / 256) < (1ll << 30), "gemm_dgrad_normbwd: too many tiles");
+  return mh_gemm_pp256_normbwd_bf16(A, lda, B, ldb, C, ldc, R, ldr, X, ldx, coef, M, N, K, (hipStream_t)stream);
 }
 
 extern "C" int mh_gemm_nt_scaled(const void* A, int64_t lda, const void* B, int64_t ldb, void* C, int64_t ldc,
diff --git a/midi-model_amd/csrc/gemm_pp256.hip b/midi-model_amd/csrc/gemm_pp256.hip
--- a/midi-model_amd/csrc/gemm_pp256.hip
+++ b/midi-model_amd/csrc/gemm_pp256.hip
@@ -100,6 +100,26 @@
   } x;
   x.u = v;
   return x.b;
+}
+
+__device__ inline float line_dot2(const bf16x8& a0, const bf16x8& b0, const bf16x8& a1, const bf16x8& b1) {
+  union {
+    bf16x8 v8;
+    bf16x2 h[4];
+  } ua0, ub0, ua1, ub1;
+  ua0.v8 = a0;
+  ub0.v8 = b0;
+  ua1.v8 = a1;
+  ub1.v8 = b1;
+  float d = 0.f;
+#pragma unroll
+  for (int e = 0; e < 4; ++e) d = __builtin_amdgcn_fdot2_f32_bf16(ua0.h[e], ub0.h[e], d, false);
+#pragma unroll
+  for (int e = 0; e < 4; ++e) d = __builtin_amdgcn_fdot2_f32_bf16(ua1.h[e], ub1.h[e], d, false);
+  d += dpp_move<0xB1>(d);
+  d += dpp_move<0x4E>(d);
+  d += dpp_move<0x141>(d);
+  return d;
 }
 
 constexpr int P8_REGION = 128 * 128;
@@ -327,8 +347,12 @@
                                                             const bf16* R, int64_t ldr, int64_t M, int64_t N, int64_t K,
                                                             float alpha, float beta, int tiles_n, int nwg,
                                                             int64_t k_per_split, float* __restrict__ ws,
-                                                            const void* __restrict__ zero16, float* aux, int lean_epi) {
-  static_assert(NRM == 0 || (ML == 1 && ABL == 0 && !TA && (!TB || (EPI == 1 && NRM == 2))), "the norm forms ride on the K-step-64 loops only");
+                                                            const void* __restrict__ zero16, float* aux, int lean_epi,
+                                                            const bf16* X, int64_t ldx, float* parts) {
+  static_assert(NRM == 0 || (ML == 1 && ABL == 0 && !TA && (!TB || (EPI == 1 && (NRM == 2 || NRM == 4)) || (EPI == 0 && NRM == 3))), "the norm forms ride on the K-step-64 loops only");
+  static_assert(NRM != 4 || (TB && EPI == 1), "the row-dot partials come out of the SwiGLU-backward epilogue");
+  constexpr bool RSC = (NRM == 2 || NRM == 4);
+  static_assert(NRM != 3 || (TB && EPI == 0), "the norm-backward epilogue belongs to the dgrad form");
   static_assert(NRM != 1 || EPI == 0, "sum-of-squares partials come out of the plain epilogue");
   extern __shared__ __attribute__((aligned(16))) char smem[];
   const int tid = threadIdx.x, lane = tid & 63;
@@ -361,7 +385,7 @@
   };
 
   if constexpr (ML >= 1) {
-    if constexpr (NRM == 2) {
+    if constexpr (NRM >= 2) {
       if (wave == 0) {
         const int64_t r = m0 + lane * 4;
         glds16((r + 4 <= M) ? (const void*)(aux + r) : zero16, smem + LDS_BYTES);
@@ -458,7 +482,7 @@
   }
 
   float rs[8];
-  if constexpr (NRM == 2) {
+  if constexpr (RSC) {
     const float* rl = reinterpret_cast<const float*>(smem + LDS_BYTES);
 #pragma unroll
     for (int fm = 0; fm < 8; ++fm) rs[fm] = rl[grp * 128 + fm * 16 + fi];
@@ -478,6 +502,8 @@
       const unsigned vo_c = (unsigned)(((grp * 128 + lrow) * (int)ldc + c * 8) * 2), so_c = (unsigned)ldc * 16u;
       const unsigned up_off = (unsigned)N * 2u;
       bf16x8 gq[2][8], uq[2][8];
+      __amdgpu_buffer_rsrc_t rp;
+      if constexpr (NRM == 4) rp = tile_rsrc(parts + ((n0 + wn * 64) >> 6) * M + m0, 256 * 4);
       auto request = [&](int half, int i0) {
 #pragma unroll
         for (int i = i0; i < i0 + 4; ++i) {
@@ -495,7 +521,7 @@
           for (int fn = 0; fn < 4; ++fn) {
             const int row = fmh * 16 + fi, ch = fn * 4 + fg;
             f32x4 t4 = acc[fn][half * 4 + fmh];
-            if constexpr (NRM == 2) t4 *= rs[half * 4 + fmh];
+            if constexpr (RSC) t4 *= rs[half * 4 + fmh];
             *reinterpret_cast<f32x4*>(wreg + row * 256 + ((ch ^ (row & 15)) << 4)) = t4;
           }
 #pragma unroll
@@ -511,8 +537,13 @@
           expand8_bf16(uq[half][i], u);
           mh_dswiglu8(dv, g, u, dg, du);
           const unsigned so = (unsigned)(half * 8 + i) * so_c;
-          tile_store(as_u32x4(cvt8_bf16(dg)), rc, vo_c + so, 2 );
-          tile_store(as_u32x4(cvt8_bf16(du)), rc, vo_c + so + up_off, 2);
+          const bf16x8 og = cvt8_bf16(dg), ou = cvt8_bf16(du);
+          tile_store(as_u32x4(og), rc, vo_c + so, 2 );
+          tile_store(as_u32x4(ou), rc, vo_c + so + up_off, 2);
+          if constexpr (NRM == 4) {
+            const float d = line_dot2(og, gq[half][i], ou, uq[half][i]);
+            if (c == 0) __builtin_amdgcn_raw_buffer_store_b32(__float_as_uint(d), rp, (unsigned)((grp * 128 + half * 64 + i * 8 + lrow) * 4), 0, 0);
+          }
         }
       }
       return;
@@ -543,7 +574,7 @@
         for (int fn = 0; fn < 4; ++fn) {
           const int row = fmh * 16 + fi, ch = fn * 4 + fg;
           f32x4 t4 = acc[fn][half * 4 + fmh];
-          if constexpr (NRM == 2) t4 *= rs[half * 4 + fmh];
+          if constexpr (RSC) t4 *= rs[half * 4 + fmh];
           *reinterpret_cast<f32x4*>(wreg + row * 256 + ((ch ^ (row & 15)) << 4)) = t4;
         }
       if (half == 0) request(1);
@@ -569,6 +600,10 @@
         const bf16x8 og = cvt8_bf16(dg), ou = cvt8_bf16(du);
         __builtin_nontemporal_store(og, reinterpret_cast<bf16x8*>(C + m * ldc + n));
         __builtin_nontemporal_store(ou, reinterpret_cast<bf16x8*>(C + m * ldc + N + n));
+        if constexpr (NRM == 4) {
+          const float d = line_dot2(og, gv[i], ou, uv[i]);
+          if (c == 0) parts[((n0 + wn * 64) >> 6) * M + m] = d;
+        }
       }
     }
     return;
@@ -815,6 +850,54 @@
         }
         if (m >= M || n + 8 > N) continue;
         __builtin_nontemporal_store(cvt8_bf16(v), reinterpret_cast<bf16x8*>(C + m * ldc + n));
+      }
+    }
+    return;
+  }
+  if constexpr (NRM == 3) {
+    char* wreg = smem + wave * 16384;
+    const float* cl = reinterpret_cast<const float*>(smem + LDS_BYTES) + grp * 128;
+    const int lrow = lane >> 3, c = lane & 7;
+    const int64_t rows_left = (M - m0 < QBM) ? M - m0 : QBM, nw = n0 + wn * 64;
+    const __amdgpu_buffer_rsrc_t rc = tile_rsrc(C + m0 * ldc + nw, ((rows_left - 1) * ldc + 64) * 2);
+    const __amdgpu_buffer_rsrc_t rr = tile_rsrc(R + m0 * ldr + nw, ((rows_left - 1) * ldr + 64) * 2);
+    const __amdgpu_buffer_rsrc_t rx = tile_rsrc(X + m0 * ldx + nw, ((rows_left - 1) * ldx + 64) * 2);
+    const unsigned vo_c = (unsigned)(((grp * 128 + lrow) * (int)ldc + c * 8) * 2), so_c = (unsigned)ldc * 16u;
+    const unsigned vo_r = (unsigned)(((grp * 128 + lrow) * (int)ldr + c * 8) * 2), so_r = (unsigned)ldr * 16u;
+    const unsigned vo_x = (unsigned)(((grp * 128 + lrow) * (int)ldx + c * 8) * 2), so_x = (unsigned)ldx * 16u;
+    bf16x8 rq[2][8], xq[2][8];
+    auto request = [&](int half, int i0) {
+#pragma unroll
+      for (int i = i0; i < i0 + 4; ++i) {
+        rq[half][i] = as_bf16x8(__builtin_amdgcn_raw_buffer_load_b128(rr, vo_r, (unsigned)(half * 8 + i) * so_r, 0));
+        xq[half][i] = as_bf16x8(__builtin_amdgcn_raw_buffer_load_b128(rx, vo_x, (unsigned)(half * 8 + i) * so_x, 0));
+      }
+    };
+    request(0, 0);
+    request(0, 4);
+#pragma unroll
+    for (int half = 0; half < 2; ++half) {
+#pragma unroll
+      for (int fmh = 0; fmh < 4; ++fmh)
+#pragma unroll
+        for (int fn = 0; fn < 4; ++fn) {
+          const int row = fmh * 16 + fi, ch = fn * 4 + fg;
+          *reinterpret_cast<f32x4*>(wreg + row * 256 + ((ch ^ (row & 15)) << 4)) = acc[fn][half * 4 + fmh];
+        }
+#pragma unroll
+      for (int i = 0; i < 8; ++i) {
+        if (half == 0 && (i == 2 || i == 6)) request(1, i == 2 ? 0 : 4);
+        const int row = i * 8 + lrow;
+        const f32x4 lo = *reinterpret_cast<const f32x4*>(wreg + row * 256 + (((2 * c) ^ (row & 15)) << 4));
+        const f32x4 hi = *reinterpret_cast<const f32x4*>(wreg + row * 256 + (((2 * c + 1) ^ (row & 15)) << 4));
+        const float ncf = -cl[half * 64 + row];
+        const float v[8] = {lo[0], lo[1], lo[2], lo[3], hi[0], hi[1], hi[2], hi[3]};
+        float rf[8], xf[8], of[8];
+        expand8_bf16(rq[half][i], rf);
+        expand8_bf16(xq[half][i], xf);
+#pragma unroll
+        for (int e = 0; e < 8; ++e) of[e] = __builtin_fmaf(ncf, xf[e], v[e] + rf[e]);
+        tile_store(as_u32x4(cvt8_bf16(of)), rc, vo_c + (unsigned)(half * 8 + i) * so_c, 2 );
       }
     }
     return;
@@ -1013,8 +1096,8 @@
 template <bool TA, bool TB, int ABL, int EPI = 0, int ML = 0, int NRM = 0>
 int launch_one(const void* A, int64_t lda, const void* B, int64_t ldb, void* C, int64_t ldc, const void* R, int64_t ldr,
                int64_t M, int64_t N, int64_t K, float alpha, float beta, int splitk, void* workspace, hipStream_t st,
-               float* aux = nullptr) {
-  constexpr int LDSB = LDS_BYTES + ((ABL & 128) ? P8_DBG_BYTES : 0) + (NRM == 2 ? 1024 : 0);
+               float* aux = nullptr, const void* X = nullptr, int64_t ldx = 0, float* parts = nullptr) {
+  constexpr int LDSB = LDS_BYTES + ((ABL & 128) ? P8_DBG_BYTES : 0) + (NRM >= 2 ? 1024 : 0);
   constexpr int MAX_DEV = 64;
   static void* zero16_of[MAX_DEV] = {};
   static bool attr_set_of[MAX_DEV] = {};
@@ -1047,7 +1130,7 @@
   dim3 grid(nwg, 1, splitk);
   gemm_pp256_kernel<TA, TB, ABL, EPI, ML, NRM><<<grid, 512, LDSB, st>>>((const bf16*)A, lda, (const bf16*)B, ldb, (bf16*)C, ldc,
                                                           (const bf16*)R, ldr, M, N, K, alpha, beta, (int)tiles_n, nwg, kps,
-                                                          (float*)workspace, zero16, aux, g_mh_gemm_lean_epi);
+                                                          (float*)workspace, zero16, aux, g_mh_gemm_lean_epi, (const bf16*)X, ldx, parts);
   MH_LAUNCH_CHECK();
   return MH_OK;
 }
@@ -1140,9 +1223,14 @@
 }
 
 int mh_gemm_pp256_dswiglu_bf16(const void* A, int64_t lda, const void* B, int64_t ldb, const void* GU, int64_t ldgu,
-                               void* DGU, int64_t lddgu, int64_t M, int64_t I, int64_t K, hipStream_t st, const float* rowscale) {
+                               void* DGU, int64_t lddgu, int64_t M, int64_t I, int64_t K, hipStream_t st, const float* rowscale,
+                               float* parts) {
+  MH_REQUIRE(parts == nullptr || (rowscale != nullptr && I % 64 == 0), "gemm_dswiglu_parts: the row-dot partials come out of the row-scaled form, one per 64 columns (I %% 64 == 0)");
   if (rowscale != nullptr) {
     MH_REQUIRE(g_mh_gemm_k64 == 1 && M % 4 == 0, "gemm_dswiglu_scaled: needs the K-step-64 dgrad loop and M %% 4 == 0");
+    if (parts != nullptr)
+      return launch_one<false, true, 0, 1, 1, 4>(A, lda, B, ldb, DGU, lddgu, GU, ldgu, M, I, K, 1.f, 0.f, 1, nullptr, st,
+                                                 const_cast<float*>(rowscale), nullptr, 0, parts);
     return launch_one<false, true, 0, 1, 1, 2>(A, lda, B, ldb, DGU, lddgu, GU, ldgu, M, I, K, 1.f, 0.f, 1, nullptr, st,
                                                const_cast<float*>(rowscale));
   }
@@ -1155,3 +1243,12 @@
   MH_REQUIRE(g_mh_gemm_k64 != 0, "gemm_rowss: needs the K-step-64 main loop (option gemm_k64)");
   return launch_one<false, false, 0, 0, 1, 1>(A, lda, B, ldb, C, ldc, R, ldr, M, N, K, 1.f, R ? 1.f : 0.f, 1, nullptr, st, rowss);
 }
+
+int mh_gemm_pp256_normbwd_bf16(const void* A, int64_t lda, const void* B, int64_t ldb, void* C, int64_t ldc, const void* R,
+                               int64_t ldr, const void* X, int64_t ldx, const float* coef, int64_t M, int64_t N, int64_t K,
+                               hipStream_t st) {
+  MH_REQUIRE(g_mh_gemm_k64 == 1 && M % 4 == 0 && N % 256 == 0, "gemm_dgrad_normbwd: needs the K-step-64 dgrad loop, M %% 4 == 0 and N %% 256 == 0");
+  MH_REQUIRE(ldc < (1 << 22) && ldr < (1 << 22) && ldx < (1 << 22), "gemm_dgrad_normbwd: row strides beyond 2^22 elements are not supported (32-bit tile offsets)");
+  return launch_one<false, true, 0, 0, 1, 3>(A, lda, B, ldb, C, ldc, R, ldr, M, N, K, 1.f, 1.f, 1, nullptr, st,
+                                             const_cast<float*>(coef), X, ldx, nullptr);
+}
diff --git a/midi-model_amd/engine.py b/midi-model_amd/engine.py
--- a/midi-model_amd/engine.py
+++ b/midi-model_amd/engine.py
@@ -8,7 +8,7 @@
 
 import torch
 
-from . import ops
+from . import norm_bwd, ops
 
 
 @dataclass
@@ -227,6 +227,13 @@
     return ok
 
 
+def norm_bwd_fused(spec: StackSpec, x: torch.Tensor):
+    mode = os.environ.get("MH_NORM_BWD_FUSED", "1")
+    if mode == "0" or not norm_bwd.dgrad_normbwd_ok(x, spec.D):
+        return False, False
+    return spec.I % 64 == 0 and (spec.kind == "token" or mode == "2"), spec.kind == "token"
+
+
 def runs_folded(spec: StackSpec, x: torch.Tensor, save: bool, kv_out: Optional[list], fold_kept: bool) -> bool:
     if save:
         return fold_kept and kv_out is None and train_fold_ok(spec, x)
@@ -279,24 +286,48 @@
     M, D = dx.shape
     H, I = spec.H, spec.I
     wq_n, wgu_n = fold
+    fuse_mlp, fuse_attn = norm_bwd_fused(spec, dx)
     a = keep.a
     if a is None:
         a = _empty((M, I), dx)
         ops.swiglu_fwd(keep.gu, a)
     dz2 = _empty((M, 2 * I), dx)
-    ops.gemm_dswiglu(dx, lw.wd, keep.gu, dz2, rowscale=keep.rstd2)
-    linear_wgrad(dx, a, lg.wd, accumulate)
-    del a
-    t2 = _empty((M, D), dx)
-    ops.gemm_nt(dz2, wgu_n, t2, tb=True)
-    ops.wgrad_folded(dz2, keep.x2, lg.wgu, lw.n2, lw.wgu, lg.n2, accumulate)
-    del dz2
     dx2 = _empty((M, D), dx)
-    ops.rmsnorm_bwd_folded(keep.x2, keep.rstd2, t2, dx, dx2)
-    do = t2
+    if fuse_mlp:
+        parts = _empty((I // 64, M), dx, torch.float32)
+        ops.gemm_dswiglu(dx, lw.wd, keep.gu, dz2, rowscale=keep.rstd2, parts=parts)
+        linear_wgrad(dx, a, lg.wd, accumulate)
+        del a
+        coef = _empty((M,), dx, torch.float32)
+        norm_bwd.row_coef(parts, keep.rstd2, D, coef)
+        del parts
+        norm_bwd.gemm_dgrad_normbwd(dz2, wgu_n, dx, keep.x2, coef, dx2)
+        ops.wgrad_folded(dz2, keep.x2, lg.wgu, lw.n2, lw.wgu, lg.n2, accumulate)
+        del dz2
+        do = _empty((M, D), dx)
+    else:
+        ops.gemm_dswiglu(dx, lw.wd, keep.gu, dz2, rowscale=keep.rstd2)
+        linear_wgrad(dx, a, lg.wd, accumulate)
+        del a
+        t2 = _empty((M, D), dx)
+        ops.gemm_nt(dz2, wgu_n, t2, tb=True)
+        ops.wgrad_folded(dz2, keep.x2, lg.wgu, lw.n2, lw.wgu, lg.n2, accumulate)
+        del dz2
+        ops.rmsnorm_bwd_folded(keep.x2, keep.rstd2, t2, dx, dx2)
+        do = t2
     ops.gemm_nt(dx2, lw.wo, do, tb=True)
     linear_wgrad(dx2, keep.o, lg.wo, accumulate)
     dz1 = _empty((M, 3 * D), dx)
+    if fuse_attn:
+        parts = _empty((H, M), dx, torch.float32)
+        ops.tokattn_bwd(keep.qkv, do, dz1, nseq, slen, H, spec.scale, rope.cos, rope.sin, rowscale=keep.rstd1, parts=parts)
+        del do
+        coef = _empty((M,), dx, torch.float32)
+        norm_bwd.row_coef(parts, keep.rstd1, D, coef)
+        del parts
+        norm_bwd.gemm_dgrad_normbwd(dz1, wq_n, dx2, keep.x, coef, dx)
+        ops.wgrad_folded(dz1, keep.x, lg.wqkv, lw.n1, lw.wqkv, lg.n1, accumulate)
+        return dx
     if spec.kind == "event":
         ops.attn_bwd(keep.qkv, keep.o, do, keep.lse, dz1, nseq, slen, H, spec.scale, rope.cos, rope.sin, rowscale=keep.rstd1)
     else:
diff --git a/midi-model_amd/norm_bwd.py b/midi-model_amd/norm_bwd.py
--- /dev/null
+++ b/midi-model_amd/norm_bwd.py
@@ -0,0 +1,39 @@
+from __future__ import annotations
+
+import torch
+
+from . import ops
+from .lib import lib
+from .ops import _p, _rowmajor, _stream, dt
+
+
+def dgrad_normbwd_ok(x: torch.Tensor, D: int) -> bool:
+    return (x.is_cuda and x.dtype == torch.bfloat16 and D % 256 == 0 and x.shape[0] % 4 == 0 and ops.get_option("gemm") != 0
+            and ops.get_option("gemm_k64") == 1)
+
+
+def row_coef(parts: torch.Tensor, rstd: torch.Tensor, D: int, coef: torch.Tensor) -> torch.Tensor:
+    nparts, M = parts.shape
+    assert parts.dtype == rstd.dtype == coef.dtype == torch.float32 and rstd.shape == coef.shape == (M,)
+    assert parts.is_contiguous() and rstd.is_contiguous() and coef.is_contiguous()
+    lib().call("mh_row_coef", _p(parts), nparts, _p(rstd), M, D, _p(coef), _stream())
+    return coef
+
+
+def gemm_dgrad_normbwd(dz: torch.Tensor, w: torch.Tensor, res: torch.Tensor, x: torch.Tensor, coef: torch.Tensor,
+                       out: torch.Tensor) -> torch.Tensor:
+    M, K = dz.shape
+    N = w.shape[1]
+    assert w.shape[0] == K and res.shape == x.shape == out.shape == (M, N) and coef.shape == (M,) and coef.dtype == torch.float32
+    assert dz.dtype == w.dtype == res.dtype == x.dtype == out.dtype and coef.is_contiguous()
+    assert out.data_ptr() != res.data_ptr() and out.data_ptr() != x.data_ptr()
+    prof = ops.gemm_profile
+    if prof is not None:
+        e0, e1 = torch.cuda.Event(enable_timing=True), torch.cuda.Event(enable_timing=True)
+        e0.record()
+    lib().call("mh_gemm_dgrad_normbwd", _p(dz), _rowmajor(dz), _p(w), _rowmajor(w), _p(out), _rowmajor(out), _p(res), _rowmajor(res),
+               _p(x), _rowmajor(x), _p(coef), M, N, K, dt(dz), _stream())
+    if prof is not None:
+        e1.record()
+        prof.append((e0, e1, 2.0 * M * N * K, (M, N, K, 1, 0, 1, "+normbwd")))
+    return out
diff --git a/midi-model_amd/ops.py b/midi-model_amd/ops.py
--- a/midi-model_amd/ops.py
+++ b/midi-model_amd/ops.py
@@ -238,7 +238,7 @@
 
 
 def gemm_dswiglu(dx: torch.Tensor, wd: torch.Tensor, gu: torch.Tensor, dgu: torch.Tensor,
-                 rowscale: Optional[torch.Tensor] = None) -> torch.Tensor:
+                 rowscale: Optional[torch.Tensor] = None, parts: Optional[torch.Tensor] = None) -> torch.Tensor:
     M, K = dx.shape
     I = wd.shape[1]
     assert wd.shape[0] == K and gu.shape == (M, 2 * I) and dgu.shape == (M, 2 * I) and dx.dtype == wd.dtype == gu.dtype
@@ -246,7 +246,13 @@
     if prof is not None:
         e0, e1 = torch.cuda.Event(enable_timing=True), torch.cuda.Event(enable_timing=True)
         e0.record()
-    if rowscale is not None:
+    assert parts is None or rowscale is not None
+    if parts is not None:
+        assert rowscale.shape == (M,) and rowscale.dtype == torch.float32 and rowscale.is_contiguous()
+        assert I % 64 == 0 and parts.shape == (I // 64, M) and parts.dtype == torch.float32 and parts.is_contiguous()
+        lib().call("mh_gemm_dswiglu_parts", _p(dx), _rowmajor(dx), _p(wd), _rowmajor(wd), _p(gu), _rowmajor(gu), _p(dgu),
+                   _rowmajor(dgu), _p(rowscale), _p(parts), M, I, K, dt(dx), _stream())
+    elif rowscale is not None:
         assert rowscale.shape == (M,) and rowscale.dtype == torch.float32 and rowscale.is_contiguous()
         lib().call("mh_gemm_dswiglu_scaled", _p(dx), _rowmajor(dx), _p(wd), _rowmajor(wd), _p(gu), _rowmajor(gu), _p(dgu),
                    _rowmajor(dgu), _p(rowscale), M, I, K, dt(dx), _stream())
@@ -515,7 +521,14 @@
     return o
 
 
-def tokattn_bwd(qkv, dout, dqkv, N: int, T: int, H: int, scale: float, cos_t=None, sin_t=None, rowscale=None):
+def tokattn_bwd(qkv, dout, dqkv, N: int, T: int, H: int, scale: float, cos_t=None, sin_t=None, rowscale=None, parts=None):
+    assert parts is None or rowscale is not None
+    if parts is not None:
+        assert rowscale.shape == (N * T,) and rowscale.dtype == torch.float32 and rowscale.is_contiguous()
+        assert parts.shape == (H, N * T) and parts.dtype == torch.float32 and parts.is_contiguous()
+        lib().call("mh_tokattn_bwd_parts", _p(qkv), _p(dout), _p(dqkv), _p(rowscale), _p(parts), N, T, H, scale, _p(cos_t), _p(sin_t),
+                   dt(qkv), _stream())
+        return dqkv
     if rowscale is not None:
         assert rowscale.shape == (N * T,) and rowscale.dtype == torch.float32 and rowscale.is_contiguous()
         lib().call("mh_tokattn_bwd_scaled", _p(qkv), _p(dout), _p(dqkv), _p(rowscale), N, T, H, scale, _p(cos_t), _p(sin_t),
```

Result: no change. 365,800 events/s (median of 6 runs) (+0.9%).
